# IvanBanny/para-ortho-pca-bo

Hardware: AMD Instinct MI355X
Metric: BO iterations/sec (incl. GP refit + EI opt), BBOB f15 d=40 (higher is better)
Workload: dtype f64; 1 GPU; configs[1]: PCA_BO on BBOB f15 d=40, budget=450, n_DoE=120, EI, var_threshold=0.95; one run per GPU (run list f15/d40/instances 0..N-1 partitioned by pcabo.sharding), timed steps spread evenly over the 330 BO iterations of the run; num_restarts=10, raw_samples=512, batch_limit=5, maxiter=200, parallelism=run-parallel x1

## Files before the change

para-ortho-pca-bo_amd/csrc/host_selftest.cpp:

```cpp
#include "../../include/pcabo.h"
#include "host_side.h"
#include "lb_plan.h"

#include <atomic>
#include <cmath>
#include <cstdint>
#include <cstdio>
#include <cstdlib>
#include <cstring>
#include <vector>

namespace {

int g_fail = 0;
#define CHECK(c, ...) do { if (!(c)) { std::fprintf(stderr, "FAIL %s:%d: ", __FILE__, __LINE__); std::fprintf(stderr, __VA_ARGS__); std::fprintf(stderr, "\n"); ++g_fail; } } while (0)

struct Lcg {
  uint64_t s;
  explicit Lcg(uint64_t seed) : s(seed * 6364136223846793005ull + 1442695040888963407ull) {}
  double uni() { s = s * 6364136223846793005ull + 1442695040888963407ull; return (double)(s >> 11) * (1.0 / 9007199254740992.0); }
};

struct Objective { std::vector<double> c; };
double fg_objective(const double* x, double* g, void* user) {
  const Objective* o = static_cast<const Objective*>(user);
  const int n = (int)o->c.size();
  double f = 0.0;
  for (int i = 0; i < n; ++i) {
    const double d = x[i] - o->c[i], s = 1.0 + 0.3 * std::sin(3.0 * x[i]);
    f += d * d * s;
    g[i] = 2.0 * d * s + d * d * 0.9 * std::cos(3.0 * x[i]);
  }
  for (int i = 0; i + 1 < n; ++i) { f += 0.1 * x[i] * x[i + 1]; g[i] += 0.1 * x[i + 1]; g[i + 1] += 0.1 * x[i]; }
  return f;
}

void test_minimize() {
  for (int nvar : {1, 2, 7, 33, 64, 65, 200}) {
    for (int variant = 0; variant < 3; ++variant) {
      pcabo_lbfgsb_set_vector_kernels(variant == 1);
      pcabo_lbfgsb_set_sum_order(variant == 2);
      Lcg r(17 + nvar);
      Objective o; o.c.resize(nvar);
      std::vector<double> x(nvar), lo(nvar), hi(nvar);
      for (int i = 0; i < nvar; ++i) { o.c[i] = 4.0 * r.uni() - 2.0; lo[i] = -1.0 - r.uni(); hi[i] = 1.0 + r.uni(); x[i] = 6.0 * r.uni() - 3.0; }
      double f = 0.0; int nit = 0, nfev = 0, task = 0;
      const int wf = pcabo_lbfgsb_minimize(nvar, x.data(), lo.data(), hi.data(), fg_objective, &o, 10, 1e7, 1e-5, 200, 15000, 20, &f, &nit, &nfev, &task);
      CHECK(wf >= 0 && wf <= 2, "warnflag %d", wf);
      CHECK(std::isfinite(f) && nfev >= 1, "f %g nfev %d", f, nfev);
      for (int i = 0; i < nvar; ++i) CHECK(x[i] >= lo[i] && x[i] <= hi[i], "x[%d] = %g outside the box", i, x[i]);
    }
  }
  pcabo_lbfgsb_set_vector_kernels(1);
  pcabo_lbfgsb_set_sum_order(0);
  {
    const int nvar = 12;
    Objective o; o.c.assign(nvar, 0.5);
    std::vector<double> x(nvar, 2.0), lo(nvar, -INFINITY), hi(nvar, INFINITY);
    for (int i = 0; i < nvar; i += 3) lo[i] = 0.75;
    for (int i = 1; i < nvar; i += 3) hi[i] = 0.25;
    double f = 0.0; int nit = 0, nfev = 0, task = 0;
    const int wf = pcabo_lbfgsb_minimize(nvar, x.data(), lo.data(), hi.data(), fg_objective, &o, 17, 1e7, 1e-5, 200, 15000, 20, &f, &nit, &nfev, &task);
    CHECK(wf == 0, "half-bounded problem: warnflag %d task %d", wf, task);
  }
  CHECK(pcabo_lbfgsb_minimize(0, nullptr, nullptr, nullptr, fg_objective, nullptr, 10, 1e7, 1e-5, 1, 1, 20, nullptr, nullptr, nullptr, nullptr) == PCABO_ERR_ARG, "bad arguments accepted");
}

void test_sobol() {
  for (int k : {1, 3, 36, 89}) {
    Lcg r(5 + k);
    std::vector<int64_t> state((size_t)k * 30), ltm((size_t)k * 30 * 30), shift(k);
    for (auto& v : state) v = (int64_t)(r.uni() * 1073741824.0);
    for (auto& v : ltm) v = r.uni() < 0.5 ? 0 : 1;
    for (auto& v : shift) v = (int64_t)(r.uni() * 1073741824.0);
    CHECK(pcabo_sobol_scramble(state.data(), ltm.data(), k) == PCABO_OK, "scramble");
    for (int n : {1, 2, 512, 513}) {
      std::vector<double> lo(k, -1.5), rng(k, 3.0), out((size_t)n * k, -7.0);
      CHECK(pcabo_sobol_draw(state.data(), shift.data(), k, n, lo.data(), rng.data(), out.data()) == PCABO_OK, "draw");
      for (double v : out) CHECK(v >= -1.5 && v <= 1.5, "sample %g outside the box", v);
      CHECK(pcabo_sobol_draw(state.data(), shift.data(), k, n, nullptr, nullptr, out.data()) == PCABO_OK, "draw (unit cube)");
      for (double v : out) CHECK(v >= 0.0 && v < 1.0, "unit sample %g", v);
    }
  }
}

void test_torch_rng() {
  struct Blob { uint64_t seed; int32_t left, seeded; uint64_t next; uint64_t state[624]; unsigned char tail[32]; };
  const int rows = 70, n = 512, n_pick = 10;
  std::vector<Blob> blobs(rows), again;
  std::vector<double> vals((size_t)rows * n);
  for (int r = 0; r < rows; ++r) {
    Lcg g(900 + r);
    blobs[r].seed = 900 + r; blobs[r].left = 1 + (r * 37) % 624; blobs[r].seeded = 1; blobs[r].next = 624 - blobs[r].left;
    for (auto& w : blobs[r].state) w = (uint64_t)(g.uni() * 4294967296.0);
    for (auto& c : blobs[r].tail) c = 0;
    for (int i = 0; i < n; ++i) vals[(size_t)r * n + i] = r == 5 ? 1.25 : 40.0 * g.uni() - 20.0;
  }
  again = blobs;
  std::vector<void*> ptr(rows);
  for (int r = 0; r < rows; ++r) ptr[r] = &blobs[r];
  ptr[7] = nullptr;
  std::vector<int64_t> out((size_t)rows * n_pick, -1), out1((size_t)rows * n_pick, -1);
  std::vector<int> flags(rows, -1), flags1(rows, -1);
  CHECK(pcabo_boltzmann_pick_rows(ptr.data(), vals.data(), rows, n, n_pick, 1.0, out.data(), flags.data()) == PCABO_OK, "pick rows");
  for (int r = 0; r < rows; ++r) {
    void* p1 = r == 7 ? nullptr : (void*)&again[r];
    CHECK(pcabo_boltzmann_pick_rows(&p1, vals.data() + (size_t)r * n, 1, n, n_pick, 1.0, out1.data() + (size_t)r * n_pick, flags1.data() + r) == PCABO_OK, "pick row %d", r);
    CHECK(flags[r] == flags1[r] && flags[r] == (r == 7 ? 2 : r == 5 ? 1 : 0), "flag of row %d: %d / %d", r, flags[r], flags1[r]);
    if (flags[r] != 0) continue;
    for (int j = 0; j < n_pick; ++j) {
      CHECK(out[(size_t)r * n_pick + j] == out1[(size_t)r * n_pick + j], "row %d pick %d differs between the all-rows call and the one-row call", r, j);
      CHECK(out[(size_t)r * n_pick + j] >= 0 && out[(size_t)r * n_pick + j] < n, "row %d pick %d out of range", r, j);
    }
    CHECK(blobs[r].left == again[r].left && blobs[r].next == again[r].next && blobs[r].state[0] == again[r].state[0], "generator of row %d", r);
  }
  std::vector<int64_t> bits(2000);
  CHECK(pcabo_torch_randint2(&blobs[0], 2000, bits.data()) == PCABO_OK, "randint2");
  for (int64_t b : bits) CHECK(b == 0 || b == 1, "bit %lld", (long long)b);
  std::vector<double> w((size_t)3 * n);
  Lcg g(77);
  for (auto& v : w) v = 0.01 + g.uni();
  void* three[3] = {&blobs[1], nullptr, &blobs[2]};
  std::vector<int64_t> idx(3 * n_pick, -1);
  CHECK(pcabo_torch_multinomial_rows(three, w.data(), 3, n, n_pick, idx.data()) == PCABO_OK, "multinomial rows");
  for (int j = 0; j < n_pick; ++j) CHECK(idx[j] >= 0 && idx[j] < n && idx[n_pick + j] == -1 && idx[2 * n_pick + j] >= 0, "multinomial pick %d", j);
  blobs[3].left = 900;
  CHECK(pcabo_torch_randint2(&blobs[3], 4, bits.data()) == PCABO_ERR_ARG, "a broken blob accepted");
}

void test_sobol_rows() {
  const int rows = 37, n = 130, kmax = 36;
  int ks[rows];
  for (int r = 0; r < rows; ++r) ks[r] = r == 0 ? 3 : r == 2 ? 1 : 1 + (r * 7) % 36;
  std::vector<std::vector<int64_t>> st(rows), sh(rows);
  std::vector<double> boxes((size_t)rows * 2 * kmax, NAN), out((size_t)rows * n * kmax, -7.0), one((size_t)n * kmax);
  std::vector<const int64_t*> sp(rows), hp(rows);
  std::vector<double*> op(rows);
  for (int r = 0; r < rows; ++r) {
    Lcg g(40 + r);
    st[r].resize((size_t)ks[r] * 30); sh[r].resize(ks[r]);
    for (auto& v : st[r]) v = (int64_t)(g.uni() * 1073741824.0);
    for (auto& v : sh[r]) v = (int64_t)(g.uni() * 1073741824.0);
    for (int j = 0; j < ks[r]; ++j) { boxes[(size_t)r * 2 * kmax + j] = -1.0 - j; boxes[(size_t)r * 2 * kmax + ks[r] + j] = 2.0 + r; }
    sp[r] = r == 2 ? nullptr : st[r].data(); hp[r] = sh[r].data(); op[r] = out.data() + (size_t)r * n * kmax;
  }
  CHECK(pcabo_sobol_draw_rows(sp.data(), hp.data(), ks, rows, n, boxes.data(), 2 * kmax, op.data()) == PCABO_OK, "draw rows");
  for (int r = 0; r < rows; ++r) {
    if (r == 2) { CHECK(op[r][0] == -7.0, "a skipped run was written"); continue; }
    std::vector<double> rng(ks[r]);
    for (int j = 0; j < ks[r]; ++j) rng[j] = boxes[(size_t)r * 2 * kmax + ks[r] + j] - boxes[(size_t)r * 2 * kmax + j];
    CHECK(pcabo_sobol_draw(st[r].data(), sh[r].data(), ks[r], n, boxes.data() + (size_t)r * 2 * kmax, rng.data(), one.data()) == PCABO_OK, "draw");
    for (int i = 0; i < n * ks[r]; ++i) CHECK(one[i] == op[r][i], "run %d element %d", r, i);
    if (ks[r] < kmax) CHECK(op[r][(size_t)n * ks[r]] == -7.0, "write behind the points of run %d", r);
  }
}

void test_plan() {
  std::vector<int> plan(LB_PLAN_INTS + 64, 0x5a5a5a5a);
  for (int NP = 64; NP <= LB_MAXNP; NP += 64) {
    const int S = NP / 64;
    for (int n = NP - 63; n <= NP; ++n) {
      lb_build_plan_t(plan.data(), n, S);
// ... 169 lines not shown
    for (int j = 0; j < n; ++j) {
      double v = 0.0;
      for (int p = std::max(i, j); p < n; ++p) v += Li[p * n + i] * Li[p * n + j];
      Kin[i * n + j] = v;
      a[i] += v * (gp.y[j] - c);
    }
  for (int t = 0; t < 6; ++t) h[t] = 0.0;
  for (int i = 0; i < n; ++i) {
    h[0] += std::log(L[i * n + i]); h[1] += (gp.y[i] - c) * a[i]; h[2] += a[i]; h[3] += a[i] * a[i]; h[4] += Kin[i * n + i];
    for (int j = 0; j < n; ++j) h[5] += (a[i] * a[j] - Kin[i * n + j]) * dK[i * n + j];
  }
  return true;
}
TinyGP tiny_gp(int seed, int n = 12, int k = 2) {
  Lcg r(seed);
  TinyGP gp; gp.n = n; gp.k = k; gp.Z.resize((size_t)n * k); gp.y.resize(n);
  for (auto& v : gp.Z) v = r.uni();
  for (int i = 0; i < n; ++i) gp.y[i] = std::sin(3.0 * gp.Z[i * k] + 0.3 * seed) + gp.Z[i * k + 1] * gp.Z[i * k + 1] - 0.6 + 0.1 * (r.uni() - 0.5);
  return gp;
}

struct FitOut { int status; double theta[3], loss; int info[4]; };
FitOut fit_out(const FitRun& r) {
  FitOut o;
  std::memset(&o, 0, sizeof(o));
  o.status = r.status;
  if (r.status == PCABO_OK) { std::memcpy(o.theta, r.xr, sizeof(o.theta)); o.loss = r.fr; r.report(o.info); }
  return o;
}
const double FIT_START[3] = {0.006737946999085467, 0.0, 0.0};

struct FitDrive { std::vector<FitOut> out; std::vector<std::vector<double>> evals; std::vector<int> rested; int rounds = 0; };
FitDrive drive_fits(const std::vector<TinyGP>& gps, const std::vector<const double*>& start, const std::vector<int>& fail_at) {
  const size_t B = gps.size();
  std::vector<FitRun> runs(B);
  std::vector<double> hs(6 * B, 0.0);
  FitDrive d;
  d.evals.resize(B); d.rested.assign(B, 0);
  for (size_t b = 0; b < B; ++b) { runs[b].bind(&hs[6 * b]); if (start[b]) runs[b].init(start[b]); }
  const int rc = fit_rounds(runs, gps[0].n, [&](const std::vector<const double*>& th, int* st) {
    ++d.rounds;
    for (size_t b = 0; b < B; ++b) {
      const FitRun& r = runs[b];
      if (!th[b]) { CHECK(r.state == FitRun::OUT, "run %zu: no theta but not out", b); continue; }
      const bool resting = r.state == FitRun::RESTING;
      if (resting) {
        CHECK(std::memcmp(th[b], r.xr, sizeof(r.xr)) == 0, "run %zu rests away from its result", b);
        ++d.rested[b];
      } else {
        d.evals[b].insert(d.evals[b].end(), th[b], th[b] + 3);
      }
      const bool fail = !resting && fail_at[b] > 0 && (int)d.evals[b].size() / 3 == fail_at[b];
      st[b] = !fail && tiny_gp_sums(gps[b], th[b], &hs[6 * b]) ? PCABO_OK : PCABO_ERR_NOT_PD;
    }
    return (int)PCABO_OK;
  });
  CHECK(rc == PCABO_OK, "fit_rounds: %d", rc);
  for (const FitRun& r : runs) {
    CHECK(r.state == FitRun::RESTING || r.state == FitRun::OUT, "a run is still stepping after the rounds");
    d.out.push_back(fit_out(r));
  }
  return d;
}

void test_fit_run() {
  {
    const TinyGP gp = tiny_gp(3);
    const double th[3] = {0.02, 0.15, -0.4};
    double h[6], f = 0.0, g[3], worst = 0.0;
    CHECK(tiny_gp_sums(gp, th, h), "the dense GP could not be factored");
    mll_assemble(h, gp.n, th, &f, g);
    for (int i = 0; i < 3; ++i) {
      const double step = i == 0 ? 1e-6 * th[0] : 1e-6;
      double tp[3] = {th[0], th[1], th[2]}, tm[3] = {th[0], th[1], th[2]}, fp = 0.0, fm = 0.0;
      tp[i] += step; tm[i] -= step;
      CHECK(tiny_gp_sums(gp, tp, h), "factor"); mll_assemble(h, gp.n, tp, &fp, nullptr);
      CHECK(tiny_gp_sums(gp, tm, h), "factor"); mll_assemble(h, gp.n, tm, &fm, nullptr);
      const double fd = (fp - fm) / (tp[i] - tm[i]), err = std::fabs(fd - g[i]) / (1.0 + std::fabs(g[i]));
      if (err > worst) worst = err;
      CHECK(err < 1e-6, "gradient %d: %.12g against the difference quotient %.12g", i, g[i], fd);
    }
    std::printf("mll_assemble against central differences: worst %.2e (bound 1e-6)\n", worst);
  }
  const int B = 5;
  std::vector<TinyGP> gps;
  for (int b = 0; b < B; ++b) gps.push_back(tiny_gp(10 + b));
  const FitDrive all = drive_fits(gps, std::vector<const double*>(B, FIT_START), std::vector<int>(B, 0));
  int rested = 0, nfev_min = 1 << 30, nfev_max = 0;
  for (int b = 0; b < B; ++b) {
    const FitDrive one = drive_fits({gps[b]}, {FIT_START}, {0});
    CHECK(all.out[b].status == PCABO_OK && all.out[b].info[0] > 2, "run %d: status %d after %d iterations", b, all.out[b].status, all.out[b].info[0]);
    CHECK(std::memcmp(&all.out[b], &one.out[0], sizeof(FitOut)) == 0, "run %d in lock-step differs from the run alone", b);
    CHECK(all.evals[b] == one.evals[0], "run %d was evaluated at other points in lock-step", b);
    CHECK(all.out[b].info[1] <= (int)all.evals[b].size() / 3, "run %d counts %d evaluations of %zu", b, all.out[b].info[1], all.evals[b].size() / 3);
    CHECK(one.rested[0] == 0 && one.rounds == (int)one.evals[0].size() / 3, "a run alone took a round without an evaluation");
    rested += all.rested[b];
    nfev_min = std::min(nfev_min, all.out[b].info[1]); nfev_max = std::max(nfev_max, all.out[b].info[1]);
  }
  CHECK(nfev_min < nfev_max && rested > 0, "no run finished before another (evaluations %d .. %d): nothing rode along", nfev_min, nfev_max);
  {
    const FitDrive d = drive_fits({gps[0], gps[1]}, {nullptr, FIT_START}, {0, 0});
    CHECK(d.out[0].status == PCABO_ERR_ARG && d.evals[0].empty(), "a parked run was stepped");
    CHECK(std::memcmp(&d.out[1], &all.out[1], sizeof(FitOut)) == 0, "a run beside a parked run differs from the run alone");
  }
  const int total = (int)all.evals[0].size() / 3;
  int end_at_last_evaluated = 0;
  for (int e = 1; e <= total; ++e) {
    const FitDrive d = drive_fits({gps[0], gps[1]}, {FIT_START, FIT_START}, {e, 0});
    CHECK(std::memcmp(&d.out[1], &all.out[1], sizeof(FitOut)) == 0, "failure %d of run 0 disturbed run 1", e);
    const FitOut& o = d.out[0];
    const std::vector<double>& ev = d.evals[0];
    if (e == 1) { CHECK(o.status == PCABO_ERR_NOT_PD && ev.size() == 3, "start not factored: status %d", o.status); continue; }
    CHECK(o.status == PCABO_OK && o.info[2] == 2 && o.info[3] == PCABO_FIT_TASK_NOT_PD, "failure %d: status %d warnflag %d task %d", e, o.status, o.info[2], o.info[3]);
    CHECK(o.info[1] == e - 1, "failure %d: %d evaluations counted", e, o.info[1]);
    CHECK((int)ev.size() / 3 == e + 1 && std::memcmp(&ev[3 * e], o.theta, sizeof(o.theta)) == 0, "failure %d: no evaluation at the result behind it", e);
    bool evaluated = false;
    for (int i = 0; i < e - 1; ++i) evaluated = evaluated || std::memcmp(&ev[3 * i], o.theta, sizeof(o.theta)) == 0;
    CHECK(evaluated, "failure %d: the result was never evaluated", e);
    if (std::memcmp(&ev[3 * (e - 2)], o.theta, sizeof(o.theta)) == 0) ++end_at_last_evaluated;
    double h[6], f = 0.0;
    CHECK(tiny_gp_sums(gps[0], o.theta, h), "factor"); mll_assemble(h, gps[0].n, o.theta, &f, nullptr);
    CHECK(f == o.loss, "failure %d: the loss is not the one at the result", e);
  }
  CHECK(end_at_last_evaluated > 0, "no failure met the first trial of a line search");
  {
    std::vector<FitRun> run(1);
    double h[6] = {0, 0, 0, 0, 0, 0};
    int evals = 0;
    std::vector<double> rhos;
    const int n = 12;
    const double G = 0.5;
    const auto linear = [&](const std::vector<const double*>& th, int* st) {
      const double s2 = th[0][0], rho = th[0][2], u = std::log(s2) + 4.0;
      CHECK(mll_theta_ok(th[0]), "asked to evaluate a theta outside the domain");
      h[1] = 2.0 * n * G * rho; h[5] = -2.0 * n * G * softplus_host(rho) * (1.0 + std::exp(-rho)); h[3] = 2.0 * (1.0 + u) / s2;
      ++evals; rhos.push_back(rho); st[0] = PCABO_OK;
      return (int)PCABO_OK;
    };
    run[0].bind(h); run[0].init(FIT_START);
    CHECK(fit_rounds(run, n, linear) == PCABO_OK, "fit_rounds");
    const FitOut o = fit_out(run[0]);
    CHECK(o.status == PCABO_OK && o.info[2] == 2 && o.info[3] == PCABO_FIT_TASK_DOMAIN, "domain stop: status %d warnflag %d task %d", o.status, o.info[2], o.info[3]);
    CHECK(o.info[0] >= 1 && evals == o.info[1] + 1 && evals > 3, "domain stop: %d iterations, %d evaluations, %d counted", o.info[0], evals, o.info[1]);
    CHECK(rhos.back() == o.theta[2] && rhos[evals - 2] < -600.0 && std::count(rhos.begin(), rhos.end(), o.theta[2]) == 2,
          "domain stop: the result rho %g is not an earlier iterate evaluated again at the end (last trial %g)", o.theta[2], rhos[evals - 2]);
    const double far[3] = {FIT_START[0], 0.0, -800.0};
    evals = 0;
    run[0].init(far);
    CHECK(fit_rounds(run, n, linear) == PCABO_OK, "fit_rounds");
    CHECK(run[0].status == PCABO_ERR_ARG && run[0].state == FitRun::OUT && evals == 0, "start outside the domain: status %d, %d evaluations", run[0].status, evals);
  }
}

}

int main(int argc, char** argv) {
  const int workers = argc > 1 ? std::atoi(argv[1]) : 4;
  test_minimize();
  test_sobol();
  test_sobol_rows();
  test_torch_rng();
  test_plan();
  test_restart_group();
  test_fit_run();
  test_gang_pool(1, 3);
  test_gang_pool(workers, 11);
  if (g_fail) { std::fprintf(stderr, "host selftest: %d check(s) failed\n", g_fail); return 1; }
  std::printf("host selftest ok\n");
  return 0;
}
```

para-ortho-pca-bo_amd/csrc/host_side.h:

```cpp
#pragma once
#include "../../include/pcabo.h"
#include "lbfgsb.h"

#include <algorithm>
#include <cmath>
#include <condition_variable>
#include <cstring>
#include <functional>
#include <mutex>
#include <thread>
#include <utility>
#include <vector>

struct RestartGroup : LbfgsbDriver {
  int q0 = 0, nq = 0, k = 0;
  std::vector<double> lo, hi, vc;
  void init(const double* ics, const double* bounds, int q0_, int nq_, int k_, int maxiter, int sum_order = 0) {
    q0 = q0_; nq = nq_; k = k_;
    lo.resize(nq * k); hi.resize(nq * k);
    for (int j = 0; j < nq; ++j)
      for (int c = 0; c < k; ++c) { lo[j * k + c] = bounds[c]; hi[j * k + c] = bounds[k + c]; }
    LbfgsbDriver::init(nq * k, ics + (size_t)q0 * k, lo.data(), hi.data(), sum_order, maxiter);
  }
  bool absorb(const double* hVal, const double* hGrad, int row) {
    double fs = 0.0;
    bool nan = false;
    for (int j = 0; j < nq; ++j) fs += hVal[row + j];
    for (int t = 0; t < nq * k; ++t) {
      const double gv = -hGrad[(size_t)row * k + t];
      if (gv != gv) nan = true;
      g[t] = gv;
    }
    if (nan) return false;
    LbfgsbDriver::absorb(-fs);
    vc.assign(hVal + row, hVal + row + nq);
    return true;
  }
};

struct RunRestarts {
  std::vector<RestartGroup> grp;
  int status = PCABO_OK;
  double* xq = nullptr;
  const double *val = nullptr, *grad = nullptr;
  void init(const double* ics, const double* bounds, int num_restarts, int batch_limit, int k, int maxiter, int sum_order = 0) {
    grp.resize((num_restarts + batch_limit - 1) / batch_limit);
    for (size_t gi = 0; gi < grp.size(); ++gi) {
      const int q0 = (int)gi * batch_limit;
      grp[gi].init(ics, bounds, q0, std::min(batch_limit, num_restarts - q0), k, maxiter, sum_order);
    }
    status = PCABO_OK;
  }
  void bind(double* xq_, const double* val_, const double* grad_) { xq = xq_; val = val_; grad = grad_; }
  template <class Redo> int end_points(double* cand, double* vals, Redo&& redo) const {
    int n = 0;
    for (const RestartGroup& rg : grp) {
      double* c = cand + (size_t)rg.q0 * rg.k;
      for (size_t t = 0; t < rg.x.size(); ++t) c[t] = rg.x[t] < rg.lo[t] ? rg.lo[t] : (rg.x[t] > rg.hi[t] ? rg.hi[t] : rg.x[t]);
      if (rg.have_cache && memcmp(c, rg.xc.data(), rg.x.size() * sizeof(double)) == 0) std::copy(rg.vc.begin(), rg.vc.end(), vals + rg.q0);
      else { redo(rg); ++n; }
    }
    return n;
  }
  int end_points(double* cand, double* vals) const { return end_points(cand, vals, [](const RestartGroup&) {}); }
  bool report(int* info, size_t slot0) const {
    bool any = false;
    for (size_t gi = 0; gi < grp.size(); ++gi) {
      const RestartGroup& rg = grp[gi];
      const int wf = rg.opt.warnflag();
      if (info) { int* o = info + 4 * (slot0 + gi); o[0] = rg.niter; o[1] = rg.nfev; o[2] = wf; o[3] = rg.opt.task(); }
      if (wf == 2) any = true;
    }
    return any;
  }
};

inline unsigned group_entry(int run, int q0, int nq) { return ((unsigned)run << 16) | ((unsigned)q0 << 8) | (unsigned)nq; }
inline unsigned query_entry(int run, int q) { return ((unsigned)run << 16) | (unsigned)q; }

template <class Stage, class Eval>
int run_rounds(RunRestarts* runs, const std::vector<int>& order, Stage&& stage, Eval&& eval) {
  std::vector<std::pair<RunRestarts*, RestartGroup*>> pend;
  size_t ng = 0;
  for (int b : order) ng += runs[b].grp.size();
  pend.reserve(ng);
  for (;;) {
    pend.clear();
    for (int b : order) {
      RunRestarts& run = runs[b];
      if (run.status != PCABO_OK) continue;
      for (RestartGroup& rg : run.grp) {
        if (!rg.advance()) continue;
        std::memcpy(run.xq + (size_t)rg.q0 * rg.k, rg.x.data(), rg.x.size() * sizeof(double));
        stage(b, rg);
        pend.push_back({&run, &rg});
      }
    }
    if (pend.empty()) return PCABO_OK;
    const int rc = eval();
    if (rc != PCABO_OK) return rc;
    for (auto& pe : pend)
      if (!pe.second->absorb(pe.first->val, pe.first->grad, pe.second->q0)) pe.first->status = PCABO_ERR_NAN;
  }
}

inline double softplus_host(double x) { return x > 20.0 ? x : std::log1p(std::exp(x)); }
inline bool mll_theta_ok(const double* theta) {
  const double s2 = theta[0], c = theta[1], ls = softplus_host(theta[2]);
  return s2 > 0.0 && std::isfinite(s2) && std::isfinite(c) && ls > 0.0 && std::isfinite(ls);
}
inline void mll_assemble(const double* h, int n, const double* theta, double* loss, double* grad) {
  const double s2 = theta[0], rho = theta[2];
  const double ls = softplus_host(rho);
  const double LOG2PI = 1.8378770664093453;
  const double lnz = std::log(s2), u = lnz + 4.0;
  const double log_n = -0.5 * h[1] - h[0] - 0.5 * n * LOG2PI;
  const double log_prior = -lnz - 0.5 * LOG2PI - 0.5 * u * u;
  *loss = -(log_n + log_prior) / n;
  if (grad) {
    const double sig = 1.0 / (1.0 + std::exp(-rho));
    grad[0] = -((0.5 * (h[3] - h[4])) + (-1.0 - u) / s2) / n;
    grad[1] = -h[2] / n;
    grad[2] = -(0.5 * h[5] * sig / ls) / n;
  }
}

struct FitRun {
  enum { STEPPING, END, RESTING, OUT };
  LbfgsbDriver fit;
  int state = OUT, status = PCABO_ERR_ARG, stop_task = 0;
  double xr[3] = {0, 0, 0}, fr = 0.0;
  const double* h = nullptr;
  void bind(const double* h_) { h = h_; }
  void init(const double* theta0) {
    const double lower[3] = {1e-4, -INFINITY, -INFINITY}, upper[3] = {INFINITY, INFINITY, INFINITY};
    fit.keep_accepted = true;
    fit.init(3, theta0, lower, upper);
    state = STEPPING; status = PCABO_OK; stop_task = 0;
  }
  const double* next() {
    if (state == STEPPING && !fit.advance()) finish();
    if (state == STEPPING && !mll_theta_ok(fit.x.data())) {
      if (fit.have_cache) { stop_task = PCABO_FIT_TASK_DOMAIN; finish(); }
      else { state = OUT; status = PCABO_ERR_ARG; }
    }
    return state == STEPPING ? fit.x.data() : (state == END ? xr : nullptr);
  }
  const double* rest() const { return state == RESTING ? xr : nullptr; }
  void took(int st, int n) {
    if (state == OUT) return;
    if (state == STEPPING && st == PCABO_ERR_NOT_PD && fit.have_cache) {
      stop_task = PCABO_FIT_TASK_NOT_PD;
      finish();
      return;
    }
    if (st != PCABO_OK) { state = OUT; status = st; return; }
    if (state == STEPPING) {
      double f = 0.0;
      mll_assemble(h, n, fit.x.data(), &f, fit.g.data());
      fit.absorb(f);
    } else if (state == END) {
      mll_assemble(h, n, xr, &fr, nullptr);
      state = RESTING;
    }
  }
  void report(int* info) const {
    info[0] = fit.niter; info[1] = fit.nfev;
    info[2] = stop_task ? 2 : fit.opt.warnflag();
    info[3] = stop_task ? stop_task : fit.opt.task();
  }

 private:
  void finish() {
    std::memcpy(xr, stop_task ? fit.xacc.data() : fit.x.data(), sizeof(xr));
    fr = fit.fc;
    state = (stop_task == PCABO_FIT_TASK_NOT_PD || !fit.have_cache || std::memcmp(xr, fit.xc.data(), sizeof(xr)) != 0) ? END : RESTING;
  }
};

template <class Eval>
int fit_rounds(std::vector<FitRun>& runs, int n, Eval&& eval) {
  std::vector<const double*> th(runs.size(), nullptr);
  std::vector<int> st(runs.size(), PCABO_OK);
  for (;;) {
    int pending = 0;
    for (size_t b = 0; b < runs.size(); ++b) {
      const double* t = runs[b].next();
      if (t) ++pending;
      th[b] = t ? t : runs[b].rest();
    }
    if (pending == 0) return PCABO_OK;
    const int rc = eval(th, st.data());
    if (rc != PCABO_OK) return rc;
    for (size_t b = 0; b < runs.size(); ++b) runs[b].took(st[b], n);
  }
}

struct GangPool {
  std::vector<std::thread> th;
  std::mutex mu;
  std::condition_variable cv, cv_done;
  std::function<void(int)> fn;
  unsigned epoch = 0;
  int pending = 0;
  bool quit = false;
  void start(int n) {
    const unsigned epoch0 = epoch;
    for (int i = 1; i < n; ++i)
      th.emplace_back([this, i, epoch0] {
        unsigned seen = epoch0;
        for (;;) {
          std::function<void(int)> f;
          {
            std::unique_lock<std::mutex> lk(mu);
            cv.wait(lk, [&] { return quit || epoch != seen; });
            if (quit) return;
            seen = epoch;
            f = fn;
          }
          f(i);
          { std::lock_guard<std::mutex> lk(mu); if (--pending == 0) cv_done.notify_all(); }
        }
      });
  }
  void run(std::function<void(int)> f) {
    {
      std::lock_guard<std::mutex> lk(mu);
      fn = f;
// ... 17 lines not shown
```

para-ortho-pca-bo_amd/csrc/kernels_acq.hip:

```cpp
#include "pcabo_internal.h"
#include <algorithm>
#include <cstdlib>
#include <mutex>

#define PSTRIDE (2 + 2 * PCABO_MAXD)

#ifdef PCABO_ACQ_TIMING
__device__ unsigned long long g_acq_stamps[16];
#define STAMP(i) do { if (blockIdx.x == gridDim.x / 2 && blockIdx.y == 0 && threadIdx.x == 0) g_acq_stamps[i] = wall_clock64(); } while (0)
#define STAMP_FIN(i) do { if (blockIdx.y == 0 && threadIdx.x == 0) g_acq_stamps[i] = wall_clock64(); } while (0)
extern "C" int pcabo_debug_acq_stamps(unsigned long long* out16) {
  return hipMemcpyFromSymbol(out16, HIP_SYMBOL(g_acq_stamps), sizeof(g_acq_stamps)) == hipSuccess ? 0 : -3;
}
#else
#define STAMP(i)
#define STAMP_FIN(i)
#endif

__device__ inline void st_wt(double* p, double v) {
  __hip_atomic_store(p, v, __ATOMIC_RELAXED, __HIP_MEMORY_SCOPE_AGENT);
}

template <int SLAB>
__device__ inline int slab_row(int s, int m, int NP) {
  return m < SLAB / 2 ? (SLAB / 2) * s + m : NP - (SLAB / 2) * (s + 1) + (m - SLAB / 2);
}

__device__ void acq_finish_query(const double* base, int S, int k, int q, const double* bounds4, const double* ystats,
                                 const AcqParams& p, double* val, double* grad, double* host_val, double* host_grad,
                                 int lane);

__device__ inline void grad_partial_sum(const double* base, int S, int c, int first, double* gs_out, double* gm_out) {
  double gs = 0.0, gm = 0.0;
  int sl = first;
  for (; sl + 21 < S; sl += 24) {
    double a[8], b[8];
#pragma unroll
    for (int t = 0; t < 8; ++t) {
      a[t] = base[(size_t)(sl + 3 * t) * PSTRIDE + 2 + c];
      b[t] = base[(size_t)(sl + 3 * t) * PSTRIDE + 2 + PCABO_MAXD + c];
    }
#pragma unroll
    for (int t = 0; t < 8; ++t) { gs += a[t]; gm += b[t]; }
  }
  {
    double a[8], b[8];
#pragma unroll
    for (int t = 0; t < 8; ++t) {
      const int si = sl + 3 * t;
      const int sc = si < S ? si : 0;
      a[t] = base[(size_t)sc * PSTRIDE + 2 + c];
      b[t] = base[(size_t)sc * PSTRIDE + 2 + PCABO_MAXD + c];
    }
#pragma unroll
    for (int t = 0; t < 8; ++t) { if (sl + 3 * t < S) { gs += a[t]; gm += b[t]; } }
  }
  *gs_out = gs;
  *gm_out = gm;
}

__device__ void acq_finish_scalar(const double* base, int S, int q, const double* ystats, const AcqParams& p, double* val,
                                  double* host_val, double* coef, int lane);
__device__ void acq_scalar_core(double vv, double mus, int q, double ym, double ysd, const AcqParams& p, double* val,
                                double* host_val, double* coef, int l);
template <int SLAB>
__device__ inline void acq_tail(int combine, double* s_v, double* partial, unsigned int* counters, int q, int S, int k,
                                const double* bounds4, const double* ystats, const AcqParams& prm, double* val,
                                double* grad, double* host_val, double* host_grad, HostMirror* hm,
                                unsigned long long seq, int tid, int w, int l) {
  if (!combine) return;
  int* s_flag = reinterpret_cast<int*>(s_v + SLAB);
  STAMP(6);
  asm volatile("s_waitcnt vmcnt(0)" ::: "memory");
  __syncthreads();
  STAMP(7);
  if (tid == 0) {
    unsigned int t = __hip_atomic_fetch_add(&counters[q], 1u, __ATOMIC_RELAXED, __HIP_MEMORY_SCOPE_AGENT);
    int last = ((t % (unsigned int)S) == (unsigned int)(S - 1));
    if (last) {
      __builtin_amdgcn_fence(__ATOMIC_ACQUIRE, "agent");
      asm volatile("s_waitcnt vmcnt(0)" ::: "memory");
    }
    *s_flag = last;
  }
  __syncthreads();
  if (!*s_flag) return;
  STAMP_FIN(8);
  const double* base = partial + (size_t)q * S * PSTRIDE;
  double* s_fin = s_v + SLAB + 2;
  double* s_coef = s_fin + 6 * PCABO_MAXD;
  double rng_c = 1.0;
  if (w == 0) {
    if (prm.want_grad && l < k) rng_c = bounds4[PCABO_MAXD + l] - bounds4[l];
    acq_finish_scalar(base, S, q, ystats, prm, val, host_val, s_coef, l);
  } else if (prm.want_grad) {
    for (int c = l; c < k; c += 64) {
      double gs, gm;
      grad_partial_sum(base, S, c, w - 1, &gs, &gm);
      s_fin[(w - 1) * 2 * PCABO_MAXD + c] = gs;
      s_fin[(w - 1) * 2 * PCABO_MAXD + PCABO_MAXD + c] = gm;
    }
  }
  __syncthreads();
  STAMP_FIN(13);
  if (w == 0) {
    if (prm.want_grad) {
      const double c_mu = s_coef[0], c_sg = s_coef[1];
      for (int c = l; c < k; c += 64) {
        const double gs = (s_fin[c] + s_fin[2 * PCABO_MAXD + c]) + s_fin[4 * PCABO_MAXD + c];
        const double gm = (s_fin[PCABO_MAXD + c] + s_fin[3 * PCABO_MAXD + c]) + s_fin[5 * PCABO_MAXD + c];
        const double g = __fma_rn(c_mu, gm, c_sg * gs) / (c == l ? rng_c : bounds4[PCABO_MAXD + c] - bounds4[c]);
        grad[(size_t)q * k + c] = g;
        if (host_grad) host_grad[(size_t)q * k + c] = g;
      }
    }
    if (hm && l == 0)
      __hip_atomic_store(const_cast<unsigned long long*>(&hm->qflag[q]), seq, __ATOMIC_RELEASE, __HIP_MEMORY_SCOPE_SYSTEM);
    STAMP_FIN(9);
#ifdef PCABO_ACQ_TIMING
    asm volatile("s_waitcnt vmcnt(0)" ::: "memory");
    STAMP_FIN(10);
#endif
  }
}

#define ACQ_BATCH_PROLOGUE()                                                                                     \
  unsigned run_ = blockIdx.z;                                                                                    \
  int qsel_ = -1;                                                                                                \
  if (ab.table) {                                                                                                \
    const unsigned e_ = reinterpret_cast<const unsigned*>(qa.x)[blockIdx.y];                                     \
    run_ = e_ >> 16; qsel_ = (int)(e_ & 0xffffu);                                                                \
  }                                                                                                              \
  if (ab.zs) {                                                                                                   \
    ZnT = zrun(ZnT, ab.zs, run_); R = zrun(R, ab.zs, run_); alpha = zrun(alpha, ab.zs, run_);                    \
    bounds4 = zrun(bounds4, ab.zs, run_); ystats = zrun(ystats, ab.zs, run_); partial = zrun(partial, ab.zs, run_); \
    counters = zrun(counters, ab.zs, run_); val = zrun(val, ab.zs, run_); grad = zrun(grad, ab.zs, run_);        \
    Xq = zrun(Xq, ab.xq_host ? ab.hzs : ab.zs, run_);                                                            \
    host_val = zrun(host_val, ab.hzs, run_); host_grad = zrun(host_grad, ab.hzs, run_); hm = zrun(hm, ab.hzs, run_); \
    if (ab.k_dev) k = *zrun(ab.k_dev, ab.zs, run_);                                                              \
    if (ab.bestf) prm.best_f = *zrun(ab.bestf, ab.zs, run_);                                                     \
    if (ab.hyp) prm.inv_ls = zrun(ab.hyp, ab.zs, run_)[PCABO_HYP_INV_LS];                                        \
  }                                                                                                              \
  (void)qsel_;

template <int SLAB>
__global__ __launch_bounds__(256) void k_acq_fused(
    QueryArgs qa, const double* __restrict__ Xq, int q_total, int n, int k, int NP, int ld,
    const double* __restrict__ ZnT, const double* __restrict__ R, const double* __restrict__ alpha,
    const double* __restrict__ bounds4, const double* __restrict__ ystats, AcqParams prm, double* partial,
    unsigned int* counters, double* __restrict__ val, double* __restrict__ grad,
    double* host_val, double* host_grad, HostMirror* hm, unsigned long long seq, int combine, int ,
    MailPair* , MailPair* , AcqBatch ab) {
  ACQ_BATCH_PROLOGUE()
  const double inv_ls = prm.inv_ls;
  const int kernel = prm.kernel, want_grad = prm.want_grad;
  extern __shared__ __attribute__((aligned(16))) double s_dyn[];
  double* s_ks = s_dyn;
  double* s_cf = s_dyn + NP;
  double* s_tm = s_dyn + 2 * NP;
  double* s_xn = s_dyn + 3 * NP;
  double* s_v = s_xn + PCABO_MAXD;
  const int tid = threadIdx.x, w = tid >> 6, l = tid & 63;
  const int s = blockIdx.x, q = ab.table ? qsel_ : (int)blockIdx.y, S = gridDim.x;
  double* out = partial + ((size_t)q * S + s) * PSTRIDE;
  STAMP(0);

  if (tid < k) {
    double lo = bounds4[tid], hi = bounds4[PCABO_MAXD + tid];
    double xv = Xq ? Xq[(size_t)q * k + tid] : qa.x[q * k + tid];
    s_xn[tid] = (xv - lo) / (hi - lo);
  }
  __syncthreads();
  STAMP(1);
  const double s5 = 2.23606797749979;
  for (int j = tid; j < NP; j += 256) {
    double ks = 0.0, cf = 0.0;
    if (j < n) {
      double sq = 0.0;
      for (int c = 0; c < k; ++c) { double dlt = s_xn[c] - ZnT[(size_t)c * ld + j]; sq += dlt * dlt; }
      sq *= inv_ls * inv_ls;
      if (kernel == 1) {
        ks = exp(-0.5 * sq);
        cf = -ks * inv_ls * inv_ls;
      } else {
        double dist = sqrt(fmax(sq, 1e-30));
        double e = exp(-s5 * dist);
        ks = ((s5 * dist + 1.0) + (5.0 / 3.0) * (dist * dist)) * e;
        cf = -(5.0 / 3.0) * (1.0 + s5 * dist) * e * inv_ls * inv_ls;
      }
    }
    s_ks[j] = ks;
    s_cf[j] = cf;
  }
  __syncthreads();
  STAMP(2);
  {
    constexpr int RW = SLAB / 4;
    int ri[RW];
    const double* Rr[RW];
    double acc[RW];
    int imax = 0;
#pragma unroll
    for (int u = 0; u < RW; ++u) {
      ri[u] = slab_row<SLAB>(s, w + 4 * u, NP); Rr[u] = R + (size_t)ri[u] * ld; acc[u] = 0.0; imax = max(imax, ri[u]);
    }
    for (int j = l; j <= imax; j += 64) {
      const double kj = s_ks[j];
#pragma unroll
      for (int u = 0; u < RW; ++u) acc[u] += Rr[u][j] * kj;
    }
#pragma unroll
    for (int u = 0; u < RW; ++u) acc[u] = wave_sum(acc[u]);
    if (l == 0) {
#pragma unroll
      for (int u = 0; u < RW; ++u) s_v[w + 4 * u] = acc[u];
    }
  }
  __syncthreads();
  STAMP(3);
  if (w == 0) {
    double vv = 0.0, mu = 0.0;
    if (l < SLAB) {
      const int i = slab_row<SLAB>(s, l, NP);
      const double vi = s_v[l];
      vv = vi * vi;
      if (i < n) mu = alpha[i] * s_ks[i];
    }
    vv = wave_sum(vv);
    mu = wave_sum(mu);
    if (l == 0) { st_wt(out + 0, vv); st_wt(out + 1, mu); }
  }
  if (want_grad) {
  __syncthreads();
  STAMP(4);
  for (int j = tid; j < NP; j += 256) {
    double wj = 0.0;
#pragma unroll
    for (int m = 0; m < SLAB; ++m) wj += R[(size_t)slab_row<SLAB>(s, m, NP) * ld + j] * s_v[m];
    const bool mine = ((j / (SLAB / 2)) == s) || (((NP - 1 - j) / (SLAB / 2)) == s);
    const double cf = s_cf[j];
    s_tm[j] = (mine && j < n) ? alpha[j] * cf : 0.0;
    s_ks[j] = wj * cf;
  }
  __syncthreads();
  STAMP(5);
  for (int c0 = 0; c0 < k; c0 += 32) {
    double gs[8], gm[8], xc[8];
    const double* zrow[8];
#pragma unroll
    for (int u = 0; u < 8; ++u) {
      const int c = c0 + w + 4 * u;
      const int cc = c < k ? c : 0;
      gs[u] = 0.0; gm[u] = 0.0; xc[u] = s_xn[cc]; zrow[u] = ZnT + (size_t)cc * ld;
    }
    for (int j = l; j < n; j += 64) {
      const double ts = s_ks[j], tm = s_tm[j];
#pragma unroll
      for (int u = 0; u < 8; ++u) {
        const double dlt = xc[u] - zrow[u][j];
        gs[u] += ts * dlt;
        gm[u] += tm * dlt;
      }
    }
#pragma unroll
    for (int u = 0; u < 8; ++u) { gs[u] = wave_sum(gs[u]); gm[u] = wave_sum(gm[u]); }
    if (l == 0) {
#pragma unroll
      for (int u = 0; u < 8; ++u) {
        const int c = c0 + w + 4 * u;
        if (c < k) { st_wt(out + 2 + c, gs[u]); st_wt(out + 2 + PCABO_MAXD + c, gm[u]); }
      }
    }
  }
  }

  acq_tail<SLAB>(combine, s_v, partial, counters, q, S, k, bounds4, ystats, prm, val, grad, host_val, host_grad, hm, seq, tid, w, l);
}

#define FIN_STAGE_PER_WAVE (11 * 2 * 40)
__device__ inline bool acq_server_finisher(const MailPair* rec, int S, int k, int q, unsigned long long seq,
                                           const double* ystats, const AcqParams& prm, double* val, double* grad,
                                           double* host_val, double* host_grad, HostMirror* hm, double rng_c,
                                           double* s_fin, double* s_coef, double* s_stage, int* s_srv,
                                           unsigned long long t0, int w, int l) {
  if (w == 0) {
    const double ym = ystats[0], ysd = ystats[1];
    const void* ptr[8];
    pcabo_u4 o[8];
    const MailPair* mine = rec + (size_t)(l < S ? l : 0) * PSTRIDE;
#pragma unroll
    for (int t = 0; t < 8; ++t) ptr[t] = mine + (t & 1);
    for (;;) {
      ld_pairs_sys8(ptr, o);
      const bool ok = pair_tag(o[0]) == seq && pair_tag(o[1]) == seq;
      if (__all(ok)) break;
      if (__any(wall_clock64() - t0 > PCABO_SERVER_TIMEOUT_TICKS)) { if (l == 0) *s_srv = 1; break; }
      __builtin_amdgcn_s_sleep(1);
    }
    double vm[2] = {l < S ? pair_value(o[0]) : 0.0, l < S ? pair_value(o[1]) : 0.0};
    wave_sum_multi<2>(vm, l);
    constexpr int lane_vv = wave_multi_lane(2, 0), lane_mus = wave_multi_lane(2, 1);
    const double vv = read_lane(vm[0], lane_vv), mus = read_lane(vm[0], lane_mus);
    acq_scalar_core(vv, mus, q, ym, ysd, prm, val, host_val, s_coef, l);
  } else if (prm.want_grad) {
    const int first = w - 1;
    const int ns = first < S ? (S - first + 2) / 3 : 0;
    const int total = ns * 2 * k;
    double* stage = s_stage + (size_t)(w - 1) * FIN_STAGE_PER_WAVE;
    for (int i0 = 0; i0 < total; i0 += 512) {
      const void* ptr[8];
      int item[8];
#pragma unroll
      for (int t = 0; t < 8; ++t) {
        const int i = i0 + l + 64 * t;
        item[t] = i < total ? i : -1;
        const int ii = i < total ? i : 0;
        const int st = ii / (2 * k), rem = ii - st * 2 * k, which = rem >= k, c = rem - which * k;
        ptr[t] = rec + (size_t)(first + 3 * st) * PSTRIDE + 2 + which * PCABO_MAXD + c;
      }
      pcabo_u4 o[8];
      for (;;) {
        ld_pairs_sys8(ptr, o);
        bool ok = true;
#pragma unroll
        for (int t = 0; t < 8; ++t) ok = ok && (item[t] < 0 || pair_tag(o[t]) == seq);
        if (__all(ok)) break;
        if (__any(wall_clock64() - t0 > PCABO_SERVER_TIMEOUT_TICKS)) { if (l == 0) *s_srv = 1; break; }
        __builtin_amdgcn_s_sleep(1);
      }
#pragma unroll
      for (int t = 0; t < 8; ++t) if (item[t] >= 0) stage[item[t]] = pair_value(o[t]);
    }
    __builtin_amdgcn_fence(__ATOMIC_RELEASE, "wavefront");
    __builtin_amdgcn_wave_barrier();
    __builtin_amdgcn_fence(__ATOMIC_ACQUIRE, "wavefront");
    if (l < k) {
      double gs = 0.0, gm = 0.0;
      for (int st = 0; st < ns; ++st) { gs += stage[st * 2 * k + l]; gm += stage[st * 2 * k + k + l]; }
      s_fin[(w - 1) * 2 * PCABO_MAXD + l] = gs;
      s_fin[(w - 1) * 2 * PCABO_MAXD + PCABO_MAXD + l] = gm;
    }
  }
  __syncthreads();
  if (*s_srv) return false;
  if (w == 0) {
    if (prm.want_grad && l < k) {
      const double c_mu = s_coef[0], c_sg = s_coef[1];
      const double gs = (s_fin[l] + s_fin[2 * PCABO_MAXD + l]) + s_fin[4 * PCABO_MAXD + l];
      const double gm = (s_fin[PCABO_MAXD + l] + s_fin[3 * PCABO_MAXD + l]) + s_fin[5 * PCABO_MAXD + l];
      const double g = __fma_rn(c_mu, gm, c_sg * gs) / rng_c;
      grad[(size_t)q * k + l] = g;
      if (host_grad) host_grad[(size_t)q * k + l] = g;
    }
    if (hm && l == 0)
      __hip_atomic_store(const_cast<unsigned long long*>(&hm->qflag[q]), seq, __ATOMIC_RELEASE, __HIP_MEMORY_SCOPE_SYSTEM);
  }
  return true;
}

#define FIN_LDS_DOUBLES (6 * PCABO_MAXD + 2 + 3 * FIN_STAGE_PER_WAVE + 2)
__device__ __noinline__ void acq_server_finish_main(double* s_mem, MailPair* dev_mail,
                                                    int ctrl_idx, const MailPair* part_pairs, int S, int k, int q,
                                                    const double* __restrict__ bounds4, const double* __restrict__ ystats,
                                                    const AcqParams& prm, double* val, double* grad, double* host_val,
                                                    double* host_grad, HostMirror* hm, unsigned long long seq) {
  double* s_fin = s_mem;
  int* s_srvp = reinterpret_cast<int*>(s_mem + FIN_LDS_DOUBLES - 1);
  const int tid = threadIdx.x, l = tid & 63;
  const int w = __builtin_amdgcn_readfirstlane(tid >> 6);
  double rng_c = 1.0;
  if (tid < k) rng_c = bounds4[PCABO_MAXD + tid] - bounds4[tid];
  for (unsigned long long cur_seq = seq;; ++cur_seq) {
    const unsigned long long t0 = wall_clock64();
    if (tid == 0) { s_srvp[0] = 0; s_srvp[1] = 0; }
    __syncthreads();
    if (w == 0) {
      for (;;) {
        const pcabo_u4 hd = ld_pair_sys(dev_mail + ctrl_idx);
        if (__all(mail_seq(hd) == cur_seq)) { if (pair_value(hd) == 0.0 && l == 0) *s_srvp = 1; break; }
        if (__any(wall_clock64() - t0 > PCABO_SERVER_TIMEOUT_TICKS)) { if (l == 0) *s_srvp = 1; break; }
        __builtin_amdgcn_s_sleep(1);
      }
    }
    __syncthreads();
    if (*s_srvp) return;
    if (!acq_server_finisher(part_pairs + (size_t)q * S * PSTRIDE, S, k, q, cur_seq, ystats, prm, val, grad, host_val,
                             host_grad, hm, rng_c, s_fin, s_fin + 6 * PCABO_MAXD, s_fin + 6 * PCABO_MAXD + 2, s_srvp, t0, w, l))
      return;
    __syncthreads();
  }
}

#define ACQ_SLAB32_NP 448
int acq_slabs(int NP) { return NP / (NP >= ACQ_SLAB32_NP ? 32 : 16); }

template <int NU, int CU>
__device__ inline void publish_grad(const double (&gs)[CU], const double (&gm)[CU], int w, int k, int l, MailPair* pout,
                                    double* out, unsigned long long seq) {
  static_assert(NU <= CU, "components per wave");
  double v[2 * NU];
#pragma unroll
  for (int u = 0; u < NU; ++u) { v[2 * u] = gs[u]; v[2 * u + 1] = gm[u]; }
  wave_sum_multi<2 * NU>(v, l);
  const int i = wave_multi_owner<2 * NU>(l);
  const int c = w + 4 * (i >> 1);
  if (i >= 0 && c < k) {
    const int off = 2 + (i & 1) * PCABO_MAXD + c;
    if (pout) st_pair_sys(pout + off, make_pair(v[0], seq));
    else st_wt(out + off, v[0]);
  }
}

template <int SLAB, int NB, bool SRV>
__global__ __launch_bounds__(256) void k_acq_fast(
    QueryArgs qa, const double* __restrict__ Xq, int q_total, int n, int k, int NP_rt, int ld,
    const double* __restrict__ ZnT, const double* __restrict__ R, const double* __restrict__ alpha,
    const double* __restrict__ bounds4, const double* __restrict__ ystats, AcqParams prm, double* partial,
    unsigned int* counters, double* __restrict__ val, double* __restrict__ grad,
    double* host_val, double* host_grad, HostMirror* hm, unsigned long long seq, int combine, int qb,
    MailPair* dev_mail, MailPair* part_pairs, AcqBatch ab) {
  if (!SRV) { ACQ_BATCH_PROLOGUE() }
  constexpr int NP = NB * 64;
  constexpr int CU = 10;
  constexpr int RW = SLAB / 4;
  constexpr int NM = (NB + 3) / 4;
  const double inv_ls = prm.inv_ls;
  const int kernel = prm.kernel, want_grad = prm.want_grad;
  extern __shared__ __attribute__((aligned(16))) double s_dyn[];
  double* s_ks = s_dyn;
  double* s_cf = s_dyn + NP;
  double* s_tm = s_dyn + 2 * NP;
  double* s_xn = s_dyn + 3 * NP;
  double* s_v = s_xn + PCABO_MAXD;
  double* s_p4 = s_v + SLAB + 2;
  const int tid = threadIdx.x, l = tid & 63;
  const int w = __builtin_amdgcn_readfirstlane(tid >> 6);
  constexpr bool server = SRV;
  const int s = blockIdx.x, S = server ? (int)gridDim.x - 1 : (int)gridDim.x;
  if (server && s == S) {
    acq_server_finish_main(s_dyn, dev_mail, 1 + q_total * k + (int)blockIdx.y, part_pairs, S, k,
                           blockIdx.y, bounds4, ystats, prm, val, grad, host_val, host_grad, hm, seq);
    return;
  }
  STAMP(0);

  double z[CU][NB], r[RW][NB], al[NM];
  const unsigned lane8 = (unsigned)l * 8u;
#pragma unroll
  for (int u = 0; u < CU; ++u) {
    const int c = w + 4 * u;
    const char* zr = reinterpret_cast<const char*>(ZnT + (size_t)c * ld);
#pragma unroll
    for (int b = 0; b < NB; ++b) {
      z[u][b] = 0.0;
      if (c < k) z[u][b] = *reinterpret_cast<const double*>(zr + lane8 + 512 * b);
    }
  }
#pragma unroll
  for (int u = 0; u < RW; ++u) {
    const int ri = slab_row<SLAB>(s, w + 4 * u, NP);
    const char* Rr = reinterpret_cast<const char*>(R + (size_t)ri * ld);
#pragma unroll
    for (int b = 0; b < NB; ++b) {
      r[u][b] = 0.0;
      if (64 * b <= ri) r[u][b] = *reinterpret_cast<const double*>(Rr + lane8 + 512 * b);
    }
  }
#pragma unroll
  for (int m = 0; m < NM; ++m) { const int j = tid + 256 * m; al[m] = j < n ? alpha[j] : 0.0; }
  int* s_srv = reinterpret_cast<int*>(s_v + SLAB + 1);
  unsigned long long cur_seq = seq;
  double b_lo = 0.0, b_hi = 1.0;
  if (server && l < k) { b_lo = bounds4[l]; b_hi = bounds4[PCABO_MAXD + l]; }
  for (;;) {
  int q = (!SRV && ab.table) ? (int)(reinterpret_cast<const unsigned*>(qa.x)[blockIdx.y] & 0xffffu) : (int)blockIdx.y * qb;
  double* out = partial + ((size_t)q * S + s) * PSTRIDE;
  if (server) {
    const unsigned long long t0 = wall_clock64();
    if (tid == 0) { s_srv[0] = 0; s_srv[1] = 0; }
    __syncthreads();
    if (w == 0) {
      volatile int* flags = s_srv;
      const void* ptr[8];
#pragma unroll
      for (int t = 0; t < 8; ++t) ptr[t] = (t & 1) && l < k ? (const void*)(dev_mail + 1 + q * k + l) : (const void*)(dev_mail + 1 + q_total * k + q);
      for (;;) {
        pcabo_u4 o[8];
        ld_pairs_sys8(ptr, o);
        const bool ctl = mail_seq(o[0]) == cur_seq;
        const bool bye = ctl && pair_value(o[0]) == 0.0;
        const bool ok = ctl && (bye || l >= k || mail_seq(o[1]) == cur_seq);
        if (__all(ok)) {
          if (pair_value(o[0]) == 0.0) { if (l == 0) flags[0] = 1; }
          else if (l < k) s_xn[l] = (pair_value(o[1]) - b_lo) / (b_hi - b_lo);
          break;
        }
        if (__any(wall_clock64() - t0 > PCABO_SERVER_TIMEOUT_TICKS)) { if (l == 0) flags[0] = 1; break; }
        __builtin_amdgcn_s_sleep(1);
      }
    }
    __syncthreads();
    if (*s_srv) return;
  }
  MailPair* pout = server ? part_pairs + ((size_t)q * S + s) * PSTRIDE : nullptr;
  for (int qi = 0; qi < qb; ++qi, ++q, out += (size_t)S * PSTRIDE) {
  if (q >= q_total) break;
  if (qi > 0) __syncthreads();
  if (!server) {
  if (tid < k) {
    double lo = bounds4[tid], hi = bounds4[PCABO_MAXD + tid];
    double xv = Xq ? Xq[(size_t)q * k + tid] : qa.x[q * k + tid];
    s_xn[tid] = (xv - lo) / (hi - lo);
  }
  __syncthreads();
  }
  STAMP(1);
  double xc[CU];
#pragma unroll
  for (int u = 0; u < CU; ++u) xc[u] = s_xn[(w + 4 * u < k) ? w + 4 * u : k - 1];
  {
    double sq[NB];
#pragma unroll
    for (int b = 0; b < NB; ++b) sq[b] = 0.0;
#pragma unroll
    for (int u = 0; u < CU; ++u) {
      if (w + 4 * u < k) {
#pragma unroll
        for (int b = 0; b < NB; ++b) { const double d = xc[u] - z[u][b]; sq[b] += d * d; }
      }
    }
#pragma unroll
    for (int b = 0; b < NB; ++b) s_p4[w * NP + l + 64 * b] = sq[b];
  }
  __syncthreads();
  const double s5 = 2.23606797749979;
#pragma unroll
  for (int m = 0; m < NM; ++m) {
    const int j = tid + 256 * m;
    if (j < NP) {
      double ks = 0.0, cf = 0.0;
      if (j < n) {
        double sq = ((s_p4[j] + s_p4[NP + j]) + s_p4[2 * NP + j]) + s_p4[3 * NP + j];
        sq *= inv_ls * inv_ls;
        if (kernel == 1) {
          ks = exp(-0.5 * sq);
          cf = -ks * inv_ls * inv_ls;
        } else {
          double dist = sqrt(fmax(sq, 1e-30));
          double e = exp(-s5 * dist);
          ks = ((s5 * dist + 1.0) + (5.0 / 3.0) * (dist * dist)) * e;
          cf = -(5.0 / 3.0) * (1.0 + s5 * dist) * e * inv_ls * inv_ls;
        }
      }
      s_ks[j] = ks;
      s_cf[j] = cf;
    }
  }
  __syncthreads();
  STAMP(2);
  {
    double acc[RW];
#pragma unroll
    for (int u = 0; u < RW; ++u) acc[u] = 0.0;
#pragma unroll
    for (int b = 0; b < NB; ++b) {
      const double kj = s_ks[l + 64 * b];
#pragma unroll
      for (int u = 0; u < RW; ++u) acc[u] += r[u][b] * kj;
    }
    wave_sum_multi<RW>(acc, l);
    const int u = wave_multi_owner<RW>(l);
    if (u >= 0) s_v[w + 4 * u] = acc[0];
  }
  __syncthreads();
  STAMP(3);
  if (w == 0) {
    double vv = 0.0, mu = 0.0;
    if (l < SLAB) {
      const int i = slab_row<SLAB>(s, l, NP);
      const double vi = s_v[l];
      vv = vi * vi;
      if (i < n) mu = alpha[i] * s_ks[i];
    }
    double vm[2] = {vv, mu};
    wave_sum_multi<2>(vm, l);
    const int i = wave_multi_owner<2>(l);
    if (i >= 0) {
      if (server) st_pair_sys(pout + i, make_pair(vm[0], cur_seq));
      else st_wt(out + i, vm[0]);
    }
  }
  if (want_grad) {
  {
    double vw[RW];
#pragma unroll
    for (int u = 0; u < RW; ++u) vw[u] = s_v[w + 4 * u];
#pragma unroll
    for (int b = 0; b < NB; ++b) {
      double pw = 0.0;
#pragma unroll
      for (int u = 0; u < RW; ++u) pw += r[u][b] * vw[u];
      s_p4[w * NP + l + 64 * b] = pw;
    }
  }
  __syncthreads();
  STAMP(4);
#pragma unroll
  for (int m = 0; m < NM; ++m) {
    const int j = tid + 256 * m;
    if (j < NP) {
      const double wj = ((s_p4[j] + s_p4[NP + j]) + s_p4[2 * NP + j]) + s_p4[3 * NP + j];
      const bool mine = ((j / (SLAB / 2)) == s) || (((NP - 1 - j) / (SLAB / 2)) == s);
      const double cf = s_cf[j];
      s_tm[j] = mine ? al[m] * cf : 0.0;
      s_ks[j] = wj * cf;
    }
  }
  __syncthreads();
  STAMP(5);
  {
    double gs[CU], gm[CU];
#pragma unroll
    for (int u = 0; u < CU; ++u) { gs[u] = 0.0; gm[u] = 0.0; }
#pragma unroll
    for (int b = 0; b < NB; ++b) {
      const double ts = s_ks[l + 64 * b], tm = s_tm[l + 64 * b];
#pragma unroll
      for (int u = 0; u < CU; ++u) {
        const double dlt = xc[u] - z[u][b];
        gs[u] += ts * dlt;
        gm[u] += tm * dlt;
      }
    }
    const int nu = k > w ? (k - w + 3) / 4 : 0;
    if (nu > 5) publish_grad<10>(gs, gm, w, k, l, pout, out, cur_seq);
    else if (nu > 2) publish_grad<5>(gs, gm, w, k, l, pout, out, cur_seq);
    else if (nu > 0) publish_grad<2>(gs, gm, w, k, l, pout, out, cur_seq);
  }
  }
  }
  q = (!SRV && ab.table) ? (int)(reinterpret_cast<const unsigned*>(qa.x)[blockIdx.y] & 0xffffu) : (int)blockIdx.y * qb;
  out = partial + ((size_t)q * S + s) * PSTRIDE;
  if (!server) {
    acq_tail<SLAB>(combine, s_v, partial, counters, q, S, k, bounds4, ystats, prm, val, grad, host_val, host_grad, hm, cur_seq, tid, w, l);
    break;
  }
  ++cur_seq;
  __syncthreads();
  }
}

__device__ inline void log_ei_helper(double u, double* h, double* dh) {
  const double inv_sqrt2 = 0.7071067811865476;
  const double inv_sqrt_2pi = 0.3989422804014327;
  const double log2pi = 1.8378770664093453;
  if (u > -1.0) {
    double phi = inv_sqrt_2pi * exp(-0.5 * u * u);
    double Phi = 0.5 * erfc(-inv_sqrt2 * u);
    double ei = phi + u * Phi;
    *h = log(ei);
    *dh = Phi / ei;
    return;
  }
  double log_phi = -0.5 * (u * u + log2pi);
  if (u > -1e6) {
    const double ex = erfcx(-inv_sqrt2 * u);
    const double E = (ex * fabs(u)) * 1.2533141373155003;
    *h = log_phi + log1p(-E);
    const double dw = (u + 0.7978845608028654 / ex) + 1.0 / u;
    *dh = -u - dw * E / (1.0 - E);
  } else {
    *h = log_phi - 2.0 * log(fabs(u));
    *dh = -u - 2.0 / u;
  }
}

__device__ void acq_scalar_core(double vv, double mus, int q, double ym, double ysd, const AcqParams& p, double* val,
                                double* host_val, double* coef, int l) {
  const double mu = ym + ysd * mus;
  double var = (1.0 - vv) * (ysd * ysd);
  bool clamped = false;
  if (!(var >= 1e-10)) { var = 1e-10; clamped = true; }
  if (var < 1e-12) { var = 1e-12; clamped = true; }
  const double sigma = sqrt(var);
  double u = (mu - p.best_f) / sigma;
  const double sgn = p.maximize ? 1.0 : -1.0;
  u *= sgn;
  double value, dv_du, dv_dsig;
  if (p.acq == 0) {
    double h, dh;
    log_ei_helper(u, &h, &dh);
    value = h + log(sigma);
    dv_du = dh;
    dv_dsig = 1.0 / sigma;
  } else {
    value = 0.5 * erfc(-0.7071067811865476 * u);
    dv_du = 0.3989422804014327 * exp(-0.5 * u * u);
    dv_dsig = 0.0;
  }
  if (l == 0) {
    val[q] = value;
    if (host_val) host_val[q] = value;
    coef[0] = dv_du * sgn * ysd / sigma;
    coef[1] = clamped ? 0.0 : (dv_dsig - dv_du * u / sigma) * (-(ysd * ysd) / sigma);
  }
  STAMP_FIN(12);
}

__device__ void acq_finish_scalar(const double* base, int S, int q, const double* ystats, const AcqParams& p, double* val,
                                  double* host_val, double* coef, int l) {
  const double ym = ystats[0], ysd = ystats[1];
  double vv = 0.0, mus = 0.0;
  for (int s = l; s < S; s += 64) { vv += base[(size_t)s * PSTRIDE]; mus += base[(size_t)s * PSTRIDE + 1]; }
  vv = wave_sum(vv);
  mus = wave_sum(mus);
  STAMP_FIN(11);
  acq_scalar_core(vv, mus, q, ym, ysd, p, val, host_val, coef, l);
}

__device__ void acq_finish_query(const double* base, int S, int k, int q, const double* bounds4, const double* ystats,
                                 const AcqParams& p, double* val, double* grad, double* host_val, double* host_grad,
                                 int l) {
  __shared__ double s_cf2[4][2];
  double* coef = s_cf2[(threadIdx.x >> 6) & 3];
  acq_finish_scalar(base, S, q, ystats, p, val, host_val, coef, l);
  if (p.want_grad) {
    __builtin_amdgcn_wave_barrier();
    const double c_mu = coef[0], c_sg = coef[1];
    for (int c = l; c < k; c += 64) {
      double a0, b0, a1, b1, a2, b2;
      grad_partial_sum(base, S, c, 0, &a0, &b0);
      grad_partial_sum(base, S, c, 1, &a1, &b1);
      grad_partial_sum(base, S, c, 2, &a2, &b2);
      const double gs = (a0 + a1) + a2, gm = (b0 + b1) + b2;
      double g = __fma_rn(c_mu, gm, c_sg * gs) / (bounds4[PCABO_MAXD + c] - bounds4[c]);
      grad[(size_t)q * k + c] = g;
      if (host_grad) host_grad[(size_t)q * k + c] = g;
    }
  }
}

__global__ __launch_bounds__(256) void k_acq_combine(const double* __restrict__ partial, int q_total, int S, int k,
                                                     const double* __restrict__ bounds4,
                                                     const double* __restrict__ ystats, AcqParams p,
                                                     double* __restrict__ val, double* __restrict__ grad, AcqBatch ab) {
  if (ab.zs) {
    const unsigned run_ = blockIdx.z;
    partial = zrun(partial, ab.zs, run_); bounds4 = zrun(bounds4, ab.zs, run_); ystats = zrun(ystats, ab.zs, run_);
    val = zrun(val, ab.zs, run_); grad = zrun(grad, ab.zs, run_);
    if (ab.k_dev) k = *zrun(ab.k_dev, ab.zs, run_);
    if (ab.bestf) p.best_f = *zrun(ab.bestf, ab.zs, run_);
  }
  const int q = blockIdx.x * 4 + (threadIdx.x >> 6);
  if (q < q_total)
    acq_finish_query(partial + (size_t)q * S * PSTRIDE, S, k, q, bounds4, ystats, p, val, grad, nullptr, nullptr,
                     threadIdx.x & 63);
}

#ifdef PCABO_ACQ_TIMING
#define GSTAMP(i) do { if (blockIdx.x == gridDim.x - 1 && blockIdx.y == 0 && threadIdx.x == 0) g_acq_stamps[i] = wall_clock64(); } while (0)
#else
#define GSTAMP(i)
#endif
#define GQ 5
#define GT_LD 17
#define WAVE_LDS_SYNC() asm volatile("s_waitcnt lgkmcnt(0)" ::: "memory")
template <int NT>
__global__ __launch_bounds__(256) void k_acq_group(
    QueryArgs qa, const double* __restrict__ Xq, int n, int k, int NP, int ld,
    const double* __restrict__ ZnT, const double* __restrict__ R, const double* __restrict__ alpha,
    const double* __restrict__ bounds4, const double* __restrict__ ystats, AcqParams prm, double* partial,
    unsigned int* counters, double* __restrict__ val, double* __restrict__ grad, double* host_val, double* host_grad,
    HostMirror* hm, unsigned long long seq, AcqBatch ab) {
  const unsigned ent = reinterpret_cast<const unsigned*>(qa.x)[blockIdx.y];
  const unsigned run_ = ent >> 16;
  const int q0 = (int)((ent >> 8) & 0xffu), nq = (int)(ent & 0xffu);
  if (ab.zs) {
    ZnT = zrun(ZnT, ab.zs, run_); R = zrun(R, ab.zs, run_); alpha = zrun(alpha, ab.zs, run_);
    bounds4 = zrun(bounds4, ab.zs, run_); ystats = zrun(ystats, ab.zs, run_); partial = zrun(partial, ab.zs, run_);
    counters = zrun(counters, ab.zs, run_); val = zrun(val, ab.zs, run_); grad = zrun(grad, ab.zs, run_);
    Xq = zrun(Xq, ab.xq_host ? ab.hzs : ab.zs, run_);
    host_val = zrun(host_val, ab.hzs, run_); host_grad = zrun(host_grad, ab.hzs, run_); hm = zrun(hm, ab.hzs, run_);
    if (ab.k_dev) k = *zrun(ab.k_dev, ab.zs, run_);
    if (ab.bestf) prm.best_f = *zrun(ab.bestf, ab.zs, run_);
    if (ab.hyp) prm.inv_ls = zrun(ab.hyp, ab.zs, run_)[PCABO_HYP_INV_LS];
  }
  const int tid = threadIdx.x, l = tid & 63;
  const int w = __builtin_amdgcn_readfirstlane(tid >> 6);
  const int s = blockIdx.x, S = gridDim.x;
  const int r0 = 64 * s, ncol = 64 * (s + 1);
  const int KS = (k + 1) & ~1;
  extern __shared__ __attribute__((aligned(16))) double s_dyn[];
  double* s_ks = s_dyn;
  double* s_tile = s_ks + GQ * NP;
  double* s_v = s_tile + 4 * 64 * GT_LD;
  double* s_tm = s_v + 64 * 8;
  double* s_coef = s_tm + GQ * 64;
  int* s_flag = reinterpret_cast<int*>(s_coef + 2 * GQ);
  double* s_vvmu = s_coef + 2 * GQ + 4;
  double* s_xn = s_vvmu + 2 * GQ;
  double* s_part = s_tile;
  double* s_gout = s_ks;
  const double inv_ls = prm.inv_ls;
  const int kernel = prm.kernel;

  GSTAMP(0);
  for (int idx = tid; idx < GQ * k; idx += 256) {
    const int q = idx / k, c = idx - q * k;
    const int qq = q < nq ? q : 0;
    const double lo = bounds4[c], hi = bounds4[PCABO_MAXD + c];
    s_xn[q * KS + c] = (Xq[(size_t)(q0 + qq) * k + c] - lo) / (hi - lo);
  }
  __syncthreads();
  GSTAMP(1);
  double cfr[NT][GQ];
  const double s5 = 2.23606797749979;
  {
    const int jlim = n < ncol ? n : ncol;
    double sq[NT][GQ];
#pragma unroll
    for (int t = 0; t < NT; ++t)
#pragma unroll
      for (int q = 0; q < GQ; ++q) sq[t][q] = 0.0;
    constexpr int CB = NT == 1 ? 40 : (NT == 2 ? 20 : 8);
    for (int c0 = 0; c0 < k; c0 += CB) {
      double z[NT][CB];
#pragma unroll
      for (int t = 0; t < NT; ++t)
#pragma unroll
        for (int u = 0; u < CB; ++u) {
          const int cc = c0 + u < k ? c0 + u : k - 1, jj = tid + 256 * t < NP ? tid + 256 * t : NP - 1;
          z[t][u] = ZnT[(size_t)cc * ld + jj];
        }
#pragma unroll
      for (int u = 0; u < CB; ++u) {
        if (c0 + u < k) {
#pragma unroll
          for (int q = 0; q < GQ; ++q) {
            const double xq = s_xn[q * KS + c0 + u];
#pragma unroll
            for (int t = 0; t < NT; ++t) { const double d = xq - z[t][u]; sq[t][q] += d * d; }
          }
        }
      }
    }
#pragma unroll
    for (int t = 0; t < NT; ++t) {
      const int j = tid + 256 * t;
#pragma unroll
      for (int q = 0; q < GQ; ++q) {
        double ks = 0.0, cf = 0.0;
        if (j < jlim) {
          const double sqq = sq[t][q] * (inv_ls * inv_ls);
          if (kernel == 1) {
// ... 304 lines not shown

#define SC_QB 16
__global__ __launch_bounds__(256) void k_score_ks(const double* __restrict__ Xq, int q_total, int n, int k, int NP, int ld,
                                                  const double* __restrict__ ZnT, const double* __restrict__ alpha,
                                                  const double* __restrict__ bounds4, AcqParams prm,
                                                  double* __restrict__ KS, double* __restrict__ partial, int S, AcqBatch ab) {
  if (ab.zs) {
    const unsigned run_ = blockIdx.z;
    Xq = zrun(Xq, ab.zs, run_); ZnT = zrun(ZnT, ab.zs, run_); alpha = zrun(alpha, ab.zs, run_);
    bounds4 = zrun(bounds4, ab.zs, run_); KS = zrun(KS, ab.zs, run_); partial = zrun(partial, ab.zs, run_);
    if (ab.k_dev) k = *zrun(ab.k_dev, ab.zs, run_);
    if (ab.hyp) prm.inv_ls = zrun(ab.hyp, ab.zs, run_)[PCABO_HYP_INV_LS];
  }
  __shared__ double s_xn[SC_QB][PCABO_MAXD];
  __shared__ double s_mu[4][SC_QB];
  const int tid = threadIdx.x, l = tid & 63, w = tid >> 6;
  const int j = blockIdx.x * 256 + tid, q0 = blockIdx.y * SC_QB;
  for (int idx = tid; idx < SC_QB * k; idx += 256) {
    const int q = idx / k, c = idx - q * k;
    const int qq = q0 + q < q_total ? q0 + q : q_total - 1;
    const double lo = bounds4[c], hi = bounds4[PCABO_MAXD + c];
    s_xn[q][c] = (Xq[(size_t)qq * k + c] - lo) / (hi - lo);
  }
  __syncthreads();
  double sq[SC_QB];
#pragma unroll
  for (int q = 0; q < SC_QB; ++q) sq[q] = 0.0;
  if (j < n) {
    for (int c0 = 0; c0 < k; c0 += 8) {
      double z[8];
#pragma unroll
      for (int u = 0; u < 8; ++u) z[u] = (c0 + u < k) ? ZnT[(size_t)(c0 + u) * ld + j] : 0.0;
#pragma unroll
      for (int u = 0; u < 8; ++u)
        if (c0 + u < k) {
#pragma unroll
          for (int q = 0; q < SC_QB; ++q) { const double d = s_xn[q][c0 + u] - z[u]; sq[q] += d * d; }
        }
    }
  }
  const double inv_ls = prm.inv_ls, s5 = 2.23606797749979;
  const double aj = j < n ? alpha[j] : 0.0;
#pragma unroll
  for (int q = 0; q < SC_QB; ++q) {
    double ks = 0.0;
    if (j < n) {
      const double sqq = sq[q] * (inv_ls * inv_ls);
      if (prm.kernel == 1) ks = exp(-0.5 * sqq);
      else {
        const double dist = sqrt(fmax(sqq, 1e-30));
        ks = ((s5 * dist + 1.0) + (5.0 / 3.0) * (dist * dist)) * exp(-s5 * dist);
      }
    }
    if (j < NP && q0 + q < q_total) KS[(size_t)(q0 + q) * ld + j] = ks;
    const double m = wave_sum(aj * ks);
    if (l == 0) s_mu[w][q] = m;
  }
  __syncthreads();
  if (tid < SC_QB && q0 + tid < q_total)
    partial[((size_t)(q0 + tid) * S + blockIdx.x) * PSTRIDE + 1] = ((s_mu[0][tid] + s_mu[1][tid]) + s_mu[2][tid]) + s_mu[3][tid];
}

__global__ __launch_bounds__(256) void k_score_gemm(const double* __restrict__ R, const double* __restrict__ KS,
                                                    int q_total, int NP, int ld, int njb, double* __restrict__ partial,
                                                    size_t zs) {
  ZRUN(R); ZRUN(KS); ZRUN(partial);
  __shared__ __attribute__((aligned(16))) double s_a[64 * PCABO_TLD];
  __shared__ __attribute__((aligned(16))) double s_b[64 * PCABO_TLD];
  __shared__ double s_red[4][64];
  const int tid = threadIdx.x, w = tid >> 6, l = tid & 63;
  const int I = blockIdx.x, qb = blockIdx.y, S = gridDim.x;
  const double* Rrow = R + (size_t)(I * 64) * ld;
  const double* Krow = KS + (size_t)(qb * 64) * ld;
  double pa[16], pb[16];
  auto fetch = [&](int J) {
#pragma unroll
    for (int u = 0; u < 16; ++u) {
      const int idx = tid + 256 * u, r = idx >> 6, c = idx & 63;
      pa[u] = Rrow[(size_t)r * ld + J * 64 + c];
      pb[u] = (qb * 64 + r < q_total) ? Krow[(size_t)r * ld + J * 64 + c] : 0.0;
    }
  };
  auto put = [&]() {
#pragma unroll
    for (int u = 0; u < 16; ++u) {
      const int idx = tid + 256 * u, r = idx >> 6, c = idx & 63;
      s_a[r * PCABO_TLD + c] = pa[u];
      s_b[r * PCABO_TLD + c] = pb[u];
    }
  };
  double4_t acc[4];
#pragma unroll
  for (int t = 0; t < 4; ++t) acc[t] = (double4_t){0.0, 0.0, 0.0, 0.0};
  fetch(0);
  for (int J = 0; J <= I; ++J) {
    __syncthreads();
    put();
    if (J < I) fetch(J + 1);
    __syncthreads();
    for (int kk = 0; kk < 64; kk += 4) {
      const double a = s_a[(16 * w + (l & 15)) * PCABO_TLD + kk + (l >> 4)];
#pragma unroll
      for (int t = 0; t < 4; ++t) {
        const double b = s_b[(16 * t + (l & 15)) * PCABO_TLD + kk + (l >> 4)];
        acc[t] = __builtin_amdgcn_mfma_f64_16x16x4f64(a, b, acc[t], 0, 0, 0);
      }
    }
  }
#pragma unroll
  for (int t = 0; t < 4; ++t) {
    double v = ((acc[t][0] * acc[t][0] + acc[t][1] * acc[t][1]) + acc[t][2] * acc[t][2]) + acc[t][3] * acc[t][3];
    v += __shfl_xor(v, 16, 64);
    v += __shfl_xor(v, 32, 64);
    if (l < 16) s_red[w][16 * t + l] = v;
  }
  __syncthreads();
  if (tid < 64 && qb * 64 + tid < q_total) {
    double* rec = partial + ((size_t)(qb * 64 + tid) * S + I) * PSTRIDE;
    rec[0] = ((s_red[0][tid] + s_red[1][tid]) + s_red[2][tid]) + s_red[3][tid];
    if (I >= njb) rec[1] = 0.0;
  }
}

bool score_gemm_possible(int q) { return q >= 64; }

void launch_score(hipStream_t st, const double* Xq, int q, int n, int k, int NP, int ld, const double* ZnT, const double* R,
                  const double* alpha, const double* bounds4, const double* ystats, AcqParams p, double* KS, double* partial,
                  double* val, AcqBatch ab, int B) {
  const int S = NP / 64, njb = (NP + 255) / 256;
  hipLaunchKernelGGL(k_score_ks, dim3(njb, (q + SC_QB - 1) / SC_QB, B), dim3(256), 0, st, Xq, q, n, k, NP, ld, ZnT, alpha, bounds4,
                     p, KS, partial, S, ab);
  hipLaunchKernelGGL(k_score_gemm, dim3(S, (q + 63) / 64, B), dim3(256), 0, st, R, KS, q, NP, ld, njb, partial, ab.zs);
  p.want_grad = 0;
  hipLaunchKernelGGL(k_acq_combine, dim3((q + 3) / 4, 1, B), dim3(256), 0, st, partial, q, S, k, bounds4, ystats, p, val,
                     (double*)nullptr, ab);
}

bool acq_server_possible(int q, int n, int k, int NP) {
  static int cus = -1;
  if (cus < 0) {
    int dev = 0;
    if (hipGetDevice(&dev) != hipSuccess || hipDeviceGetAttribute(&cus, hipDeviceAttributeMultiprocessorCount, dev) != hipSuccess) cus = 0;
  }
  if (k > 40 || NP > 512 || q < 1 || q > PCABO_INLAUNCH_MAXQ || (size_t)q * k > PCABO_QA_MAX) return false;
  const int S = acq_slabs(NP);
  return (S + 1) * q <= cus && S <= 32;
}

void launch_acq(hipStream_t st, const QueryArgs* qa, const double* Xq, int q, int n, int k, int NP, int ld,
                const double* ZnT, const double* R, const double* alpha, const double* bounds4, const double* ystats,
                AcqParams p, double* partial, unsigned int* counters, double* val,
                double* grad, double* host_val, double* host_grad, HostMirror* hm, unsigned long long seq,
                MailPair* dev_mail, MailPair* part_pairs, AcqBatch ab, int B,
                int table_entries) {
  const int slab = NP >= ACQ_SLAB32_NP ? 32 : 16;
  const int S = NP / slab;
  static const QueryArgs empty = {};
  const int combine = hm != nullptr;
  const int nb = NP / 64;
  const bool fast = k <= 40 && nb <= 8;
  const int qb = (fast && !combine && q >= 64) ? 8 : 1;
  const int gy = ab.table ? table_entries : (q + qb - 1) / qb;
  const int gz = ab.table ? 1 : B;
#define ACQ_ARGS qa ? *qa : empty, Xq, q, n, k, NP, ld, ZnT, R, alpha, bounds4, ystats, p, partial, counters, val, grad, \
                 host_val, host_grad, hm, seq, combine, qb, dev_mail, part_pairs, ab
  const int FIN_LDS = 6 * PCABO_MAXD + 2;
#define ACQ_LDS(SL, NBV) (3 * NBV * 64 + PCABO_MAXD + SL + 2 + (4 * NBV * 64 > FIN_LDS ? 4 * NBV * 64 : FIN_LDS))
#define ACQ_FAST(SL, NBV)                                                                                      \
  case NBV:                                                                                                    \
    if (dev_mail)                                                                                              \
      hipLaunchKernelGGL((k_acq_fast<SL, NBV, true>), dim3(S + 1, gy), dim3(256),                              \
                         (size_t)std::max<int>(ACQ_LDS(SL, NBV), FIN_LDS_DOUBLES) * sizeof(double), st, ACQ_ARGS); \
    else                                                                                                       \
      hipLaunchKernelGGL((k_acq_fast<SL, NBV, false>), dim3(S, gy, gz), dim3(256),                             \
                         (size_t)ACQ_LDS(SL, NBV) * sizeof(double), st, ACQ_ARGS);                             \
    break;
  if (fast) {
    if (slab == 16) {
      switch (nb) { ACQ_FAST(16, 1) ACQ_FAST(16, 2) ACQ_FAST(16, 3) ACQ_FAST(16, 4) ACQ_FAST(16, 5) ACQ_FAST(16, 6)
                    ACQ_FAST(16, 7) ACQ_FAST(16, 8) }
    } else {
      switch (nb) { ACQ_FAST(32, 1) ACQ_FAST(32, 2) ACQ_FAST(32, 3) ACQ_FAST(32, 4) ACQ_FAST(32, 5) ACQ_FAST(32, 6)
                    ACQ_FAST(32, 7) ACQ_FAST(32, 8) }
    }
  } else {
    size_t lds = (size_t)(3 * NP + PCABO_MAXD + 32 + 2 + 6 * PCABO_MAXD + 2) * sizeof(double);
    if (slab == 16)
      hipLaunchKernelGGL(k_acq_fused<16>, dim3(S, ab.table ? gy : q, gz), dim3(256), lds, st, ACQ_ARGS);
    else
      hipLaunchKernelGGL(k_acq_fused<32>, dim3(S, ab.table ? gy : q, gz), dim3(256), lds, st, ACQ_ARGS);
  }
#undef ACQ_FAST
#undef ACQ_LDS
#undef ACQ_ARGS
  if (!combine)
    hipLaunchKernelGGL(k_acq_combine, dim3((q + 3) / 4, 1, gz), dim3(256), 0, st, partial, q, S, k, bounds4, ystats, p, val,
                       grad, ab);
}

template <int N>
__global__ __launch_bounds__(64) void k_debug_wave_sum_multi(const double* __restrict__ in, double* ref, double* multi,
                                                             double* uni, int* mism) {
  const int l = threadIdx.x;
  double v[N];
#pragma unroll
  for (int i = 0; i < N; ++i) v[i] = in[i * 64 + l];
#pragma unroll
  for (int i = 0; i < N; ++i) { const double r = wave_sum(v[i]); if (l == 0) ref[i] = r; }
  wave_sum_multi<N>(v, l);
  const int own = wave_multi_owner<N>(l), idx = wave_multi_index<N>(l);
  if (own >= 0) multi[own] = v[0];
  __syncthreads();
  if (__double_as_longlong(multi[idx]) != __double_as_longlong(v[0])) atomicAdd(&mism[idx], 1);
#pragma unroll
  for (int i = 0; i < N; ++i) { const double r = read_lane(v[0], __builtin_amdgcn_readfirstlane(wave_multi_lane(N, i))); if (l == 0) uni[i] = r; }
}

extern "C" int pcabo_debug_wave_sum_multi(const double* in, int N, double* ref, double* multi, double* uni, int* mism) {
  double* d = nullptr;
  if (hipMalloc(&d, (size_t)N * (64 + 3) * sizeof(double) + (size_t)N * sizeof(int)) != hipSuccess) return -3;
  double *dref = d + N * 64, *dmul = dref + N, *duni = dmul + N;
  int* dmis = reinterpret_cast<int*>(duni + N);
  int rc = hipMemcpy(d, in, (size_t)N * 64 * sizeof(double), hipMemcpyHostToDevice) == hipSuccess ? 0 : -3;
  if (rc == 0 && hipMemset(dref, 0, (size_t)N * 3 * sizeof(double) + (size_t)N * sizeof(int)) != hipSuccess) rc = -3;
#define DBG_WSM(NV) case NV: hipLaunchKernelGGL(k_debug_wave_sum_multi<NV>, dim3(1), dim3(64), 0, 0, d, dref, dmul, duni, dmis); break;
  if (rc == 0) {
    switch (N) { DBG_WSM(1) DBG_WSM(2) DBG_WSM(3) DBG_WSM(4) DBG_WSM(5) DBG_WSM(7) DBG_WSM(8) DBG_WSM(10) DBG_WSM(13)
                 DBG_WSM(20) DBG_WSM(33) DBG_WSM(64) default: rc = -1; }
  }
#undef DBG_WSM
  if (rc == 0 && hipGetLastError() != hipSuccess) rc = -3;
  if (rc == 0 && (hipMemcpy(ref, dref, N * sizeof(double), hipMemcpyDeviceToHost) != hipSuccess ||
                  hipMemcpy(multi, dmul, N * sizeof(double), hipMemcpyDeviceToHost) != hipSuccess ||
                  hipMemcpy(uni, duni, N * sizeof(double), hipMemcpyDeviceToHost) != hipSuccess ||
                  hipMemcpy(mism, dmis, N * sizeof(int), hipMemcpyDeviceToHost) != hipSuccess)) rc = -3;
  (void)hipFree(d);
  return rc;
}
```

para-ortho-pca-bo_amd/csrc/pcabo_api.hip:

```cpp
#include "../../include/pcabo.h"
#include "pcabo_internal.h"
#include "lbfgsb.h"
#include "host_side.h"

#include <algorithm>
#include <atomic>
#include <chrono>
#include <thread>
#include <condition_variable>
#include <functional>
#include <mutex>
#include <cstdlib>
#include <cmath>
#include <cstdio>
#include <cstring>
#include <new>
#include <optional>
#include <vector>
#include <dirent.h>
#include <fcntl.h>
#include <signal.h>
#include <stdint.h>
#include <cerrno>
#include <unistd.h>
#include <emmintrin.h>

#define PCABO_ABI_VERSION 2
#define PROF_GROUPS 6
#define PROF_POOL 4096

struct ProfPair { hipEvent_t a, b; int group; double bytes, flops; };

struct OptHelper {
  std::thread th;
  std::mutex mu;
  std::condition_variable cv;
  std::atomic<unsigned> go{0}, done{0};
  std::atomic<bool> quit{false}, active{false};
  std::function<void()> fn;
  void run() {
    unsigned seen = 0;
    while (true) {
      {
        std::unique_lock<std::mutex> lk(mu);
        cv.wait(lk, [&] { return active.load(std::memory_order_acquire) || quit.load(std::memory_order_acquire); });
      }
      if (quit.load(std::memory_order_acquire)) return;
      while (active.load(std::memory_order_acquire)) {
        const unsigned cur = go.load(std::memory_order_acquire);
        if (cur == seen) { __builtin_ia32_pause(); continue; }
        seen = cur;
        fn();
        done.store(cur, std::memory_order_release);
      }
    }
  }
  void start() { if (!th.joinable()) th = std::thread([this] { run(); }); }
  void begin(std::function<void()> f) {
    start();
    fn = std::move(f);
    { std::lock_guard<std::mutex> lk(mu); active.store(true, std::memory_order_release); }
    cv.notify_one();
  }
  void end() { active.store(false, std::memory_order_release); }
  void shutdown() {
    if (!th.joinable()) return;
    { std::lock_guard<std::mutex> lk(mu); quit.store(true, std::memory_order_release); active.store(false, std::memory_order_release); }
    cv.notify_one();
    th.join();
  }
};

struct pcabo_ctx {
  int device = 0;
  hipStream_t stream = nullptr;
  hipEvent_t evBounds = nullptr;
  hipEvent_t evPca = nullptr;
  int max_n = 0, max_d = 0, max_q = 0;
  int NPcap = 0, ld = 0, DPcap = 0, KPcap = 0, Scap = 0;
  int ptr_mode = PCABO_PTR_HOST;
  int n = 0, d = 0, k = 0, NP = 0, KP = 0;
  bool have_wpca = false, have_gp = false, gp_pending = false;
  int wpca_n = 0, wpca_d = 0; bool wpca_uncollected = false;
  double lengthscale = 0.0, noise = 0.0;
  int kernel = 0;
  double *dX = nullptr, *dNoise = nullptr, *dF = nullptr, *dWeights = nullptr, *dWc = nullptr;
  long long* dRanks = nullptr;
  double *dDataMean = nullptr, *dPcaMean = nullptr, *dC = nullptr, *dG = nullptr, *dLam = nullptr;
  double* dGbuf[2] = {nullptr, nullptr};
  int gcur = 0, vprev_d = 0;
  double *dComps = nullptr, *dEvr = nullptr, *dZ = nullptr;
  double* dPcaOut = nullptr;
  double *dIn = nullptr, *hIn = nullptr;
  int *dK = nullptr, *dSweeps = nullptr, *dInfo = nullptr;
  double *dY = nullptr, *dYs = nullptr, *dYstats = nullptr, *dBounds4 = nullptr, *dZnMean = nullptr, *dUserNB = nullptr;
  double *dZnT = nullptr, *dAT = nullptr, *dNrm = nullptr, *dGram = nullptr, *dL = nullptr, *dR = nullptr;
  double *dTmp = nullptr, *dAlpha = nullptr, *dDiag = nullptr;
  double *dXq = nullptr, *dPartial = nullptr, *dVal = nullptr, *dGrad = nullptr, *dZq = nullptr, *dXout = nullptr;
  unsigned int* dCounters = nullptr;
  int cnt_S = 0; bool cnt_dirty = true;
  double* dKS = nullptr;
  double* dBestF = nullptr;
  double* dMll = nullptr;
  double* dHyp = nullptr;
  char *dRegion = nullptr, *hRegion = nullptr;
  size_t region_bytes = 0, hregion_bytes = 0;
  bool in_batch = false; int batch_index = 0;
  bool rt_stale = false;
  HostMirror* hm = nullptr;
  double *hXq = nullptr, *hVal = nullptr, *hGrad = nullptr, *hSmall = nullptr, *hBestF = nullptr;
  double* hMll = nullptr;
  double* hHyp = nullptr;
  MailPair* dMail = nullptr;
  bool mail_bar = false;
  MailPair* dPairs = nullptr;
  bool opt_resident = true;
  bool opt_group_acq = false;
  bool bestf_f32 = true;
  int srv_penalty = 0;
  unsigned long long seq = 0;
  OptHelper helper;
  std::vector<std::unique_ptr<OptHelper>> more_helpers;
  bool registered = false;
  bool alone = true; int alone_age = 0;
  char err[512] = {0};
  bool prof = false;
  std::vector<ProfPair> pairs;
  size_t pairs_used = 0;
  double prof_ms[PROF_GROUPS] = {0};
  double prof_pair_ms = 0.0;
  double prof_empty_ms = 0.0;
  int64_t prof_launches[PROF_GROUPS] = {0};
  double prof_bytes[PROF_GROUPS] = {0}, prof_flops[PROF_GROUPS] = {0};
};

static std::mutex g_presence_mu;
static int g_presence_refs[64] = {0};
static void presence_path(char* buf, size_t n, int device, long pid) { snprintf(buf, n, "/dev/shm/pcabo.%d.%ld", device, pid); }
static void presence_register(int device) {
  if (device < 0 || device >= 64) return;
  std::lock_guard<std::mutex> lk(g_presence_mu);
  if (g_presence_refs[device]++ == 0) {
    char path[128]; presence_path(path, sizeof(path), device, (long)getpid());
    int fd = open(path, O_CREAT | O_WRONLY, 0644);
    if (fd >= 0) close(fd);
  }
}
static void presence_unregister(int device) {
  if (device < 0 || device >= 64) return;
  std::lock_guard<std::mutex> lk(g_presence_mu);
  if (g_presence_refs[device] > 0 && --g_presence_refs[device] == 0) {
    char path[128]; presence_path(path, sizeof(path), device, (long)getpid());
    unlink(path);
  }
}
static int presence_local_contexts(int device) {
  if (device < 0 || device >= 64) return 1;
  std::lock_guard<std::mutex> lk(g_presence_mu);
  return g_presence_refs[device];
}
static bool presence_alone(int device) {
  DIR* d = opendir("/dev/shm");
  if (!d) return true;
  char prefix[64]; snprintf(prefix, sizeof(prefix), "pcabo.%d.", device);
  const size_t pl = strlen(prefix);
  bool alone = true;
  while (struct dirent* e = readdir(d)) {
    if (strncmp(e->d_name, prefix, pl) != 0) continue;
    const long pid = atol(e->d_name + pl);
    if (pid <= 0 || pid == (long)getpid()) continue;
    if (kill((pid_t)pid, 0) == 0 || errno == EPERM) { alone = false; break; }
    char path[300]; snprintf(path, sizeof(path), "/dev/shm/%s", e->d_name);
    unlink(path);
  }
  closedir(d);
  return alone;
}

static int set_err(pcabo_ctx* c, int code, const char* fmt, const char* a = "", int v = 0) {
  if (c) snprintf(c->err, sizeof(c->err), fmt, a, v);
  if (c && (code == PCABO_ERR_TIMEOUT || code == PCABO_ERR_HIP)) c->cnt_dirty = true;
  return code;
}
#define HIPCHK(call)                                                                         \
  do {                                                                                       \
    hipError_t e_ = (call);                                                                  \
    if (e_ != hipSuccess) return set_err(ctx, PCABO_ERR_HIP, "HIP error: %s (line %d)", hipGetErrorString(e_), __LINE__); \
  } while (0)

static hipError_t wait_stream(hipStream_t s) {
  const auto t0 = std::chrono::steady_clock::now();
  for (unsigned spins = 1;; ++spins) {
    hipError_t e = hipStreamQuery(s);
    if (e != hipErrorNotReady) return e == hipSuccess ? hipStreamSynchronize(s) : e;
    if ((spins & 63) == 0 && std::chrono::steady_clock::now() - t0 > std::chrono::milliseconds(2)) break;
    __builtin_ia32_pause();
  }
  return hipStreamSynchronize(s);
}
static hipError_t wait_event(hipEvent_t ev) {
  const auto t0 = std::chrono::steady_clock::now();
  for (unsigned spins = 1;; ++spins) {
    hipError_t e = hipEventQuery(ev);
    if (e != hipErrorNotReady) return e;
    if ((spins & 63) == 0 && std::chrono::steady_clock::now() - t0 > std::chrono::milliseconds(2)) break;
    __builtin_ia32_pause();
  }
  return hipEventSynchronize(ev);
}
enum FlagWait { FLAGS_SET, FLAGS_LATE, FLAGS_UNPUBLISHED };
static FlagWait wait_flags(const HostMirror* hm, int q0, int nq, unsigned long long seq,
                           std::chrono::steady_clock::time_point deadline, const hipStream_t* s = nullptr) {
  unsigned long spins = 0;
  for (int q = q0; q < q0 + nq; ++q)
    while (__atomic_load_n(&hm->qflag[q], __ATOMIC_ACQUIRE) != seq) {
      if ((++spins & 0xFFFF) != 0) continue;
      if (s && hipStreamQuery(*s) == hipSuccess) {
        if (__atomic_load_n(&hm->qflag[q], __ATOMIC_ACQUIRE) == seq) break;
        return FLAGS_UNPUBLISHED;
      }
      if (std::chrono::steady_clock::now() > deadline) return FLAGS_LATE;
    }
  return FLAGS_SET;
}
static std::chrono::steady_clock::time_point deadline_in(int seconds) {
  return std::chrono::steady_clock::now() + std::chrono::seconds(seconds);
}

static inline void put_mail_pair(MailPair* dst, double v, unsigned long long seq) {
  unsigned long long vb; memcpy(&vb, &v, 8);
  const __m128i x = _mm_set_epi64x((long long)(seq ^ mail_mix(vb)), (long long)vb);
  _mm_store_si128(reinterpret_cast<__m128i*>(dst), x);
}
static bool host_mapping_writable(const void* p, size_t len) {
  FILE* f = fopen("/proc/self/maps", "r");
  if (!f) return false;
  const unsigned long long a = (unsigned long long)(uintptr_t)p, b = a + len;
  char line[512];
  bool ok = false;
  while (fgets(line, sizeof(line), f)) {
    unsigned long long lo = 0, hi = 0;
    char perms[8] = {0};
    if (sscanf(line, "%llx-%llx %7s", &lo, &hi, perms) != 3) continue;
    if (a >= lo && b <= hi) { ok = perms[0] == 'r' && perms[1] == 'w'; break; }
  }
  fclose(f);
  return ok;
}
static bool mail_bar_usable(pcabo_ctx* ctx) {
  int large = 0;
  if (hipDeviceGetAttribute(&large, hipDeviceAttributeIsLargeBar, ctx->device) != hipSuccess) { (void)hipGetLastError(); large = 0; }
  if (!large) return false;
  if (!host_mapping_writable(ctx->dMail, PCABO_MAIL_PAIRS * sizeof(MailPair))) return false;
  MailPair* probe = ctx->dMail + (PCABO_MAIL_PAIRS - 1);
  put_mail_pair(probe, 42.5, 0x1234ull);
  _mm_sfence();
  MailPair back{0.0, 0};
  if (hipMemcpy(&back, probe, sizeof(back), hipMemcpyDeviceToHost) != hipSuccess) { (void)hipGetLastError(); return false; }
  unsigned long long vb; const double v = 42.5; memcpy(&vb, &v, 8);
  const bool seen = back.v == 42.5 && back.tag == (0x1234ull ^ mail_mix(vb));
  put_mail_pair(probe, 0.0, 0); _mm_sfence();
  return seen;
}

__global__ void k_nop() {}

static void prof_resolve(pcabo_ctx* c) {
  if (c->pairs_used == 0) return;
  (void)hipStreamSynchronize(c->stream);
  for (size_t i = 0; i < c->pairs_used; ++i) {
    float ms = 0.f;
    if (hipEventElapsedTime(&ms, c->pairs[i].a, c->pairs[i].b) == hipSuccess) {
      ms = ms > (float)c->prof_pair_ms ? ms - (float)c->prof_pair_ms : 0.f;
      c->prof_ms[c->pairs[i].group] += ms;
      c->prof_launches[c->pairs[i].group] += 1;
      c->prof_bytes[c->pairs[i].group] += c->pairs[i].bytes;
      c->prof_flops[c->pairs[i].group] += c->pairs[i].flops;
    }
  }
  c->pairs_used = 0;
}
struct ProfScope {
  pcabo_ctx* c; ProfPair* p = nullptr;
  ProfScope(pcabo_ctx* ctx, int group, double bytes = 0.0, double flops = 0.0) : c(ctx) {
    if (!c->prof) return;
    if (c->pairs_used == c->pairs.size()) prof_resolve(c);
    p = &c->pairs[c->pairs_used++];
    p->group = group; p->bytes = bytes; p->flops = flops;
    (void)hipEventRecord(p->a, c->stream);
  }
  ~ProfScope() { if (p) (void)hipEventRecord(p->b, c->stream); }
};

static double acq_bytes(int n, int k, int q, int grad) {
  return 4.0 * n * (n + 1.0) + 8.0 * n * k + 8.0 * n + 8.0 * q * k + 8.0 * q * (grad ? 1 + k : 1);
}
static double acq_flops(int n, int k, int q, int grad) {
  double v = 3.0 * n * k + 20.0 * n + (double)n * n;
  if (grad) v += (double)n * n + 4.0 * n * k;
  return q * v;
}

template <typename T>
static hipError_t dalloc(T** p, size_t count) { return hipMalloc((void**)p, count * sizeof(T)); }

extern "C" {

int pcabo_abi_version(void) { return PCABO_ABI_VERSION; }

int pcabo_device_count(void) {
  int n = 0;
  if (hipGetDeviceCount(&n) != hipSuccess) return 0;
  return n;
}

}

struct Carver {
  char* base; size_t off = 0;
  template <typename T> T* take(size_t count) {
    off = (off + 255) & ~(size_t)255;
    T* p = base ? reinterpret_cast<T*>(base + off) : nullptr;
    off += count * sizeof(T);
    return p;
  }
};
static size_t carve_device(pcabo_ctx* ctx, char* base) {
  Carver c{base};
  const size_t N = ctx->NPcap, D = ctx->DPcap, n = ctx->max_n, d = ctx->max_d, Q = ctx->max_q;
  ctx->dX = c.take<double>(n * d);        ctx->dNoise = c.take<double>(n * d);
  ctx->dF = c.take<double>(n);            ctx->dWeights = c.take<double>(n);
  ctx->dWc = c.take<double>((n + 4) * D); ctx->dRanks = c.take<long long>(n);
  ctx->dPcaOut = c.take<double>(3 * d + d * d);
  ctx->dDataMean = ctx->dPcaOut; ctx->dPcaMean = ctx->dPcaOut + d; ctx->dEvr = ctx->dPcaOut + 2 * d;
  ctx->dComps = ctx->dPcaOut + 3 * d;
  ctx->dIn = c.take<double>(n * (2 * d + 2));
  ctx->dC = c.take<double>(D * D);        ctx->dGbuf[0] = c.take<double>(d * d); ctx->dGbuf[1] = c.take<double>(d * d);
  ctx->dG = ctx->dGbuf[0];
  ctx->dLam = c.take<double>(d);          ctx->dZ = c.take<double>(n * d);
  ctx->dK = c.take<int>(1);               ctx->dSweeps = c.take<int>(1);         ctx->dInfo = c.take<int>(1);
  ctx->dY = c.take<double>(n);            ctx->dYs = c.take<double>(N);
  ctx->dYstats = c.take<double>(2);       ctx->dBounds4 = c.take<double>(4 * PCABO_MAXD);
  ctx->dZnMean = c.take<double>(PCABO_MAXD); ctx->dUserNB = c.take<double>(2 * PCABO_MAXD);
  ctx->dZnT = c.take<double>((size_t)ctx->KPcap * N); ctx->dAT = c.take<double>((size_t)ctx->KPcap * N);
  ctx->dNrm = c.take<double>(N);
  ctx->dGram = c.take<double>(N * N);     ctx->dL = c.take<double>(N * N);       ctx->dR = c.take<double>(N * N);
  ctx->dTmp = c.take<double>(N);          ctx->dAlpha = c.take<double>(N);
  ctx->dDiag = c.take<double>((size_t)2 * PCABO_BS * PCABO_BS);
  ctx->dXq = c.take<double>(Q * d + 8);
  ctx->dPartial = c.take<double>(Q * (size_t)ctx->Scap * (2 + 2 * PCABO_MAXD));
  ctx->dVal = c.take<double>(Q);          ctx->dGrad = c.take<double>(Q * d);
  ctx->dZq = c.take<double>(d);           ctx->dXout = c.take<double>(d);
  ctx->dBestF = c.take<double>(2);
  ctx->dKS = c.take<double>(Q * N);
  ctx->dCounters = c.take<unsigned int>(PCABO_CNT_DONE + 1);
  const size_t nb = N / PCABO_BS;
  ctx->dMll = c.take<double>(nb * (nb + 1) + 8);
  ctx->dHyp = c.take<double>(PCABO_HYP_WORDS);
  return (c.off + 4095) & ~(size_t)4095;
}
static size_t carve_host(pcabo_ctx* ctx, char* base) {
  Carver c{base};
  const size_t n = ctx->max_n, d = ctx->max_d, Q = ctx->max_q;
  ctx->hm = c.take<HostMirror>(1);
  ctx->hXq = c.take<double>(std::max<size_t>(Q * d, PCABO_QA_MAX) + 8);
  ctx->hVal = c.take<double>(Q);
  ctx->hGrad = c.take<double>(Q * d);
  ctx->hSmall = c.take<double>(d * d + 8 * d + 64);
  ctx->hIn = c.take<double>(n * (2 * d + 2));
  ctx->hBestF = c.take<double>(2);
  ctx->hMll = c.take<double>(8);
  ctx->hHyp = c.take<double>(PCABO_HYP_WORDS);
  return (c.off + 4095) & ~(size_t)4095;
}

static int ctx_setup(pcabo_ctx* ctx, int device, int max_n, int max_d, int max_q, char* dreg, char* hreg,
                     hipStream_t stream) {
  ctx->device = device;
  ctx->max_n = max_n; ctx->max_d = max_d; ctx->max_q = max_q;
  ctx->NPcap = round_up(max_n, PCABO_BS);
  ctx->ld = ctx->NPcap;
  ctx->DPcap = round_up(max_d, 16);
  ctx->KPcap = round_up(max_d, 4);
  ctx->Scap = ctx->NPcap / PCABO_SLAB;
  ctx->in_batch = dreg != nullptr;
  HIPCHK(hipSetDevice(device));
  if (stream) ctx->stream = stream;
  else HIPCHK(hipStreamCreateWithFlags(&ctx->stream, hipStreamNonBlocking));
  presence_register(ctx->device); ctx->registered = true;
  HIPCHK(hipEventCreateWithFlags(&ctx->evBounds, hipEventDisableTiming));
  HIPCHK(hipEventCreateWithFlags(&ctx->evPca, hipEventDisableTiming));
  ctx->region_bytes = carve_device(ctx, nullptr);
  ctx->hregion_bytes = carve_host(ctx, nullptr);
  if (dreg) {
    ctx->dRegion = dreg; ctx->hRegion = hreg;
  } else {
    HIPCHK(hipMalloc((void**)&ctx->dRegion, ctx->region_bytes));
    HIPCHK(hipHostMalloc((void**)&ctx->hRegion, ctx->hregion_bytes, hipHostMallocDefault));
    memset(ctx->hRegion, 0, ctx->hregion_bytes);
  }
  carve_device(ctx, ctx->dRegion);
  carve_host(ctx, ctx->hRegion);
  if (!dreg) {
    HIPCHK(hipMemsetAsync(ctx->dRegion, 0, ctx->region_bytes, ctx->stream));
    if (hipExtMallocWithFlags((void**)&ctx->dMail, PCABO_MAIL_PAIRS * sizeof(MailPair), hipDeviceMallocFinegrained) != hipSuccess) {
      (void)hipGetLastError();
      HIPCHK(dalloc(&ctx->dMail, PCABO_MAIL_PAIRS));
    }
    HIPCHK(hipMemsetAsync(ctx->dMail, 0, PCABO_MAIL_PAIRS * sizeof(MailPair), ctx->stream));
    const size_t np = (size_t)PCABO_INLAUNCH_MAXQ * 32 * (2 + 2 * PCABO_MAXD);
    HIPCHK(dalloc(&ctx->dPairs, np));
    HIPCHK(hipMemsetAsync(ctx->dPairs, 0, np * sizeof(MailPair), ctx->stream));
    HIPCHK(hipStreamSynchronize(ctx->stream));
    ctx->mail_bar = mail_bar_usable(ctx);
  } else {
    ctx->opt_resident = false;
  }
  {
    static std::atomic<unsigned long long> ctx_counter{0};
    ctx->seq = ((unsigned long long)(getpid() & 0xffff) << 44) + ((ctx_counter.fetch_add(1) + 1) << 30);
  }
  return PCABO_OK;
}

static void ctx_teardown(pcabo_ctx* ctx) {
  (void)hipSetDevice(ctx->device);
  if (ctx->stream) (void)hipStreamSynchronize(ctx->stream);
  for (auto& p : ctx->pairs) { (void)hipEventDestroy(p.a); (void)hipEventDestroy(p.b); }
  if (!ctx->in_batch) {
    if (ctx->dRegion) (void)hipFree(ctx->dRegion);
    if (ctx->hRegion) (void)hipHostFree(ctx->hRegion);
    if (ctx->dMail) (void)hipFree(ctx->dMail);
    if (ctx->dPairs) (void)hipFree(ctx->dPairs);
  }
  if (ctx->evBounds) (void)hipEventDestroy(ctx->evBounds);
  if (ctx->evPca) (void)hipEventDestroy(ctx->evPca);
  if (ctx->stream && !ctx->in_batch) (void)hipStreamDestroy(ctx->stream);
  ctx->helper.shutdown();
  for (auto& h : ctx->more_helpers) h->shutdown();
  ctx->more_helpers.clear();
  if (ctx->registered) presence_unregister(ctx->device);
}

static bool ctx_sizes_ok(int max_n, int max_d, int max_q) {
  return max_n >= 2 && max_d >= 1 && max_d <= PCABO_MAXD && max_q >= 1 && max_q < PCABO_CNT_DONE;
}

struct RowsDH {
  const double *Z, *y, *unb;
  int n, k, KP; const int* k_dev;
  double inv_ls, noise, mean_c; int kernel;
  ZB zb;
  hipEvent_t ev[2];
  int* cnt_S; bool* cnt_dirty;
};
template <class Phase>
static int enqueue_factor(pcabo_ctx* ctx, hipStream_t s, int n, int NP, ZB zb, Phase&& phase) {
  if (const int rc = phase(2)) return rc;
  if (launch_cholesky(s, ctx->dL, NP, ctx->ld, ctx->dInfo, ctx->dDiag, zb) != 0)
    return set_err(ctx, PCABO_ERR_HIP, "the Cholesky launches could not be set up (device or kernel attribute)%s", "");
  if (const int rc = phase(3)) return rc;
  launch_trinv(s, ctx->dL, NP, ctx->ld, ctx->dR, zb);
  launch_alpha(s, ctx->dR, ctx->dYs, n, NP, ctx->ld, ctx->dTmp, ctx->dAlpha, zb);
  if (const int rc = phase(4)) return rc;
  if (zb.zs) HIPCHK(hipMemcpy2DAsync((void*)&ctx->hm->chol_info, zb.hzs, ctx->dInfo, zb.zs, sizeof(int), zb.B, hipMemcpyDeviceToHost, s));
  else HIPCHK(hipMemcpyAsync((void*)&ctx->hm->chol_info, ctx->dInfo, sizeof(int), hipMemcpyDeviceToHost, s));
  return PCABO_OK;
}
template <class Phase>
static int enqueue_rows_dh(pcabo_ctx* ctx, hipStream_t s, const RowsDH& a, Phase&& phase) {
  const int NP = round_up(a.n, PCABO_BS);
  if (a.cnt_S && (acq_slabs(NP) != *a.cnt_S || *a.cnt_dirty)) {
    if (a.zb.zs) HIPCHK(hipMemset2DAsync(ctx->dCounters, a.zb.zs, 0, (PCABO_CNT_DONE + 1) * sizeof(unsigned int), a.zb.B, s));
    else HIPCHK(hipMemsetAsync(ctx->dCounters, 0, (PCABO_CNT_DONE + 1) * sizeof(unsigned int), s));
    *a.cnt_S = acq_slabs(NP); *a.cnt_dirty = false;
  }
  if (const int rc = phase(1)) return rc;
  launch_zstats(s, a.Z, a.y, a.n, a.k, a.unb, ctx->dBounds4, ctx->dZnMean, ctx->dYstats, ctx->dYs, ctx->hm, a.k_dev, a.zb, a.mean_c);
  for (hipEvent_t e : a.ev) if (e) HIPCHK(hipEventRecord(e, s));
  launch_znorm(s, a.Z, a.n, a.k, NP, a.KP, ctx->ld, ctx->dBounds4, ctx->dZnMean, a.inv_ls, ctx->dZnT, ctx->dAT, ctx->dNrm, a.k_dev, a.zb);
  launch_gram(s, ctx->dAT, ctx->dNrm, a.n, NP, a.KP, ctx->ld, a.noise, a.kernel, nullptr, a.k_dev, ctx->dL, ctx->dInfo, a.zb);
  return enqueue_factor(ctx, s, a.n, NP, a.zb, phase);
}

struct CondProf {
  pcabo_ctx* c; int kk;
  std::optional<ProfScope> ps;
  int operator()(int phase) {
    const double n = c->n;
    ps.reset();
    if (phase == 1) ps.emplace(c, 1, 8.0 * n * kk + 4.0 * n * (n + 1.0), 2.0 * n * n * kk + 12.0 * n * n);
    if (phase == 2) ps.emplace(c, 2, 16.0 * n * n, n * n * n / 3.0);
    if (phase == 3) ps.emplace(c, 3, 16.0 * n * n, n * n * n / 3.0 + 2.0 * n * n);
    return PCABO_OK;
  }
};

static int launch_factorisation(pcabo_ctx* ctx, double jitter) {
  hipStream_t s = ctx->stream;
  if (jitter > 0.0) {
    launch_gram(s, ctx->dAT, ctx->dNrm, ctx->n, ctx->NP, round_up(ctx->k, 4), ctx->ld, ctx->noise, ctx->kernel, nullptr, nullptr,
                ctx->dL, ctx->dInfo);
    launch_add_jitter(s, ctx->dL, ctx->n, ctx->ld, jitter);
  }
  return enqueue_factor(ctx, s, ctx->n, ctx->NP, ZB(), CondProf{ctx, 0});
}

template <class Extra>
static int factor_attempts(pcabo_ctx* ctx, int attempt, Extra&& extra) {
  double jitter = 1e-8;
  for (int a = 2; a <= attempt; ++a) jitter *= 10.0;
  for (;; ++attempt) {
    if (attempt > 0) {
      const int rc = launch_factorisation(ctx, jitter);
      if (rc != PCABO_OK) return rc;
      jitter *= 10.0;
    }
    const int rc = extra();
    if (rc != PCABO_OK) return rc;
    HIPCHK(wait_stream(ctx->stream));
    HIPCHK(hipGetLastError());
    if (ctx->hm->chol_info == 0) return PCABO_OK;
    if (attempt == 3)
      return set_err(ctx, PCABO_ERR_NOT_PD, "K + s2 I not positive definite after jitter retries (pivot %s%d)", "", ctx->hm->chol_info);
  }
// ... 341 lines not shown
static AcqParams make_params(pcabo_ctx* ctx, double best_f, int maximize, int acq, int want_grad) {
  AcqParams p;
  p.best_f = ctx->bestf_f32 ? (double)(float)best_f : best_f;
  p.y_mean = 0.0; p.y_std = 1.0;
  p.inv_ls = 1.0 / ctx->lengthscale;
  p.maximize = maximize ? 1 : 0;
  p.acq = acq;
  p.kernel = ctx->kernel;
  p.want_grad = want_grad;
  return p;
}

static int acq_published(pcabo_ctx* ctx, FlagWait w) {
  if (w == FLAGS_UNPUBLISHED) {
    HIPCHK(hipGetLastError());
    return set_err(ctx, PCABO_ERR_TIMEOUT, "acquisition kernel finished without publishing its results%s", "");
  }
  if (w == FLAGS_LATE) return set_err(ctx, PCABO_ERR_TIMEOUT, "device did not publish acquisition results%s", "");
  return PCABO_OK;
}

static int eval_staged(pcabo_ctx* ctx, int nq, AcqParams& p, bool allow_gemm = true) {
  hipStream_t s = ctx->stream;
  const int k = ctx->k;
  const unsigned long long seq = ++ctx->seq;
  const QueryArgs* qa = nullptr;
  const double* xdev = nullptr;
  if ((size_t)nq * k <= PCABO_QA_MAX) {
    qa = reinterpret_cast<const QueryArgs*>(ctx->hXq);
  } else {
    HIPCHK(hipMemcpyAsync(ctx->dXq, ctx->hXq, (size_t)nq * k * sizeof(double), hipMemcpyHostToDevice, s));
    xdev = ctx->dXq;
  }
  const bool small = nq <= PCABO_INLAUNCH_MAXQ;
  if (!small && !p.want_grad && allow_gemm && score_gemm_possible(nq)) {
    if (!xdev) {
      HIPCHK(hipMemcpyAsync(ctx->dXq, ctx->hXq, (size_t)nq * k * sizeof(double), hipMemcpyHostToDevice, s));
      xdev = ctx->dXq;
    }
    ProfScope ps(ctx, 5, acq_bytes(ctx->n, k, nq, 0), acq_flops(ctx->n, k, nq, 0));
    launch_score(s, xdev, nq, ctx->n, k, ctx->NP, ctx->ld, ctx->dZnT, ctx->dR, ctx->dAlpha, ctx->dBounds4, ctx->dYstats, p,
                 ctx->dKS, ctx->dPartial, ctx->dVal);
  } else {
    ProfScope ps(ctx, small ? 4 : 5, acq_bytes(ctx->n, k, nq, p.want_grad), acq_flops(ctx->n, k, nq, p.want_grad));
    launch_acq(s, qa, xdev, nq, ctx->n, k, ctx->NP, ctx->ld, ctx->dZnT, ctx->dR, ctx->dAlpha, ctx->dBounds4, ctx->dYstats,
               p, ctx->dPartial, ctx->dCounters, ctx->dVal, ctx->dGrad, small ? ctx->hVal : nullptr,
               small ? ctx->hGrad : nullptr, small ? ctx->hm : nullptr, seq);
  }
  if (!small) {
    HIPCHK(hipMemcpyAsync(ctx->hVal, ctx->dVal, (size_t)nq * sizeof(double), hipMemcpyDeviceToHost, s));
    if (p.want_grad) HIPCHK(hipMemcpyAsync(ctx->hGrad, ctx->dGrad, (size_t)nq * k * sizeof(double), hipMemcpyDeviceToHost, s));
    HIPCHK(wait_stream(s));
    HIPCHK(hipGetLastError());
    return PCABO_OK;
  }
  return acq_published(ctx, wait_flags(ctx->hm, 0, nq, seq, deadline_in(20), &s));
}

static int eval_staged_groups(pcabo_ctx* ctx, const int* g0, const int* gn, int ng, AcqParams& p) {
  hipStream_t s = ctx->stream;
  const unsigned long long seq = ++ctx->seq;
  QueryArgs tab;
  unsigned* ent = reinterpret_cast<unsigned*>(tab.x);
  for (int g = 0; g < ng; ++g) ent[g] = ((unsigned)g0[g] << 8) | (unsigned)gn[g];
  {
    int nq = 0;
    for (int g = 0; g < ng; ++g) nq += gn[g];
    ProfScope ps(ctx, 4, acq_bytes(ctx->n, ctx->k, nq, p.want_grad), acq_flops(ctx->n, ctx->k, nq, p.want_grad));
    if (launch_acq_group(s, &tab, ng, ctx->hXq, ctx->n, ctx->k, ctx->NP, ctx->ld, ctx->dZnT, ctx->dR, ctx->dAlpha, ctx->dBounds4,
                         ctx->dYstats, p, ctx->dPartial, ctx->dCounters + PCABO_GROUP_CNT_OFFSET, ctx->dVal, ctx->dGrad, ctx->hVal,
                         ctx->hGrad, ctx->hm, seq, AcqBatch()) != 0)
      return set_err(ctx, PCABO_ERR_HIP, "the restart-group acquisition kernel could not be launched%s", "");
  }
  HIPCHK(hipGetLastError());
  const auto deadline = deadline_in(20);
  FlagWait w = FLAGS_SET;
  for (int g = 0; g < ng && w == FLAGS_SET; ++g) w = wait_flags(ctx->hm, g0[g], gn[g], seq, deadline, &s);
  return acq_published(ctx, w);
}
static bool group_mode(const pcabo_ctx* ctx, int q, int want_grad) {
  return ctx->opt_group_acq && want_grad && q <= PCABO_INLAUNCH_MAXQ && acq_group_possible(ctx->NP, ctx->k);
}

int pcabo_acq_eval(pcabo_ctx* ctx, const double* Xq, int q, double best_f, int maximize, int acq, double* val,
                   double* grad) {
  if (!ctx) return PCABO_ERR_ARG;
  if (!Xq || !val || q < 1 || q > ctx->max_q || (acq != PCABO_ACQ_LOG_EI && acq != PCABO_ACQ_PI))
    return set_err(ctx, PCABO_ERR_ARG, "pcabo_acq_eval: bad argument or q beyond context capacity%s", "");
  if (!ctx->have_gp) return set_err(ctx, PCABO_ERR_ARG, "pcabo_acq_eval: call pcabo_gp_condition first%s", "");
  HIPCHK(hipSetDevice(ctx->device));
  hipStream_t s = ctx->stream;
  const int k = ctx->k;
  const size_t nx = (size_t)q * k;
  if (ctx->ptr_mode == PCABO_PTR_HOST) memcpy(ctx->hXq, Xq, nx * sizeof(double));
  else {
    HIPCHK(hipMemcpyAsync(ctx->hXq, Xq, nx * sizeof(double), hipMemcpyDeviceToHost, s));
    HIPCHK(hipStreamSynchronize(s));
  }
  AcqParams p = make_params(ctx, best_f, maximize, acq, grad ? 1 : 0);
  int rc;
  if (group_mode(ctx, q, grad != nullptr) && ctx->ptr_mode == PCABO_PTR_HOST) {
    int g0[(PCABO_INLAUNCH_MAXQ + PCABO_GROUP_Q - 1) / PCABO_GROUP_Q], gn[(PCABO_INLAUNCH_MAXQ + PCABO_GROUP_Q - 1) / PCABO_GROUP_Q], ng = 0;
    for (int a = 0; a < q; a += PCABO_GROUP_Q) { g0[ng] = a; gn[ng] = std::min(PCABO_GROUP_Q, q - a); ++ng; }
    rc = eval_staged_groups(ctx, g0, gn, ng, p);
  } else {
    rc = eval_staged(ctx, q, p);
  }
  if (rc != PCABO_OK) return rc;
  if (ctx->ptr_mode == PCABO_PTR_HOST) {
    memcpy(val, ctx->hVal, (size_t)q * sizeof(double));
    if (grad) memcpy(grad, ctx->hGrad, nx * sizeof(double));
  } else {
    HIPCHK(hipMemcpyAsync(val, ctx->dVal, (size_t)q * sizeof(double), hipMemcpyDeviceToDevice, s));
    if (grad) HIPCHK(hipMemcpyAsync(grad, ctx->dGrad, nx * sizeof(double), hipMemcpyDeviceToDevice, s));
    HIPCHK(hipStreamSynchronize(s));
  }
  return PCABO_OK;
}

int pcabo_gp_condition_end_eval(pcabo_ctx* ctx, const double* Xq, int q, double best_f, int maximize, int acq,
                                double* val) {
  if (!ctx) return PCABO_ERR_ARG;
  if (!Xq || !val || q < 1 || q > ctx->max_q || (acq != PCABO_ACQ_LOG_EI && acq != PCABO_ACQ_PI))
    return set_err(ctx, PCABO_ERR_ARG, "pcabo_gp_condition_end_eval: bad argument or q beyond context capacity%s", "");
  if (!ctx->gp_pending) return set_err(ctx, PCABO_ERR_ARG, "pcabo_gp_condition_end_eval: no conditioning in flight%s", "");
  if (ctx->wpca_uncollected) { int rc0 = pcabo_wpca_results(ctx, nullptr, nullptr, nullptr, nullptr, nullptr); if (rc0 != PCABO_OK) return rc0; }
  if (q <= PCABO_INLAUNCH_MAXQ || ctx->ptr_mode != PCABO_PTR_HOST) {
    int rc = pcabo_gp_condition_end(ctx);
    if (rc != PCABO_OK) return rc;
    return pcabo_acq_eval(ctx, Xq, q, best_f, maximize, acq, val, nullptr);
  }
  HIPCHK(hipSetDevice(ctx->device));
  memcpy(ctx->hXq, Xq, (size_t)q * ctx->k * sizeof(double));
  AcqParams p = make_params(ctx, best_f, maximize, acq, 0);
  int rc = eval_staged(ctx, q, p);
  if (rc != PCABO_OK) { ctx->gp_pending = false; return rc; }
  if (ctx->hm->chol_info != 0) {
    rc = pcabo_gp_condition_end(ctx);
    if (rc != PCABO_OK) return rc;
    rc = eval_staged(ctx, q, p);
    if (rc != PCABO_OK) return rc;
  } else {
    ctx->gp_pending = false;
    ctx->have_gp = true;
  }
  memcpy(val, ctx->hVal, (size_t)q * sizeof(double));
  return PCABO_OK;
}

int pcabo_logei(pcabo_ctx* ctx, const double* Xq, int q, double best_f, int maximize, double* val, double* grad) {
  return pcabo_acq_eval(ctx, Xq, q, best_f, maximize, PCABO_ACQ_LOG_EI, val, grad);
}

static void server_post(pcabo_ctx* ctx, int cap, int nq, int k, unsigned long long tag) {
  MailPair* m = ctx->dMail;
  const int np = cap * k;
  for (int i = 0; i < np; ++i) put_mail_pair(m + 1 + i, ctx->hXq[i], tag);
  for (int q = 0; q < cap; ++q) put_mail_pair(m + 1 + np + q, q < nq ? 1.0 : 0.0, tag);
  _mm_sfence();
}
static int server_wait(pcabo_ctx* ctx, int nq, unsigned long long tag) {
  if (wait_flags(ctx->hm, 0, nq, tag, deadline_in(3)) != FLAGS_SET)
    return set_err(ctx, PCABO_ERR_TIMEOUT, "resident acquisition kernel did not answer%s", "");
  return PCABO_OK;
}

int pcabo_optimize_acqf(pcabo_ctx* ctx, const double* ics, int num_restarts, int batch_limit, const double* bounds,
                        int maxiter, double best_f, int maximize, int acq, double* cand, double* vals, int* info,
                        int* failed) {
  if (!ctx) return PCABO_ERR_ARG;
  if (!ics || !bounds || !cand || !vals || num_restarts < 1 || batch_limit < 1 || num_restarts > ctx->max_q ||
      (acq != PCABO_ACQ_LOG_EI && acq != PCABO_ACQ_PI))
    return set_err(ctx, PCABO_ERR_ARG, "pcabo_optimize_acqf: bad argument%s", "");
  if (!ctx->have_gp) return set_err(ctx, PCABO_ERR_ARG, "pcabo_optimize_acqf: call pcabo_gp_condition first%s", "");
  HIPCHK(hipSetDevice(ctx->device));
  const int k = ctx->k;
  RunRestarts run;
  run.init(ics, bounds, num_restarts, batch_limit, k, maxiter);
  std::vector<RestartGroup>& grp = run.grp;
  const int ngroups = (int)grp.size();
  AcqParams p = make_params(ctx, best_f, maximize, acq, 1);
  auto now = [] { return std::chrono::duration<double>(std::chrono::steady_clock::now().time_since_epoch()).count(); };
  std::vector<char> pending(ngroups, 0);
  auto advance = [&](int gi) {
    if (pending[gi]) pending[gi] = 0;
    else grp[gi].advance();
  };
  OptHelper& hp = ctx->helper;
  const int T = ngroups >= 12 ? std::min(7, 1 + ngroups / 8) : 2;
  if (T > 2) while ((int)ctx->more_helpers.size() < T - 2) ctx->more_helpers.emplace_back(new OptHelper());
  std::vector<OptHelper*> hs;
  if (ngroups > 1) hs.push_back(&hp);
  for (int i = 0; i < T - 2; ++i) hs.push_back(ctx->more_helpers[i].get());
  for (size_t i = 0; i < hs.size(); ++i) {
    const int first = (int)i + 1;
    hs[i]->begin([&, first] { for (int gi = first; gi < ngroups; gi += T) advance(gi); });
  }
  struct Ender { std::vector<OptHelper*>& h; ~Ender() { for (OptHelper* x : h) x->end(); } } ender{hs};
  unsigned round_no = 0;
  std::vector<int> qoff(ngroups, -1);
  int srv_cap = 0;
  struct ServerStop {
    pcabo_ctx* c; int& cap; int k;
    void stop() {
      if (cap <= 0) return;
      server_post(c, cap, 0, k, ++c->seq);
      (void)hipStreamSynchronize(c->stream);
      cap = 0;
    }
    ~ServerStop() { stop(); }
  } server_stop{ctx, srv_cap, k};
  while (true) {
    ++round_no;
    unsigned tickets[8] = {0};
    for (size_t i = 0; i < hs.size(); ++i) {
      tickets[i] = hs[i]->go.load(std::memory_order_relaxed) + 1;
      hs[i]->go.store(tickets[i], std::memory_order_release);
    }
    for (int gi = 0; gi < ngroups; gi += T) advance(gi);
    for (size_t i = 0; i < hs.size(); ++i)
      while (hs[i]->done.load(std::memory_order_acquire) != tickets[i]) __builtin_ia32_pause();
    int nq = 0;
    for (int gi = 0; gi < ngroups; ++gi) {
      qoff[gi] = -1;
      if (!grp[gi].active) continue;
      qoff[gi] = nq;
      memcpy(ctx->hXq + (size_t)nq * k, grp[gi].x.data(), grp[gi].x.size() * sizeof(double));
      nq += grp[gi].nq;
    }
    if (nq == 0) break;
    int rc;
    if (round_no == 1 && (ctx->alone_age++ & 7) == 0) ctx->alone = presence_alone(ctx->device);
    const bool only_context_here = presence_local_contexts(ctx->device) == 1;
    if (round_no == 1 && ctx->srv_penalty > 0) --ctx->srv_penalty;
    else if (round_no == 1 && ctx->opt_resident && ctx->mail_bar && !ctx->opt_group_acq && ctx->alone && only_context_here && !ctx->prof && acq_server_possible(nq, ctx->n, k, ctx->NP)) {
      srv_cap = nq;
      launch_acq(ctx->stream, nullptr, nullptr, srv_cap, ctx->n, k, ctx->NP, ctx->ld, ctx->dZnT, ctx->dR, ctx->dAlpha,
                 ctx->dBounds4, ctx->dYstats, p, ctx->dPartial, ctx->dCounters, ctx->dVal, ctx->dGrad, ctx->hVal, ctx->hGrad,
                 ctx->hm, ctx->seq + 1, ctx->dMail, ctx->dPairs);
      HIPCHK(hipGetLastError());
      if (ngroups == 2 && grp[0].active && grp[1].active && nq == num_restarts) {
        const unsigned long long seq0 = ctx->seq;
        MailPair* m = ctx->dMail;
        const int cap = srv_cap;
        std::atomic<int> abort_flag{0};
        int timed_out[2] = {0, 0}, got_nan[2] = {0, 0}, left[2] = {0, 0}, slow_first[2] = {0, 0};
        unsigned long long used[2] = {0, 0};
        auto free_loop = [&](int gi) {
          RestartGroup& rg = grp[gi];
          const int q0 = rg.q0, nqg = rg.nq;
          unsigned long long r = 0;
          for (;;) {
            if (abort_flag.load(std::memory_order_relaxed)) { pending[gi] = 1; break; }
            const unsigned long long tag = seq0 + (++r);
            for (int t = 0; t < nqg * k; ++t) put_mail_pair(m + 1 + q0 * k + t, rg.x[t], tag);
            for (int j = 0; j < nqg; ++j) put_mail_pair(m + 1 + cap * k + q0 + j, 1.0, tag);
            _mm_sfence();
            const auto t0 = std::chrono::steady_clock::now();
            unsigned long spins = 0;
            bool ok = true;
            for (int j = 0; j < nqg && ok; ++j) {
              while (__atomic_load_n(&ctx->hm->qflag[q0 + j], __ATOMIC_ACQUIRE) != tag) {
                if ((++spins & 0xFFF) == 0) {
                  if (abort_flag.load(std::memory_order_relaxed)) { ok = false; break; }
                  if (std::chrono::steady_clock::now() - t0 > std::chrono::seconds(3)) {
                    timed_out[gi] = 1; abort_flag.store(1, std::memory_order_relaxed); ok = false; break;
                  }
                }
              }
            }
            if (!ok) { pending[gi] = 1; break; }
            if (r == 1 && std::chrono::steady_clock::now() - t0 > std::chrono::milliseconds(1)) slow_first[gi] = 1;
            if (!rg.absorb(ctx->hVal, ctx->hGrad, q0)) { got_nan[gi] = 1; abort_flag.store(1, std::memory_order_relaxed); break; }
            if (!rg.advance()) break;
          }
          const unsigned long long bye = seq0 + r + 1;
          for (int j = 0; j < nqg; ++j) put_mail_pair(m + 1 + cap * k + q0 + j, 0.0, bye);
          _mm_sfence();
          left[gi] = 1;
          used[gi] = r + 1;
        };
        hp.fn = [&] { free_loop(1); };
        const unsigned fticket = hp.go.load(std::memory_order_relaxed) + 1;
        hp.go.store(fticket, std::memory_order_release);
        free_loop(0);
        while (hp.done.load(std::memory_order_acquire) != fticket) __builtin_ia32_pause();
        hp.fn = [&] { for (int gi = 1; gi < ngroups; gi += T) advance(gi); };
        HIPCHK(hipStreamSynchronize(ctx->stream));
        ctx->seq = seq0 + std::max(used[0], used[1]) + 1;
        srv_cap = 0;
        if (got_nan[0] || got_nan[1]) return set_err(ctx, PCABO_ERR_NAN, "NaN in acquisition gradient%s", "");
        if (timed_out[0] || timed_out[1]) ctx->srv_penalty = 1000;
        else if (slow_first[0] || slow_first[1]) ctx->srv_penalty = 40;
        if (!grp[0].active && !grp[1].active) break;
        continue;
      }
    }
    if (srv_cap > 0) {
      const unsigned long long tag = ++ctx->seq;
      const double tp = now();
      server_post(ctx, srv_cap, nq, k, tag);
      rc = server_wait(ctx, nq, tag);
      if (rc == PCABO_ERR_TIMEOUT) {
        server_stop.stop();
        ctx->srv_penalty = 1000;
        rc = eval_staged(ctx, nq, p);
      } else if (round_no == 1 && now() - tp > 1e-3) {
        ctx->srv_penalty = 40;
      }
    } else if (group_mode(ctx, nq, 1) && batch_limit <= PCABO_GROUP_Q && ngroups <= 8) {
      int g0[8], gn[8], ng = 0;
      for (int gi = 0; gi < ngroups; ++gi) if (qoff[gi] >= 0) { g0[ng] = qoff[gi]; gn[ng] = grp[gi].nq; ++ng; }
      rc = eval_staged_groups(ctx, g0, gn, ng, p);
    } else {
      rc = eval_staged(ctx, nq, p);
    }
    if (rc != PCABO_OK) return rc;
    for (int gi = 0; gi < ngroups; ++gi)
      if (qoff[gi] >= 0 && !grp[gi].absorb(ctx->hVal, ctx->hGrad, qoff[gi]))
        return set_err(ctx, PCABO_ERR_NAN, "NaN in acquisition gradient%s", "");
  }
  server_stop.stop();
  const bool redo = run.end_points(cand, vals) > 0;
  const bool any_failed = run.report(info, 0);
  if (redo) {
    AcqParams pv = make_params(ctx, best_f, maximize, acq, 0);
    memcpy(ctx->hXq, cand, (size_t)num_restarts * k * sizeof(double));
    int rc = eval_staged(ctx, num_restarts, pv, false);
    if (rc != PCABO_OK) return rc;
    for (int j = 0; j < num_restarts; ++j) vals[j] = ctx->hVal[j];
  }
  if (failed) *failed = any_failed;
  return PCABO_OK;
}

int pcabo_inverse_map(pcabo_ctx* ctx, const double* z, double* x) {
  if (!ctx || !z || !x) return PCABO_ERR_ARG;
  if (!ctx->have_wpca) return set_err(ctx, PCABO_ERR_ARG, "pcabo_inverse_map: call pcabo_wpca first%s", "");
  HIPCHK(hipSetDevice(ctx->device));
  hipStream_t s = ctx->stream;
  memcpy(ctx->hXq, z, (size_t)ctx->k * sizeof(double));
  const unsigned long long seq = ++ctx->seq;
  double* hx = ctx->hSmall + (size_t)ctx->max_d * ctx->max_d + 3 * (size_t)ctx->max_d;
  launch_inverse_map(s, ctx->hXq, ctx->dComps, ctx->dDataMean, ctx->dPcaMean, ctx->k, ctx->d, ctx->dXout, nullptr, ZB(),
                     hx, ctx->hm, seq);
  HIPCHK(hipGetLastError());
  const FlagWait w = wait_flags(ctx->hm, 0, 1, seq, deadline_in(20), &s);
  if (w == FLAGS_UNPUBLISHED) {
    HIPCHK(hipGetLastError());
    return set_err(ctx, PCABO_ERR_TIMEOUT, "inverse-map kernel finished without publishing its result%s", "");
  }
  if (w == FLAGS_LATE) return set_err(ctx, PCABO_ERR_TIMEOUT, "device did not publish the inverse map%s", "");
  memcpy(x, hx, (size_t)ctx->d * sizeof(double));
  return PCABO_OK;
}

int pcabo_get_gp_state(pcabo_ctx* ctx, double* K_chol, double* Rinv, double* alpha, double* y_mean_std,
                       double* norm_bounds) {
  if (!ctx) return PCABO_ERR_ARG;
  if (!ctx->have_gp) return set_err(ctx, PCABO_ERR_ARG, "pcabo_get_gp_state: call pcabo_gp_condition first%s", "");
  HIPCHK(hipSetDevice(ctx->device));
  hipStream_t s = ctx->stream;
  const size_t n = ctx->n, w = n * sizeof(double), pitch = (size_t)ctx->ld * sizeof(double);
  if (K_chol) HIPCHK(hipMemcpy2DAsync(K_chol, w, ctx->dL, pitch, w, n, hipMemcpyDeviceToHost, s));
  if (Rinv) HIPCHK(hipMemcpy2DAsync(Rinv, w, ctx->dR, pitch, w, n, hipMemcpyDeviceToHost, s));
  if (alpha) HOST_OUT(alpha, ctx->dAlpha, n, double);
  HIPCHK(hipStreamSynchronize(s));
  if (y_mean_std) { y_mean_std[0] = ctx->hm->y_mean; y_mean_std[1] = ctx->hm->y_std; }
  if (norm_bounds)
    for (int c = 0; c < ctx->k; ++c) { norm_bounds[c] = ctx->hm->norm_lo[c]; norm_bounds[ctx->k + c] = ctx->hm->norm_hi[c]; }
  return PCABO_OK;
}

int pcabo_get_gram(pcabo_ctx* ctx, double* K) {
  if (!ctx || !K) return PCABO_ERR_ARG;
  if (!ctx->have_gp) return set_err(ctx, PCABO_ERR_ARG, "pcabo_get_gram: call pcabo_gp_condition first%s", "");
  HIPCHK(hipSetDevice(ctx->device));
  const size_t n = ctx->n, w = n * sizeof(double), pitch = (size_t)ctx->ld * sizeof(double);
  ctx->rt_stale = true;
  launch_gram(ctx->stream, ctx->dAT, ctx->dNrm, ctx->n, ctx->NP, round_up(ctx->k, 4), ctx->ld, ctx->noise, ctx->kernel, ctx->dGram,
              nullptr, nullptr, nullptr);
  HIPCHK(hipMemcpy2DAsync(K, w, ctx->dGram, pitch, w, n, hipMemcpyDeviceToHost, ctx->stream));
  HIPCHK(hipStreamSynchronize(ctx->stream));
  for (size_t i = 0; i < n; ++i)
    for (size_t j = i + 1; j < n; ++j) K[i * n + j] = K[j * n + i];
  return PCABO_OK;
}


int pcabo_set_profiling(pcabo_ctx* ctx, int enabled) {
  if (!ctx) return PCABO_ERR_ARG;
  HIPCHK(hipSetDevice(ctx->device));
  if (enabled && ctx->pairs.empty()) {
    ctx->pairs.resize(PROF_POOL);
    for (auto& p : ctx->pairs) { HIPCHK(hipEventCreate(&p.a)); HIPCHK(hipEventCreate(&p.b)); p.group = 0; }
  }
  if (!enabled) prof_resolve(ctx);
  if (enabled && !ctx->prof) {
    prof_resolve(ctx);
    double med[2] = {0.0, 0.0};
    for (int mode = 0; mode < 2; ++mode) {
      std::vector<float> r;
      for (int i = 0; i < 64; ++i) {
        HIPCHK(hipEventRecord(ctx->pairs[i].a, ctx->stream));
        if (mode == 1) hipLaunchKernelGGL(k_nop, dim3(1), dim3(64), 0, ctx->stream);
        HIPCHK(hipEventRecord(ctx->pairs[i].b, ctx->stream));
      }
      HIPCHK(hipStreamSynchronize(ctx->stream));
      for (int i = 0; i < 64; ++i) { float ms = 0.f; if (hipEventElapsedTime(&ms, ctx->pairs[i].a, ctx->pairs[i].b) == hipSuccess) r.push_back(ms); }
      if (!r.empty()) { std::sort(r.begin(), r.end()); med[mode] = r[r.size() / 2]; }
    }
    ctx->prof_pair_ms = med[0];
    ctx->prof_empty_ms = med[1];
  }
  ctx->prof = enabled != 0;
  return PCABO_OK;
}

int pcabo_get_profile_calibration(pcabo_ctx* ctx, double* pair_ms, double* empty_kernel_ms) {
  if (!ctx) return PCABO_ERR_ARG;
  if (pair_ms) *pair_ms = ctx->prof_pair_ms;
  if (empty_kernel_ms) *empty_kernel_ms = ctx->prof_empty_ms;
  return PCABO_OK;
}

int pcabo_get_profile(pcabo_ctx* ctx, int which, double* ms, int64_t* launches, double* bytes, double* flops) {
  if (!ctx || which < 0 || which >= PROF_GROUPS) return PCABO_ERR_ARG;
  HIPCHK(hipSetDevice(ctx->device));
  prof_resolve(ctx);
  if (ms) *ms = ctx->prof_ms[which];
  if (launches) *launches = ctx->prof_launches[which];
  if (bytes) *bytes = ctx->prof_bytes[which];
  if (flops) *flops = ctx->prof_flops[which];
  return PCABO_OK;
}

int pcabo_reset_profile(pcabo_ctx* ctx) {
  if (!ctx) return PCABO_ERR_ARG;
  prof_resolve(ctx);
  for (int i = 0; i < PROF_GROUPS; ++i) { ctx->prof_ms[i] = 0.0; ctx->prof_launches[i] = 0; ctx->prof_bytes[i] = 0.0; ctx->prof_flops[i] = 0.0; }
  return PCABO_OK;
}


}


struct pcabo_batch {
  int device = 0, B = 0, max_n = 0, max_d = 0, max_q = 0;
  hipStream_t stream = nullptr;
  hipEvent_t evPca = nullptr, evBounds = nullptr;
  char *dSlab = nullptr, *hSlab = nullptr;
  size_t zs = 0, hzs = 0;
  std::vector<pcabo_ctx*> ctx;
  std::vector<char> active;
  int n = 0, d = 0, NP = 0;
  bool wpca_uncollected = false, gp_pending = false, have_gp = false;
  double lengthscale = 0.0, noise = 0.0;
  int kernel = 0;
  const double *fitZ = nullptr, *fitY = nullptr, *fitUnb = nullptr;
  bool fitted = false;
  int fit_rounds = 0;
  int gcur = 0, vprev_d = 0;
  int cnt_S = 0; bool cnt_dirty = true;
  bool prof = false; hipEvent_t pev[6] = {nullptr, nullptr, nullptr, nullptr, nullptr, nullptr};
  bool group_acq = true;
  size_t in_stride_x = 0, in_stride_noise = 0, in_stride_y = 0;
  bool score_enqueued = false;
  bool imap_enqueued = false;
  bool opt_enqueued = false; int opt_restarts = 0, opt_limit = 0; std::vector<int> opt_act;
  int dev_lbfgsb = 0;
  unsigned *dOptTab = nullptr, *hOptTab = nullptr;
  int opt_cus = 0;
  hipStream_t optStream = nullptr; int optStream_cus = 0;
  hipEvent_t evOptIn = nullptr, evOptOut = nullptr;
  int G = 0;
  std::vector<hipStream_t> gstream;
  GangPool pool;
  std::atomic<unsigned long long> seq{0};
  char err[512] = {0};
};

static int bset_err(pcabo_batch* b, int code, const char* fmt, const char* a = "", int v = 0) {
  if (b) snprintf(b->err, sizeof(b->err), fmt, a, v);
  return code;
}
#define BHIPCHK(call)                                                                        \
// ... 1030 lines not shown
```

para-ortho-pca-bo_amd/csrc/pcabo_internal.h:

```cpp
#pragma once
#include <hip/hip_runtime.h>
#include <stdint.h>
#include <type_traits>

#define PCABO_BS 64
#define PCABO_SLAB 16
#define PCABO_MAXD 128
#define PCABO_TLD 66

#define PCABO_QA_MAX 416
#define PCABO_CNT_DONE 0x3fff
#define PCABO_INLAUNCH_MAXQ 32

typedef double double4_t __attribute__((ext_vector_type(4)));
struct QueryArgs { double x[PCABO_QA_MAX]; };
struct alignas(16) MailPair { double v; unsigned long long tag; };
static inline __host__ __device__ unsigned long long mail_mix(unsigned long long vbits) {
  const unsigned int lo = (unsigned int)vbits, hi = (unsigned int)(vbits >> 32);
  return (unsigned long long)((lo ^ hi ^ (hi >> 11)) & 0xFFFFFFu);
}
#define PCABO_MAIL_PAIRS (1 + PCABO_QA_MAX + PCABO_INLAUNCH_MAXQ + 1)
#define PCABO_SERVER_TIMEOUT_TICKS 200000000ull

#ifdef __HIPCC__
__device__ inline double fast_rcp(double x) {
  double r = __builtin_amdgcn_rcp(x);
  r = fma(fma(-x, r, 1.0), r, r);
  r = fma(fma(-x, r, 1.0), r, r);
  return r;
}
__device__ inline double fast_rsq(double x) {
  double y = __builtin_amdgcn_rsq(x);
  y = y * fma(-0.5 * x * y, y, 1.5);
  y = y * fma(-0.5 * x * y, y, 1.5);
  return y;
}
#endif

static inline int round_up(int x, int m) { return (x + m - 1) / m * m; }

struct AcqParams {
  double best_f;
  double y_mean, y_std;
  double inv_ls;
  int maximize;
  int acq;
  int kernel;
  int want_grad;
};

struct AcqBatch {
  size_t zs = 0, hzs = 0;
  const int* k_dev = nullptr;
  const double* bestf = nullptr;
  int table = 0;
  int xq_host = 0;
  const double* hyp = nullptr;
};

struct HostMirror {
  int k;
  int chol_info;
  int pad0, pad1;
  double y_mean, y_std;
  double norm_lo[PCABO_MAXD], norm_hi[PCABO_MAXD];
  double acq_lo[PCABO_MAXD], acq_hi[PCABO_MAXD];
  volatile unsigned long long qflag[PCABO_INLAUNCH_MAXQ];
};

#if defined(__HIPCC__)
typedef unsigned int pcabo_u4 __attribute__((ext_vector_type(4)));
__device__ inline pcabo_u4 ld_pair_sys(const void* p) {
  pcabo_u4 r;
  asm volatile("global_load_dwordx4 %0, %1, off sc0 sc1\n\ts_waitcnt vmcnt(0)" : "=v"(r) : "v"(p) : "memory");
  return r;
}
__device__ inline void st_pair_sys(void* p, pcabo_u4 v) {
  asm volatile("global_store_dwordx4 %0, %1, off sc0 sc1" : : "v"(p), "v"(v) : "memory");
}
__device__ inline void ld_pairs_sys8(const void* const* p, pcabo_u4* o) {
  asm volatile(
      "global_load_dwordx4 %0, %8, off sc0 sc1\n\tglobal_load_dwordx4 %1, %9, off sc0 sc1\n\t"
      "global_load_dwordx4 %2, %10, off sc0 sc1\n\tglobal_load_dwordx4 %3, %11, off sc0 sc1\n\t"
      "global_load_dwordx4 %4, %12, off sc0 sc1\n\tglobal_load_dwordx4 %5, %13, off sc0 sc1\n\t"
      "global_load_dwordx4 %6, %14, off sc0 sc1\n\tglobal_load_dwordx4 %7, %15, off sc0 sc1\n\t"
      "s_waitcnt vmcnt(0)"
      : "=&v"(o[0]), "=&v"(o[1]), "=&v"(o[2]), "=&v"(o[3]), "=&v"(o[4]), "=&v"(o[5]), "=&v"(o[6]), "=&v"(o[7])
      : "v"(p[0]), "v"(p[1]), "v"(p[2]), "v"(p[3]), "v"(p[4]), "v"(p[5]), "v"(p[6]), "v"(p[7])
      : "memory");
}
__device__ inline pcabo_u4 make_pair(double v, unsigned long long tag) {
  pcabo_u4 r;
  r.x = (unsigned int)__double2loint(v); r.y = (unsigned int)__double2hiint(v);
  r.z = (unsigned int)(tag & 0xffffffffull); r.w = (unsigned int)(tag >> 32);
  return r;
}
__device__ inline unsigned long long pair_tag(pcabo_u4 v) { return ((unsigned long long)v.w << 32) | v.z; }
__device__ inline double pair_value(pcabo_u4 v) { return __hiloint2double((int)v.y, (int)v.x); }
__device__ inline unsigned long long mail_seq(pcabo_u4 v) {
  return pair_tag(v) ^ mail_mix(((unsigned long long)v.y << 32) | v.x);
}

template <typename T>
__device__ inline T* zrun(T* p, size_t stride, unsigned run) {
  typedef typename std::remove_const<T>::type U;
  return p ? reinterpret_cast<T*>(reinterpret_cast<char*>(const_cast<U*>(p)) + (size_t)run * stride) : p;
}
#define ZRUN(p) p = zrun(p, zs, blockIdx.z)

struct XcdTile { unsigned run, x, y; };
#if defined(__HIPCC__)
__device__ inline XcdTile xcd_tile() {
  const unsigned gx = gridDim.x, gy = gridDim.y, T = gx * gy;
  const unsigned lin = (blockIdx.z * gy + blockIdx.y) * gx + blockIdx.x, full = (gridDim.z & ~7u) * T;
  XcdTile t;
  if (lin < full) {
    const unsigned slot = lin >> 3, tile = slot % T;
    t.run = (slot / T) * 8u + (lin & 7u); t.x = tile % gx; t.y = tile / gx;
  } else { t.run = blockIdx.z; t.x = blockIdx.x; t.y = blockIdx.y; }
  return t;
}
#endif
#define ZRUNX(p) p = zrun(p, zs, xt_.run)

template <int CTRL, int ROW_MASK>
__device__ inline double dpp_get(double v) {
  int lo = __builtin_amdgcn_update_dpp(0, __double2loint(v), CTRL, ROW_MASK, 0xf, false);
  int hi = __builtin_amdgcn_update_dpp(0, __double2hiint(v), CTRL, ROW_MASK, 0xf, false);
  return __hiloint2double(hi, lo);
}
__device__ inline double row_sum16(double v) {
  v += dpp_get<0xB1, 0xf>(v);
  v += dpp_get<0x4E, 0xf>(v);
  v += dpp_get<0x141, 0xf>(v);
  v += dpp_get<0x140, 0xf>(v);
  return v;
}
__device__ inline double wave_sum(double v) {
  v = row_sum16(v);
  v += dpp_get<0x142, 0xa>(v);
  v += dpp_get<0x143, 0xc>(v);
  return __hiloint2double(__builtin_amdgcn_readlane(__double2hiint(v), 63),
                          __builtin_amdgcn_readlane(__double2loint(v), 63));
}

template <int T>
__device__ inline double lane_xor(double v) {
  if (T == 0) return dpp_get<0xB1, 0xf>(v);
  if (T == 1) return dpp_get<0x4E, 0xf>(v);
  if (T == 2) return dpp_get<0x141, 0xf>(dpp_get<0x1B, 0xf>(v));
  return dpp_get<0x128, 0xf>(v);
}
template <int T>
__device__ inline double swap_add(double a, double b) {
  unsigned alo = (unsigned)__double2loint(a), ahi = (unsigned)__double2hiint(a);
  unsigned blo = (unsigned)__double2loint(b), bhi = (unsigned)__double2hiint(b);
  if (T == 4) {
    const auto lo = __builtin_amdgcn_permlane16_swap(alo, blo, false, false);
    const auto hi = __builtin_amdgcn_permlane16_swap(ahi, bhi, false, false);
    alo = lo[0]; blo = lo[1]; ahi = hi[0]; bhi = hi[1];
  } else {
    const auto lo = __builtin_amdgcn_permlane32_swap(alo, blo, false, false);
    const auto hi = __builtin_amdgcn_permlane32_swap(ahi, bhi, false, false);
    alo = lo[0]; blo = lo[1]; ahi = hi[0]; bhi = hi[1];
  }
  return __hiloint2double((int)ahi, (int)alo) + __hiloint2double((int)bhi, (int)blo);
}
template <int T>
__device__ inline double pair_level(double a, double b, int lane) {
  if (T >= 4) return swap_add<T>(a, b);
  const bool hi = (lane >> T) & 1;
  return (hi ? b : a) + lane_xor<T>(hi ? a : b);
}
template <int T>
__device__ inline double single_level(double v) {
  if (T >= 4) return swap_add<T>(v, v);
  return v + lane_xor<T>(v);
}
__host__ __device__ constexpr int wave_multi_live(int n, int t) { return (n + (1 << t) - 1) >> t; }
template <int T, int N>
__device__ inline void wave_multi_level(double* v, int lane) {
  constexpr int M = wave_multi_live(N, T);
#pragma unroll
  for (int i = 0; i < M / 2; ++i) v[i] = pair_level<T>(v[2 * i], v[2 * i + 1], lane);
  if (M & 1) v[M / 2] = single_level<T>(v[M - 1]);
}
template <int N>
__device__ inline void wave_sum_multi(double* v, int lane) {
  static_assert(N >= 1 && N <= 64, "one value per lane at the end");
  wave_multi_level<0, N>(v, lane); wave_multi_level<1, N>(v, lane); wave_multi_level<2, N>(v, lane);
  wave_multi_level<3, N>(v, lane); wave_multi_level<4, N>(v, lane); wave_multi_level<5, N>(v, lane);
}
template <int N>
__device__ inline int wave_multi_index(int lane) {
  int slot = 0;
#pragma unroll
  for (int t = 5; t >= 0; --t) {
    const int m = wave_multi_live(N, t);
    slot = slot < m / 2 ? 2 * slot + ((lane >> t) & 1) : m - 1;
  }
  return slot;
}
template <int N>
__device__ inline int wave_multi_owner(int lane) {
  int slot = 0;
  bool first = true;
#pragma unroll
  for (int t = 5; t >= 0; --t) {
    const int m = wave_multi_live(N, t);
    if (slot < m / 2) slot = 2 * slot + ((lane >> t) & 1);
    else { slot = m - 1; first = first && !((lane >> t) & 1); }
  }
  return first ? slot : -1;
}
__host__ __device__ constexpr int wave_multi_lane(int n, int i, int t = 0) {
  return t == 6 ? 0
       : (i < wave_multi_live(n, t) / 2 * 2 ? ((i & 1) << t) + wave_multi_lane(n, i / 2, t + 1)
                                            : wave_multi_lane(n, wave_multi_live(n, t) / 2, t + 1));
}
__device__ inline double read_lane(double v, int lane) {
  return __hiloint2double(__builtin_amdgcn_readlane(__double2hiint(v), lane),
                          __builtin_amdgcn_readlane(__double2loint(v), lane));
}
#endif

void launch_rank(hipStream_t s, const double* f, int n, int maximize, long long* ranks);
#define PCABO_HYP_INV_LS 0
#define PCABO_HYP_NOISE 1
#define PCABO_HYP_MEAN_C 2
#define PCABO_HYP_WORDS 4
struct ZB { int B = 1; size_t zs = 0, hzs = 0; const double* hyp = nullptr; };
void launch_wpca_prep(hipStream_t s, const double* X, const long long* ranks, const double* noise, int n, int d,
                      int DP, double* weights, double* data_mean, double* pca_mean, double* Wc, ZB zb = ZB());
void launch_cov(hipStream_t s, const double* Wc, int n, int DP, double* C, ZB zb = ZB());
void launch_jacobi(hipStream_t s, const double* C, int d, int DP, const double* V0, double* G, double* lam, int* sweeps,
                   int n, double var_threshold, int n_components, double* comps, double* evr, int* k_dev, HostMirror* hm,
                   ZB zb = ZB());
void launch_project(hipStream_t s, const double* X, const double* data_mean, const double* pca_mean,
                    const double* comps, const int* k_dev, int n, int d, double* Z, ZB zb = ZB());
void launch_zstats(hipStream_t s, const double* Z, const double* y, int n, int k, const double* user_norm_bounds,
                   double* bounds4 , double* zn_mean, double* ystats,
                   double* ys, HostMirror* hm, const int* k_dev = nullptr, ZB zb = ZB(),
                   double mean_c = 0.0);
void launch_znorm(hipStream_t s, const double* Z, int n, int k, int NP, int KP, int ld, const double* bounds4,
                  const double* zn_mean, double inv_ls, double* ZnT, double* AT, double* nrm,
                  const int* k_dev = nullptr, ZB zb = ZB());
void launch_gram(hipStream_t s, const double* AT, const double* nrm, int n, int NP, int KP, int ld, double noise,
                 int kernel, double* K, const int* k_dev = nullptr, double* K2 = nullptr, int* info_reset = nullptr,
                 ZB zb = ZB());
void launch_add_jitter(hipStream_t s, double* K, int n, int ld, double jitter);
int launch_cholesky(hipStream_t s, double* L, int NP, int ld, int* info, double* diag_scratch, ZB zb = ZB());
void launch_trinv(hipStream_t s, const double* L, int NP, int ld, double* R, ZB zb = ZB());
void launch_chol_panel(hipStream_t s, double* L, int p, int nblocks, int ld, int* info, double* diag_scratch, ZB zb = ZB());
int launch_chol_steps(hipStream_t s, double* L, int NP, int ld, int* info, double* diag_scratch , ZB zb = ZB());
void launch_trinv_diag_w(hipStream_t s, const double* L, int nblk, int ld, double* R, ZB zb = ZB());
void launch_alpha(hipStream_t s, const double* R, const double* ys, int n, int NP, int ld, double* tmp, double* alpha,
                  ZB zb = ZB());
void launch_mll_grad(hipStream_t s, const double* R, const double* AT, const double* nrm, const double* alpha, const double* L,
                     const double* ys, int n, int NP, int KP, int ld, double* partial, double* out,
                     const int* k_dev = nullptr, ZB zb = ZB());
void launch_acq(hipStream_t s, const QueryArgs* qa, const double* Xq, int q, int n, int k, int NP, int ld,
                const double* ZnT, const double* R, const double* alpha, const double* bounds4, const double* ystats,
                AcqParams p, double* partial, unsigned int* counters, double* val,
                double* grad, double* host_val, double* host_grad, HostMirror* hm, unsigned long long seq,
                MailPair* dev_mail = nullptr, MailPair* part_pairs = nullptr,
                AcqBatch ab = AcqBatch(), int B = 1, int table_entries = 0);
#define PCABO_GROUP_Q 5
#define PCABO_GROUP_CNT_OFFSET 8192
bool acq_group_possible(int NP, int k);
int launch_acq_group(hipStream_t st, const QueryArgs* tab, int entries, const double* Xq, int n, int k, int NP, int ld,
                     const double* ZnT, const double* R, const double* alpha, const double* bounds4, const double* ystats,
                     AcqParams p, double* partial, unsigned int* counters, double* val, double* grad, double* host_val,
                     double* host_grad, HostMirror* hm, unsigned long long seq, AcqBatch ab);
bool score_gemm_possible(int q);
void launch_score(hipStream_t st, const double* Xq, int q, int n, int k, int NP, int ld, const double* ZnT, const double* R,
                  const double* alpha, const double* bounds4, const double* ystats, AcqParams p, double* KS, double* partial,
                  double* val, AcqBatch ab = AcqBatch(), int B = 1);
bool acq_server_possible(int q, int n, int k, int NP);
int acq_slabs(int NP);
void launch_inverse_map(hipStream_t s, const double* z, const double* comps, const double* data_mean,
                        const double* pca_mean, int k, int d, double* x, const int* k_dev = nullptr, ZB zb = ZB(),
                        double* host_x = nullptr, HostMirror* hm = nullptr, unsigned long long seq = 0);
void launch_rt_build(hipStream_t s, const double* R, int n, int NP, int ld, double* RT, ZB zb = ZB());
bool lbfgsb_device_possible(int NP, int kmax, int batch_limit);
int launch_lbfgsb_group(hipStream_t st, const unsigned* table, int entries, int mode, int num_restarts, int maxiter, int n, int NP,
                        int ld, const double* Xq, const double* ZnT, const double* R, const double* RT, const double* alpha,
                        const double* bounds4, const double* ystats, const double* bestf, const int* k_dev, double inv_ls,
                        int maximize, int acq, int kernel, double* out_x, double* out_v, size_t zs,
                        const double* hyp = nullptr);
```

Measured before the change: 371.8 BO iterations/s.

## Return resident-server acquisition results as self-tagged mail pairs in host memory

The resident acquisition server now writes each value and gradient component as a 16-byte pair whose tag combines the sequence number with a mix of the value bits. The host polls these pairs directly instead of waiting on per-query flags and then reading separate value and gradient buffers. This removes the separate flag store and its release ordering, and lets the host accept each element as soon as its own pair is valid. It depends on 128-bit loads being atomic on the host and on the tag check catching torn writes, and it adds optional timing instrumentation plus a self-test for the pair protocol.

Result: faster. 386.3 BO iterations/s (median of 4 runs) (+3.9%).

```diff
diff --git a/para-ortho-pca-bo_amd/csrc/host_selftest.cpp b/para-ortho-pca-bo_amd/csrc/host_selftest.cpp
--- a/para-ortho-pca-bo_amd/csrc/host_selftest.cpp
+++ b/para-ortho-pca-bo_amd/csrc/host_selftest.cpp
@@ -8,6 +8,7 @@
 #include <cstdio>
 #include <cstdlib>
 #include <cstring>
+#include <numeric>
 #include <vector>
 
 namespace {
@@ -483,6 +484,111 @@
   }
 }
 
+struct PairArea {
+  std::vector<MailPair> store;
+  MailPair* p;
+  explicit PairArea(size_t n) : store(n + 4) {
+    p = reinterpret_cast<MailPair*>(((uintptr_t)store.data() + 63) & ~(uintptr_t)63);
+    for (size_t i = 0; i < n; ++i) { put_half(i, 0, 0); put_half(i, 1, 0); }
+  }
+  void put_half(size_t i, int half, unsigned long long bits) {
+    __atomic_store_n(half == 0 ? reinterpret_cast<unsigned long long*>(&p[i].v) : &p[i].tag, bits, __ATOMIC_RELAXED);
+  }
+};
+unsigned long long dbits(double v) { unsigned long long b; std::memcpy(&b, &v, 8); return b; }
+double pair_value_of(int q, int i, unsigned long long r) { return (1.0 + 0.001 * (double)(r & 0xff)) * (1 + q) + 0.03125 * i - (i == 2 ? 7.5 : 0.0); }
+void write_pair(PairArea& a, size_t idx, double v, unsigned long long seq, int tag_first) {
+  const unsigned long long vb = dbits(v), tag = seq ^ mail_mix(vb);
+  a.put_half(idx, tag_first ? 1 : 0, tag_first ? tag : vb);
+  a.put_half(idx, tag_first ? 0 : 1, tag_first ? vb : tag);
+}
+
+void test_result_pairs() {
+  using namespace std::chrono;
+  const unsigned long long base = (0x2a5ull << 44) + (3ull << 30);
+  const nanoseconds brief = milliseconds(2);
+  {
+    const int k = 2;
+    PairArea a(PCABO_RES_STRIDE(k));
+    double hv[1] = {-1.0}, hg[2] = {-1.0, -1.0};
+    const unsigned long long seq = base + 7;
+    CHECK(wait_result_pairs(a.p, 0, 1, k, seq, hv, hg, nullptr, nullptr, brief) == PAIRS_LATE, "zeroed area answered");
+    write_pair(a, 0, 5e-324, seq - 1, 0);
+    CHECK(a.p[0].tag == seq, "the adversarial tag is not the raw sequence number");
+    write_pair(a, 1, 0.25, seq - 1, 0); write_pair(a, 2, -3.0, seq - 1, 0);
+    CHECK(wait_result_pairs(a.p, 0, 1, k, seq, hv, hg, nullptr, nullptr, brief) == PAIRS_LATE, "pairs of the previous round taken");
+    CHECK(wait_result_pairs(a.p, 0, 1, k, seq - 1, hv, hg, nullptr, nullptr, brief) == PAIRS_OK && hv[0] == 5e-324 && hg[0] == 0.25 && hg[1] == -3.0,
+          "the previous round itself not read back");
+    for (int idx = 0; idx <= k; ++idx)
+      for (int tear = 0; tear < 2; ++tear) {
+        const double oldv[3] = {5e-324, 0.25, -3.0}, newv[3] = {1.5, -0.125, 6.0};
+        for (int i = 0; i <= k; ++i) write_pair(a, i, newv[i], seq, 0);
+        if (tear == 0) { a.put_half(idx, 0, dbits(newv[idx])); a.put_half(idx, 1, (seq - 1) ^ mail_mix(dbits(oldv[idx]))); }
+        else { a.put_half(idx, 0, dbits(oldv[idx])); a.put_half(idx, 1, seq ^ mail_mix(dbits(newv[idx]))); }
+        CHECK(wait_result_pairs(a.p, 0, 1, k, seq, hv, hg, nullptr, nullptr, brief) == PAIRS_LATE, "torn pair %d (way %d) taken", idx, tear);
+        write_pair(a, idx, newv[idx], seq, tear);
+        CHECK(wait_result_pairs(a.p, 0, 1, k, seq, hv, hg, nullptr, nullptr, brief) == PAIRS_OK && hv[0] == 1.5 && hg[0] == -0.125 && hg[1] == 6.0,
+              "mended pair %d not taken", idx);
+      }
+    for (int miss = 0; miss <= k; ++miss) {
+      for (int i = 0; i <= k; ++i) write_pair(a, i, pair_value_of(0, i, seq + 1), i == miss ? seq : seq + 1, 0);
+      const auto t0 = steady_clock::now();
+      CHECK(wait_result_pairs(a.p, 0, 1, k, seq + 1, hv, hg, nullptr, nullptr, milliseconds(20)) == PAIRS_LATE, "answer without pair %d", miss);
+      const auto dt = steady_clock::now() - t0;
+      CHECK(dt >= milliseconds(20) && dt < seconds(2), "timeout after %lld us", (long long)duration_cast<microseconds>(dt).count());
+    }
+    std::atomic<int> abort_flag{1};
+    CHECK(wait_result_pairs(a.p, 0, 1, k, seq + 2, hv, hg, &abort_flag, nullptr, seconds(3)) == PAIRS_ABORTED, "abort flag ignored");
+  }
+  for (int k : {1, 3, 40}) {
+    const int nq_all = 5, q0 = 2, nq = 3, stride = PCABO_RES_STRIDE(k), per = 1 + k, total = nq * per;
+    PairArea a((size_t)nq_all * stride);
+    std::atomic<unsigned long long> posted{0}, taken{0};
+    const unsigned long long rounds = 150;
+    std::thread writer([&] {
+      const int steps[] = {1, 2, 3, 5, 7, 11, 13, 17, 41, 43};
+      for (unsigned long long r = 1; r <= rounds; ++r) {
+        while (posted.load(std::memory_order_acquire) != r) std::this_thread::yield();
+        int step = steps[r % 10];
+        while (std::gcd(step, total) != 1) ++step;
+        const bool reverse = (r / 10) % 2 == 1;
+        for (int t = 0; t < total; ++t) {
+          int j = (int)((r + (unsigned long long)t * step) % total);
+          if (reverse) j = total - 1 - j;
+          const int q = q0 + j / per, i = j % per;
+          const size_t idx = (size_t)q * stride + i;
+          const unsigned long long vb = dbits(pair_value_of(q, i, r)), tag = (base + r) ^ mail_mix(vb);
+          const int tag_first = (int)((r + t) & 1);
+          a.put_half(idx, tag_first, tag_first ? tag : vb);
+          if ((r + t) % 17 == 0) std::this_thread::sleep_for(microseconds(50));
+          a.put_half(idx, !tag_first, tag_first ? vb : tag);
+        }
+        while (taken.load(std::memory_order_acquire) != r) std::this_thread::yield();
+      }
+    });
+    std::vector<double> hv(nq_all, 0.0), hg((size_t)nq_all * k, 0.0);
+    int bad = 0, late = 0, same_mix = 0;
+    for (unsigned long long r = 1; r <= rounds; ++r)
+      for (int q = q0; q < q0 + nq; ++q)
+        for (int i = 0; i < per; ++i) same_mix += mail_mix(dbits(pair_value_of(q, i, r))) == mail_mix(dbits(pair_value_of(q, i, r - 1)));
+    CHECK(same_mix == 0, "k = %d: %d test values keep their mix from one round to the next", k, same_mix);
+    for (unsigned long long r = 1; r <= rounds; ++r) {
+      posted.store(r, std::memory_order_release);
+      const PairWait w = wait_result_pairs(a.p, q0, nq, k, base + r, hv.data(), hg.data(), nullptr, nullptr, seconds(20));
+      if (w != PAIRS_OK) ++late;
+      for (int q = q0; q < q0 + nq; ++q) {
+        if (hv[q] != pair_value_of(q, 0, r)) ++bad;
+        for (int c = 0; c < k; ++c) if (hg[(size_t)q * k + c] != pair_value_of(q, 1 + c, r)) ++bad;
+      }
+      taken.store(r, std::memory_order_release);
+    }
+    writer.join();
+    CHECK(late == 0, "k = %d: %d rounds timed out", k, late);
+    CHECK(bad == 0, "k = %d: %d values handed on that are not the round's", k, bad);
+    for (int q = 0; q < q0; ++q) CHECK(hv[q] == 0.0, "a query outside the group was written");
+  }
+}
+
 }
 
 int main(int argc, char** argv) {
@@ -494,6 +600,7 @@
   test_plan();
   test_restart_group();
   test_fit_run();
+  test_result_pairs();
   test_gang_pool(1, 3);
   test_gang_pool(workers, 11);
   if (g_fail) { std::fprintf(stderr, "host selftest: %d check(s) failed\n", g_fail); return 1; }
diff --git a/para-ortho-pca-bo_amd/csrc/host_side.h b/para-ortho-pca-bo_amd/csrc/host_side.h
--- a/para-ortho-pca-bo_amd/csrc/host_side.h
+++ b/para-ortho-pca-bo_amd/csrc/host_side.h
@@ -1,8 +1,11 @@
 #pragma once
 #include "../../include/pcabo.h"
 #include "lbfgsb.h"
+#include "mail_pair.h"
 
 #include <algorithm>
+#include <atomic>
+#include <chrono>
 #include <cmath>
 #include <condition_variable>
 #include <cstring>
@@ -11,6 +14,7 @@
 #include <thread>
 #include <utility>
 #include <vector>
+#include <emmintrin.h>
 
 struct RestartGroup : LbfgsbDriver {
   int q0 = 0, nq = 0, k = 0;
@@ -74,6 +78,42 @@
     return any;
   }
 };
+
+inline void load_pair(const MailPair* p, unsigned long long* vbits, unsigned long long* tag) {
+#if defined(__SANITIZE_THREAD__)
+  *vbits = __atomic_load_n(reinterpret_cast<const unsigned long long*>(&p->v), __ATOMIC_RELAXED);
+  *tag = __atomic_load_n(&p->tag, __ATOMIC_RELAXED);
+#else
+  const __m128i x = _mm_load_si128(reinterpret_cast<const __m128i*>(p));
+  *vbits = (unsigned long long)_mm_cvtsi128_si64(x);
+  *tag = (unsigned long long)_mm_cvtsi128_si64(_mm_unpackhi_epi64(x, x));
+  asm volatile("" ::: "memory");
+#endif
+}
+enum PairWait { PAIRS_OK = 0, PAIRS_ABORTED = 1, PAIRS_LATE = 2 };
+inline PairWait wait_result_pairs(const MailPair* res, int q0, int nq, int k, unsigned long long seq, double* hVal, double* hGrad,
+                                  const std::atomic<int>* abort_flag = nullptr, bool* slow_first = nullptr,
+                                  std::chrono::nanoseconds limit = std::chrono::seconds(3)) {
+  const auto t0 = std::chrono::steady_clock::now();
+  const int stride = PCABO_RES_STRIDE(k);
+  unsigned long spins = 0;
+  for (int q = q0 + nq - 1; q >= q0; --q) {
+    const MailPair* blk = res + (size_t)q * stride;
+    for (int i = k; i >= 0; --i) {
+      unsigned long long vb, tag;
+      for (;;) {
+        load_pair(blk + i, &vb, &tag);
+        if ((tag ^ mail_mix(vb)) == seq) break;
+        if ((++spins & 0xFFF) != 0) continue;
+        if (abort_flag && abort_flag->load(std::memory_order_relaxed)) return PAIRS_ABORTED;
+        if (std::chrono::steady_clock::now() - t0 > limit) return PAIRS_LATE;
+      }
+      std::memcpy(i == 0 ? hVal + q : hGrad + (size_t)q * k + (i - 1), &vb, sizeof(double));
+    }
+  }
+  if (slow_first) *slow_first = std::chrono::steady_clock::now() - t0 > std::chrono::milliseconds(1);
+  return PAIRS_OK;
+}
 
 inline unsigned group_entry(int run, int q0, int nq) { return ((unsigned)run << 16) | ((unsigned)q0 << 8) | (unsigned)nq; }
 inline unsigned query_entry(int run, int q) { return ((unsigned)run << 16) | (unsigned)q; }
diff --git a/para-ortho-pca-bo_amd/csrc/kernels_acq.hip b/para-ortho-pca-bo_amd/csrc/kernels_acq.hip
--- a/para-ortho-pca-bo_amd/csrc/kernels_acq.hip
+++ b/para-ortho-pca-bo_amd/csrc/kernels_acq.hip
@@ -12,9 +12,26 @@
 extern "C" int pcabo_debug_acq_stamps(unsigned long long* out16) {
   return hipMemcpyFromSymbol(out16, HIP_SYMBOL(g_acq_stamps), sizeof(g_acq_stamps)) == hipSuccess ? 0 : -3;
 }
+__device__ unsigned long long g_fin_timeline[8];
+#define FIN_TIMING_DOUBLES 6
+#define FIN_TS(s_srv, i) do { if ((threadIdx.x & 63) == 0) reinterpret_cast<unsigned long long*>((s_srv) + 2)[i] = wall_clock64(); } while (0)
+#define FIN_TS_ROUND(s_srv, q, t0) do { if ((q) == 0 && threadIdx.x == 0) {                                       \
+    const unsigned long long* ts_ = reinterpret_cast<const unsigned long long*>((s_srv) + 2);                     \
+    const unsigned long long g_ = ts_[2] > ts_[3] ? (ts_[2] > ts_[4] ? ts_[2] : ts_[4]) : (ts_[3] > ts_[4] ? ts_[3] : ts_[4]); \
+    g_fin_timeline[0] += 1; g_fin_timeline[1] += ts_[1] - ts_[0]; g_fin_timeline[2] += g_ - ts_[0];                \
+    g_fin_timeline[3] += ts_[5] - ts_[0]; g_fin_timeline[4] += ts_[0] - (t0); } } while (0)
+extern "C" int pcabo_debug_fin_timeline(unsigned long long* out8, int reset) {
+  static const unsigned long long zero[8] = {0};
+  if (out8 && hipMemcpyFromSymbol(out8, HIP_SYMBOL(g_fin_timeline), sizeof(g_fin_timeline)) != hipSuccess) return -3;
+  if (reset && hipMemcpyToSymbol(HIP_SYMBOL(g_fin_timeline), zero, sizeof(zero)) != hipSuccess) return -3;
+  return 0;
+}
 #else
 #define STAMP(i)
 #define STAMP_FIN(i)
+#define FIN_TIMING_DOUBLES 0
+#define FIN_TS(s_srv, i)
+#define FIN_TS_ROUND(s_srv, q, t0)
 #endif
 
 __device__ inline void st_wt(double* p, double v) {
@@ -62,7 +79,7 @@
 __device__ void acq_finish_scalar(const double* base, int S, int q, const double* ystats, const AcqParams& p, double* val,
                                   double* host_val, double* coef, int lane);
 __device__ void acq_scalar_core(double vv, double mus, int q, double ym, double ysd, const AcqParams& p, double* val,
-                                double* host_val, double* coef, int l);
+                                double* host_val, double* coef, int l, MailPair* res = nullptr, unsigned long long seq = 0);
 template <int SLAB>
 __device__ inline void acq_tail(int combine, double* s_v, double* partial, unsigned int* counters, int q, int S, int k,
                                 const double* bounds4, const double* ystats, const AcqParams& prm, double* val,
@@ -150,7 +167,7 @@
     const double* __restrict__ bounds4, const double* __restrict__ ystats, AcqParams prm, double* partial,
     unsigned int* counters, double* __restrict__ val, double* __restrict__ grad,
     double* host_val, double* host_grad, HostMirror* hm, unsigned long long seq, int combine, int ,
-    MailPair* , MailPair* , AcqBatch ab) {
+    MailPair* , MailPair* , AcqBatch ab, MailPair* ) {
   ACQ_BATCH_PROLOGUE()
   const double inv_ls = prm.inv_ls;
   const int kernel = prm.kernel, want_grad = prm.want_grad;
@@ -279,8 +296,7 @@
 
 #define FIN_STAGE_PER_WAVE (11 * 2 * 40)
 __device__ inline bool acq_server_finisher(const MailPair* rec, int S, int k, int q, unsigned long long seq,
-                                           const double* ystats, const AcqParams& prm, double* val, double* grad,
-                                           double* host_val, double* host_grad, HostMirror* hm, double rng_c,
+                                           const double* ystats, const AcqParams& prm, MailPair* res, double rng_c,
                                            double* s_fin, double* s_coef, double* s_stage, int* s_srv,
                                            unsigned long long t0, int w, int l) {
   if (w == 0) {
@@ -288,20 +304,22 @@
     const void* ptr[8];
     pcabo_u4 o[8];
     const MailPair* mine = rec + (size_t)(l < S ? l : 0) * PSTRIDE;
+    bool late = false;
 #pragma unroll
     for (int t = 0; t < 8; ++t) ptr[t] = mine + (t & 1);
     for (;;) {
       ld_pairs_sys8(ptr, o);
       const bool ok = pair_tag(o[0]) == seq && pair_tag(o[1]) == seq;
       if (__all(ok)) break;
-      if (__any(wall_clock64() - t0 > PCABO_SERVER_TIMEOUT_TICKS)) { if (l == 0) *s_srv = 1; break; }
+      if (__any(wall_clock64() - t0 > PCABO_SERVER_TIMEOUT_TICKS)) { if (l == 0) *s_srv = 1; late = true; break; }
       __builtin_amdgcn_s_sleep(1);
     }
+    FIN_TS(s_srv, 1);
     double vm[2] = {l < S ? pair_value(o[0]) : 0.0, l < S ? pair_value(o[1]) : 0.0};
     wave_sum_multi<2>(vm, l);
     constexpr int lane_vv = wave_multi_lane(2, 0), lane_mus = wave_multi_lane(2, 1);
     const double vv = read_lane(vm[0], lane_vv), mus = read_lane(vm[0], lane_mus);
-    acq_scalar_core(vv, mus, q, ym, ysd, prm, val, host_val, s_coef, l);
+    acq_scalar_core(vv, mus, q, ym, ysd, prm, nullptr, nullptr, s_coef, l, late ? nullptr : res, seq);
   } else if (prm.want_grad) {
     const int first = w - 1;
     const int ns = first < S ? (S - first + 2) / 3 : 0;
@@ -331,6 +349,7 @@
 #pragma unroll
       for (int t = 0; t < 8; ++t) if (item[t] >= 0) stage[item[t]] = pair_value(o[t]);
     }
+    FIN_TS(s_srv, 1 + w);
     __builtin_amdgcn_fence(__ATOMIC_RELEASE, "wavefront");
     __builtin_amdgcn_wave_barrier();
     __builtin_amdgcn_fence(__ATOMIC_ACQUIRE, "wavefront");
@@ -349,23 +368,21 @@
       const double gs = (s_fin[l] + s_fin[2 * PCABO_MAXD + l]) + s_fin[4 * PCABO_MAXD + l];
       const double gm = (s_fin[PCABO_MAXD + l] + s_fin[3 * PCABO_MAXD + l]) + s_fin[5 * PCABO_MAXD + l];
       const double g = __fma_rn(c_mu, gm, c_sg * gs) / rng_c;
-      grad[(size_t)q * k + l] = g;
-      if (host_grad) host_grad[(size_t)q * k + l] = g;
-    }
-    if (hm && l == 0)
-      __hip_atomic_store(const_cast<unsigned long long*>(&hm->qflag[q]), seq, __ATOMIC_RELEASE, __HIP_MEMORY_SCOPE_SYSTEM);
+      st_pair_sys(res + 1 + l, make_mail_pair(g, seq));
+    }
+    FIN_TS(s_srv, 5);
+    FIN_TS_ROUND(s_srv, q, t0);
   }
   return true;
 }
 
-#define FIN_LDS_DOUBLES (6 * PCABO_MAXD + 2 + 3 * FIN_STAGE_PER_WAVE + 2)
+#define FIN_LDS_DOUBLES (6 * PCABO_MAXD + 2 + 3 * FIN_STAGE_PER_WAVE + 2 + FIN_TIMING_DOUBLES)
 __device__ __noinline__ void acq_server_finish_main(double* s_mem, MailPair* dev_mail,
                                                     int ctrl_idx, const MailPair* part_pairs, int S, int k, int q,
                                                     const double* __restrict__ bounds4, const double* __restrict__ ystats,
-                                                    const AcqParams& prm, double* val, double* grad, double* host_val,
-                                                    double* host_grad, HostMirror* hm, unsigned long long seq) {
+                                                    const AcqParams& prm, MailPair* res, unsigned long long seq) {
   double* s_fin = s_mem;
-  int* s_srvp = reinterpret_cast<int*>(s_mem + FIN_LDS_DOUBLES - 1);
+  int* s_srvp = reinterpret_cast<int*>(s_mem + FIN_LDS_DOUBLES - FIN_TIMING_DOUBLES - 1);
   const int tid = threadIdx.x, l = tid & 63;
   const int w = __builtin_amdgcn_readfirstlane(tid >> 6);
   double rng_c = 1.0;
@@ -381,11 +398,12 @@
         if (__any(wall_clock64() - t0 > PCABO_SERVER_TIMEOUT_TICKS)) { if (l == 0) *s_srvp = 1; break; }
         __builtin_amdgcn_s_sleep(1);
       }
+      FIN_TS(s_srvp, 0);
     }
     __syncthreads();
     if (*s_srvp) return;
-    if (!acq_server_finisher(part_pairs + (size_t)q * S * PSTRIDE, S, k, q, cur_seq, ystats, prm, val, grad, host_val,
-                             host_grad, hm, rng_c, s_fin, s_fin + 6 * PCABO_MAXD, s_fin + 6 * PCABO_MAXD + 2, s_srvp, t0, w, l))
+    if (!acq_server_finisher(part_pairs + (size_t)q * S * PSTRIDE, S, k, q, cur_seq, ystats, prm, res, rng_c,
+                             s_fin, s_fin + 6 * PCABO_MAXD, s_fin + 6 * PCABO_MAXD + 2, s_srvp, t0, w, l))
       return;
     __syncthreads();
   }
@@ -418,7 +436,7 @@
     const double* __restrict__ bounds4, const double* __restrict__ ystats, AcqParams prm, double* partial,
     unsigned int* counters, double* __restrict__ val, double* __restrict__ grad,
     double* host_val, double* host_grad, HostMirror* hm, unsigned long long seq, int combine, int qb,
-    MailPair* dev_mail, MailPair* part_pairs, AcqBatch ab) {
+    MailPair* dev_mail, MailPair* part_pairs, AcqBatch ab, MailPair* res_pairs) {
   if (!SRV) { ACQ_BATCH_PROLOGUE() }
   constexpr int NP = NB * 64;
   constexpr int CU = 10;
@@ -439,7 +457,7 @@
   const int s = blockIdx.x, S = server ? (int)gridDim.x - 1 : (int)gridDim.x;
   if (server && s == S) {
     acq_server_finish_main(s_dyn, dev_mail, 1 + q_total * k + (int)blockIdx.y, part_pairs, S, k,
-                           blockIdx.y, bounds4, ystats, prm, val, grad, host_val, host_grad, hm, seq);
+                           blockIdx.y, bounds4, ystats, prm, res_pairs + (size_t)blockIdx.y * PCABO_RES_STRIDE(k), seq);
     return;
   }
   STAMP(0);
@@ -676,7 +694,7 @@
 }
 
 __device__ void acq_scalar_core(double vv, double mus, int q, double ym, double ysd, const AcqParams& p, double* val,
-                                double* host_val, double* coef, int l) {
+                                double* host_val, double* coef, int l, MailPair* res, unsigned long long seq) {
   const double mu = ym + ysd * mus;
   double var = (1.0 - vv) * (ysd * ysd);
   bool clamped = false;
@@ -699,7 +717,8 @@
     dv_dsig = 0.0;
   }
   if (l == 0) {
-    val[q] = value;
+    if (res) st_pair_sys(res, make_mail_pair(value, seq));
+    if (val) val[q] = value;
     if (host_val) host_val[q] = value;
     coef[0] = dv_du * sgn * ysd / sigma;
     coef[1] = clamped ? 0.0 : (dv_dsig - dv_du * u / sigma) * (-(ysd * ysd) / sigma);
@@ -1310,7 +1329,7 @@
                 AcqParams p, double* partial, unsigned int* counters, double* val,
                 double* grad, double* host_val, double* host_grad, HostMirror* hm, unsigned long long seq,
                 MailPair* dev_mail, MailPair* part_pairs, AcqBatch ab, int B,
-                int table_entries) {
+                int table_entries, MailPair* res_pairs) {
   const int slab = NP >= ACQ_SLAB32_NP ? 32 : 16;
   const int S = NP / slab;
   static const QueryArgs empty = {};
@@ -1321,7 +1340,7 @@
   const int gy = ab.table ? table_entries : (q + qb - 1) / qb;
   const int gz = ab.table ? 1 : B;
 #define ACQ_ARGS qa ? *qa : empty, Xq, q, n, k, NP, ld, ZnT, R, alpha, bounds4, ystats, p, partial, counters, val, grad, \
-                 host_val, host_grad, hm, seq, combine, qb, dev_mail, part_pairs, ab
+                 host_val, host_grad, hm, seq, combine, qb, dev_mail, part_pairs, ab, res_pairs
   const int FIN_LDS = 6 * PCABO_MAXD + 2;
 #define ACQ_LDS(SL, NBV) (3 * NBV * 64 + PCABO_MAXD + SL + 2 + (4 * NBV * 64 > FIN_LDS ? 4 * NBV * 64 : FIN_LDS))
 #define ACQ_FAST(SL, NBV)                                                                                      \
diff --git a/para-ortho-pca-bo_amd/csrc/mail_pair.h b/para-ortho-pca-bo_amd/csrc/mail_pair.h
--- /dev/null
+++ b/para-ortho-pca-bo_amd/csrc/mail_pair.h
@@ -0,0 +1,16 @@
+#pragma once
+
+#if defined(__HIPCC__)
+#define PCABO_HD __host__ __device__
+#else
+#define PCABO_HD
+#endif
+
+struct alignas(16) MailPair { double v; unsigned long long tag; };
+static inline PCABO_HD unsigned long long mail_mix(unsigned long long vbits) {
+  const unsigned int lo = (unsigned int)vbits, hi = (unsigned int)(vbits >> 32);
+  return (unsigned long long)((lo ^ hi ^ (hi >> 11)) & 0xFFFFFFu);
+}
+
+#define PCABO_RES_STRIDE(k) (((k) + 1 + 3) & ~3)
+#define PCABO_RES_MAXK 40
diff --git a/para-ortho-pca-bo_amd/csrc/pcabo_api.hip b/para-ortho-pca-bo_amd/csrc/pcabo_api.hip
--- a/para-ortho-pca-bo_amd/csrc/pcabo_api.hip
+++ b/para-ortho-pca-bo_amd/csrc/pcabo_api.hip
@@ -114,10 +114,15 @@
   MailPair* dMail = nullptr;
   bool mail_bar = false;
   MailPair* dPairs = nullptr;
+  MailPair* hRes = nullptr;
   bool opt_resident = true;
   bool opt_group_acq = false;
   bool bestf_f32 = true;
   int srv_penalty = 0;
+  unsigned long long res_rounds = 0;
+#ifdef PCABO_ACQ_TIMING
+  double tl[2][3] = {{0, 0, 0}, {0, 0, 0}};
+#endif
   unsigned long long seq = 0;
   OptHelper helper;
   std::vector<std::unique_ptr<OptHelper>> more_helpers;
@@ -371,6 +376,7 @@
   ctx->hBestF = c.take<double>(2);
   ctx->hMll = c.take<double>(8);
   ctx->hHyp = c.take<double>(PCABO_HYP_WORDS);
+  ctx->hRes = c.take<MailPair>(PCABO_RES_PAIRS);
   return (c.off + 4095) & ~(size_t)4095;
 }
 
@@ -1018,6 +1024,21 @@
   return pcabo_acq_eval(ctx, Xq, q, best_f, maximize, PCABO_ACQ_LOG_EI, val, grad);
 }
 
+#ifdef PCABO_ACQ_TIMING
+#define TL_BEGIN() double tl_ans_ = 0.0, tl_post_ = 0.0
+#define TL_POSTED(ctx, gi) do { tl_post_ = now(); if (tl_ans_ > 0.0) (ctx)->tl[gi][2] += tl_post_ - tl_ans_; } while (0)
+#define TL_ANSWERED(ctx, gi) do { tl_ans_ = now(); (ctx)->tl[gi][0] += 1.0; (ctx)->tl[gi][1] += tl_ans_ - tl_post_; } while (0)
+extern "C" int pcabo_debug_round_timeline(pcabo_ctx* ctx, double* out6, int reset) {
+  if (!ctx) return PCABO_ERR_ARG;
+  if (out6) memcpy(out6, ctx->tl, sizeof(ctx->tl));
+  if (reset) memset(ctx->tl, 0, sizeof(ctx->tl));
+  return PCABO_OK;
+}
+#else
+#define TL_BEGIN()
+#define TL_POSTED(ctx, gi)
+#define TL_ANSWERED(ctx, gi)
+#endif
 static void server_post(pcabo_ctx* ctx, int cap, int nq, int k, unsigned long long tag) {
   MailPair* m = ctx->dMail;
   const int np = cap * k;
@@ -1025,8 +1046,8 @@
   for (int q = 0; q < cap; ++q) put_mail_pair(m + 1 + np + q, q < nq ? 1.0 : 0.0, tag);
   _mm_sfence();
 }
-static int server_wait(pcabo_ctx* ctx, int nq, unsigned long long tag) {
-  if (wait_flags(ctx->hm, 0, nq, tag, deadline_in(3)) != FLAGS_SET)
+static int server_wait(pcabo_ctx* ctx, int nq, int k, unsigned long long tag) {
+  if (wait_result_pairs(ctx->hRes, 0, nq, k, tag, ctx->hVal, ctx->hGrad) != PAIRS_OK)
     return set_err(ctx, PCABO_ERR_TIMEOUT, "resident acquisition kernel did not answer%s", "");
   return PCABO_OK;
 }
@@ -1064,6 +1085,7 @@
   }
   struct Ender { std::vector<OptHelper*>& h; ~Ender() { for (OptHelper* x : h) x->end(); } } ender{hs};
   unsigned round_no = 0;
+  TL_BEGIN();
   std::vector<int> qoff(ngroups, -1);
   int srv_cap = 0;
   struct ServerStop {
@@ -1102,8 +1124,8 @@
     else if (round_no == 1 && ctx->opt_resident && ctx->mail_bar && !ctx->opt_group_acq && ctx->alone && only_context_here && !ctx->prof && acq_server_possible(nq, ctx->n, k, ctx->NP)) {
       srv_cap = nq;
       launch_acq(ctx->stream, nullptr, nullptr, srv_cap, ctx->n, k, ctx->NP, ctx->ld, ctx->dZnT, ctx->dR, ctx->dAlpha,
-                 ctx->dBounds4, ctx->dYstats, p, ctx->dPartial, ctx->dCounters, ctx->dVal, ctx->dGrad, ctx->hVal, ctx->hGrad,
-                 ctx->hm, ctx->seq + 1, ctx->dMail, ctx->dPairs);
+                 ctx->dBounds4, ctx->dYstats, p, ctx->dPartial, ctx->dCounters, nullptr, nullptr, nullptr, nullptr,
+                 ctx->hm, ctx->seq + 1, ctx->dMail, ctx->dPairs, AcqBatch(), 1, 0, ctx->hRes);
       HIPCHK(hipGetLastError());
       if (ngroups == 2 && grp[0].active && grp[1].active && nq == num_restarts) {
         const unsigned long long seq0 = ctx->seq;
@@ -1111,32 +1133,26 @@
         const int cap = srv_cap;
         std::atomic<int> abort_flag{0};
         int timed_out[2] = {0, 0}, got_nan[2] = {0, 0}, left[2] = {0, 0}, slow_first[2] = {0, 0};
-        unsigned long long used[2] = {0, 0};
+        unsigned long long used[2] = {0, 0}, answered[2] = {0, 0};
         auto free_loop = [&](int gi) {
           RestartGroup& rg = grp[gi];
           const int q0 = rg.q0, nqg = rg.nq;
           unsigned long long r = 0;
+          TL_BEGIN();
           for (;;) {
             if (abort_flag.load(std::memory_order_relaxed)) { pending[gi] = 1; break; }
             const unsigned long long tag = seq0 + (++r);
             for (int t = 0; t < nqg * k; ++t) put_mail_pair(m + 1 + q0 * k + t, rg.x[t], tag);
             for (int j = 0; j < nqg; ++j) put_mail_pair(m + 1 + cap * k + q0 + j, 1.0, tag);
             _mm_sfence();
-            const auto t0 = std::chrono::steady_clock::now();
-            unsigned long spins = 0;
-            bool ok = true;
-            for (int j = 0; j < nqg && ok; ++j) {
-              while (__atomic_load_n(&ctx->hm->qflag[q0 + j], __ATOMIC_ACQUIRE) != tag) {
-                if ((++spins & 0xFFF) == 0) {
-                  if (abort_flag.load(std::memory_order_relaxed)) { ok = false; break; }
-                  if (std::chrono::steady_clock::now() - t0 > std::chrono::seconds(3)) {
-                    timed_out[gi] = 1; abort_flag.store(1, std::memory_order_relaxed); ok = false; break;
-                  }
-                }
-              }
-            }
-            if (!ok) { pending[gi] = 1; break; }
-            if (r == 1 && std::chrono::steady_clock::now() - t0 > std::chrono::milliseconds(1)) slow_first[gi] = 1;
+            TL_POSTED(ctx, gi);
+            bool slow = false;
+            const PairWait pw = wait_result_pairs(ctx->hRes, q0, nqg, k, tag, ctx->hVal, ctx->hGrad, &abort_flag, r == 1 ? &slow : nullptr);
+            if (pw == PAIRS_LATE) { timed_out[gi] = 1; abort_flag.store(1, std::memory_order_relaxed); }
+            if (pw != PAIRS_OK) { pending[gi] = 1; break; }
+            if (slow) slow_first[gi] = 1;
+            ++answered[gi];
+            TL_ANSWERED(ctx, gi);
             if (!rg.absorb(ctx->hVal, ctx->hGrad, q0)) { got_nan[gi] = 1; abort_flag.store(1, std::memory_order_relaxed); break; }
             if (!rg.advance()) break;
           }
@@ -1154,6 +1170,7 @@
         hp.fn = [&] { for (int gi = 1; gi < ngroups; gi += T) advance(gi); };
         HIPCHK(hipStreamSynchronize(ctx->stream));
         ctx->seq = seq0 + std::max(used[0], used[1]) + 1;
+        ctx->res_rounds += answered[0] + answered[1];
         srv_cap = 0;
         if (got_nan[0] || got_nan[1]) return set_err(ctx, PCABO_ERR_NAN, "NaN in acquisition gradient%s", "");
         if (timed_out[0] || timed_out[1]) ctx->srv_penalty = 1000;
@@ -1166,13 +1183,16 @@
       const unsigned long long tag = ++ctx->seq;
       const double tp = now();
       server_post(ctx, srv_cap, nq, k, tag);
-      rc = server_wait(ctx, nq, tag);
+      TL_POSTED(ctx, 0);
+      rc = server_wait(ctx, nq, k, tag);
+      if (rc == PCABO_OK) { TL_ANSWERED(ctx, 0); }
       if (rc == PCABO_ERR_TIMEOUT) {
         server_stop.stop();
         ctx->srv_penalty = 1000;
         rc = eval_staged(ctx, nq, p);
-      } else if (round_no == 1 && now() - tp > 1e-3) {
-        ctx->srv_penalty = 40;
+      } else {
+        for (int gi = 0; gi < ngroups; ++gi) ctx->res_rounds += qoff[gi] >= 0;
+        if (round_no == 1 && now() - tp > 1e-3) ctx->srv_penalty = 40;
       }
     } else if (group_mode(ctx, nq, 1) && batch_limit <= PCABO_GROUP_Q && ngroups <= 8) {
       int g0[8], gn[8], ng = 0;
@@ -1199,6 +1219,8 @@
   if (failed) *failed = any_failed;
   return PCABO_OK;
 }
+
+long long pcabo_debug_resident_rounds(pcabo_ctx* ctx) { return ctx ? (long long)ctx->res_rounds : -1; }
 
 int pcabo_inverse_map(pcabo_ctx* ctx, const double* z, double* x) {
   if (!ctx || !z || !x) return PCABO_ERR_ARG;
diff --git a/para-ortho-pca-bo_amd/csrc/pcabo_internal.h b/para-ortho-pca-bo_amd/csrc/pcabo_internal.h
--- a/para-ortho-pca-bo_amd/csrc/pcabo_internal.h
+++ b/para-ortho-pca-bo_amd/csrc/pcabo_internal.h
@@ -14,11 +14,8 @@
 
 typedef double double4_t __attribute__((ext_vector_type(4)));
 struct QueryArgs { double x[PCABO_QA_MAX]; };
-struct alignas(16) MailPair { double v; unsigned long long tag; };
-static inline __host__ __device__ unsigned long long mail_mix(unsigned long long vbits) {
-  const unsigned int lo = (unsigned int)vbits, hi = (unsigned int)(vbits >> 32);
-  return (unsigned long long)((lo ^ hi ^ (hi >> 11)) & 0xFFFFFFu);
-}
+#include "mail_pair.h"
+#define PCABO_RES_PAIRS (PCABO_INLAUNCH_MAXQ * PCABO_RES_STRIDE(PCABO_RES_MAXK))
 #define PCABO_MAIL_PAIRS (1 + PCABO_QA_MAX + PCABO_INLAUNCH_MAXQ + 1)
 #define PCABO_SERVER_TIMEOUT_TICKS 200000000ull
 
@@ -99,6 +96,9 @@
 __device__ inline double pair_value(pcabo_u4 v) { return __hiloint2double((int)v.y, (int)v.x); }
 __device__ inline unsigned long long mail_seq(pcabo_u4 v) {
   return pair_tag(v) ^ mail_mix(((unsigned long long)v.y << 32) | v.x);
+}
+__device__ inline pcabo_u4 make_mail_pair(double v, unsigned long long seq) {
+  return make_pair(v, seq ^ mail_mix((unsigned long long)__double_as_longlong(v)));
 }
 
 template <typename T>
@@ -264,7 +264,8 @@
                 AcqParams p, double* partial, unsigned int* counters, double* val,
                 double* grad, double* host_val, double* host_grad, HostMirror* hm, unsigned long long seq,
                 MailPair* dev_mail = nullptr, MailPair* part_pairs = nullptr,
-                AcqBatch ab = AcqBatch(), int B = 1, int table_entries = 0);
+                AcqBatch ab = AcqBatch(), int B = 1, int table_entries = 0,
+                MailPair* res_pairs = nullptr);
 #define PCABO_GROUP_Q 5
 #define PCABO_GROUP_CNT_OFFSET 8192
 bool acq_group_possible(int NP, int k);
```
